# Diamondfan/CTC_pytorch

Measured on AMD Instinct MI355X. Metric: acoustic frames/sec/GPU (train) + utterances/sec beam-decode (`decode` object), TIMIT 4x320 BiLSTM, higher is better.
Workload: dtype f32 via bf16x3 split-operand MFMA (f32 accumulate); 1 GPU; cfg2: 4x320 BiLSTM + BN + Linear(62) + CTC, B=32/GPU, T=800, F=40, dropout 0.1, Adam; global_batch=32, seq_len=800, parallelism=dp1, full_length_utterances=True, sync_bn=False

## Files before the change

ctc_pytorch_amd/_lib.py:

```python
import ctypes
import glob
import os
import subprocess

import torch

_HERE = os.path.dirname(os.path.abspath(__file__))
_CSRC = os.path.join(_HERE, "csrc")
SO_PATH = os.environ.get("CTCN_LIBCTCN") or os.path.join(_HERE, "libctcn.so")
_lib = None

c_void_p, c_int, c_float, c_double, c_size_t, c_u64 = (ctypes.c_void_p, ctypes.c_int, ctypes.c_float,
                                                      ctypes.c_double, ctypes.c_size_t, ctypes.c_uint64)

P, I, F, D, Z, U = c_void_p, c_int, c_float, c_double, c_size_t, c_u64
_SIGS = {
    "ctcn_version": (I, []),
    "ctcn_last_error": (ctypes.c_char_p, []),
    "ctcn_device_cus": (I, []),
    "ctcn_device_xcds": (I, []),
    "ctcn_set_option": (I, [ctypes.c_char_p, I]),
    "ctcn_get_option": (I, [ctypes.c_char_p]),
    "ctcn_option_name": (ctypes.c_char_p, [I]),
    "ctcn_set_status_buffer": (I, [P]),
    "ctcn_gemm": (I, [I, I, I, I, I, P, I, P, I, P, I, F, I, P, Z, P]),
    "ctcn_gemm_dx": (I, [I, I, I, P, I, P, I, P, I, F, I, P, Z, P]),
    "ctcn_transpose01": (I, [P, P, I, I, I, P]),
    "ctcn_copy_strided4": (I, [P, P, I, I, I, I, Z, Z, Z, Z, P]),
    "ctcn_relu_fwd": (I, [P, P, Z, P]),
    "ctcn_relu_bwd": (I, [P, P, P, Z, P]),
    "ctcn_maxpool2d_fwd": (I, [P, P, P, Z, I, I, I, I, P]),
    "ctcn_maxpool2d_bwd": (I, [P, P, P, Z, I, I, I, I, P]),
    "ctcn_rnn_scratch_bytes": (Z, [I, I, I, I]),
    "ctcn_rnn_fwd": (I, [I, I, I, I, I, I, P, P, P, P, P, P, P, P, I, P, Z, P]),
    "ctcn_rnn_fwd_dropout": (I, [I, I, I, I, I, I, P, P, P, P, P, P, P, P, P, F, U, U, I, P, Z, P]),
    "ctcn_rnn_bwd": (I, [I, I, I, I, I, I, P, P, P, P, P, P, P, P, P, P, P, P, P, P, F, I, P, P, Z, P]),
    "ctcn_rnn_bwd_dropout": (I, [I, I, I, I, I, I, P, P, P, P, P, P, P, P, P, P, P, P, P, P, F, I, P, P, Z, P, F, U, U, P]),
    "ctcn_rnn_bwd_weights": (I, [I, I, I, I, I, I, P, P, P, P, P, P, P, P, F, I, ctypes.c_uint, P, Z, P]),
    "ctcn_bn_ws_bytes": (Z, [I, I, I]),
    "ctcn_bn_fwd_train": (I, [P, P, P, P, P, P, P, P, I, I, I, F, F, I, P, Z, P, P]),
    "ctcn_bn_fwd_eval": (I, [P, P, P, P, P, P, I, I, I, F, I, P]),
    "ctcn_bn_fwd_sums": (I, [P, P, I, I, I, P, Z, P]),
    "ctcn_bn_fwd_finish": (I, [P, P, P, P, P, P, P, P, P, D, I, I, I, F, F, I, P, P]),
    "ctcn_bn_bwd_sums": (I, [P, P, P, P, P, P, I, I, I, I, P, Z, P]),
    "ctcn_bn_bwd_finish": (I, [P, P, P, P, P, P, P, P, P, P, P, D, I, I, I, I, F, P, Z, P]),
    "ctcn_bn_bwd": (I, [P, P, P, P, P, P, P, P, P, I, I, I, I, F, P, Z, P]),
    "ctcn_bn_fwd_train_dropout": (I, [P, P, P, P, P, P, P, P, I, I, I, F, F, I, P, Z, P, P, F, U, U]),
    "ctcn_bn_bwd_dropout": (I, [P, P, P, P, P, P, P, P, P, I, I, I, I, F, P, Z, P, F, U, U]),
    "ctcn_dropout": (I, [P, P, Z, F, U, U, P]),
    "ctcn_bn_masked_ws_bytes": (Z, [I, I, I]),
    "ctcn_mask_frames": (I, [P, P, P, I, I, I, I, I, P]),
    "ctcn_bn_fwd_train_masked": (I, [P, P, P, P, P, P, P, P, P, I, I, I, I, I, F, F, I, P, Z, P, P]),
    "ctcn_bn_fwd_eval_masked": (I, [P, P, P, P, P, P, P, I, I, I, I, I, F, I, P]),
    "ctcn_bn_bwd_masked": (I, [P, P, P, P, P, P, P, P, P, P, I, I, I, I, I, I, F, P, Z, P]),
    "ctcn_conv2d_ws_bytes": (Z, [I] * 11),
    "ctcn_conv2d_fwd": (I, [P, P, P, P] + [I] * 11 + [P]),
    "ctcn_conv2d_bwd": (I, [P, P, P, P, P, P] + [I] * 11 + [F, P, Z, P]),
    "ctcn_bctf_to_tbcf": (I, [P, P, I, I, I, I, P]),
    "ctcn_tbcf_to_bctf": (I, [P, P, I, I, I, I, P]),
    "ctcn_log_softmax_fwd": (I, [P, P, P, I, I, P]),
    "ctcn_log_softmax_bwd": (I, [P, P, P, I, I, P]),
    "ctcn_argmax": (I, [P, P, I, I, P]),
    "ctcn_rnn_fwd_ex": (I, [I, I, I, I, I, I, P, P, P, P, P, P, P, P, I, P, Z, P, P]),
    "ctcn_rnn_bwd_ex": (I, [I, I, I, I, I, I, P, P, P, P, P, P, P, P, P, P, P, P, P, P, F, I, P, P, Z, P, P]),
    "ctcn_ctc_fwd": (I, [P, P, P, P, P, P, I, I, I, I, P]),
    "ctcn_ctc_bwd": (I, [P, P, P, P, P, P, P, P, I, I, I, I, P]),
    "ctcn_ctc_fwd_both": (I, [P, P, P, P, P, P, P, I, I, I, I, P]),
    "ctcn_ctc_grad": (I, [P, P, P, P, P, P, P, P, P, I, I, I, I, P]),
    "ctcn_sum_f32": (I, [P, P, I, P]),
    "ctcn_ctc_fwd_ex": (I, [P, P, P, P, P, P, P, I, I, I, I, I, P]),
    "ctcn_ctc_grad_ex": (I, [P, P, P, P, P, P, P, P, I, I, I, I, P, I, I, I, I, P]),
    "ctcn_ctc_reduce": (I, [P, P, P, I, I, I, P]),
    "ctcn_ctc_pack_targets": (I, [P, ctypes.c_int64, P, P, I, I, P]),
    "ctcn_ctc_align_ws_bytes": (Z, [I, I, I]),
    "ctcn_ctc_align": (I, [P, P, P, P, P, P, P, P, P, P, I, I, I, I, I, P, Z, P]),
    "ctcn_adam_step": (I, [P, P, P, P, Z, F, F, F, F, F, I, P]),
    "ctcn_grad_norm_ws_bytes": (Z, [Z, I]),
    "ctcn_grad_norm": (I, [P, Z, I, P, I, P, P, P, I, P, Z, P]),
    "ctcn_clip_control": (I, [P, F, F, F, F, I, P]),
    "ctcn_adam_step_ex": (I, [P, P, P, P, Z, F, F, F, F, P, P]),
    "ctcn_scale_by_device_scalar": (I, [P, Z, P, P]),
    "ctcn_greedy_collapse": (I, [P, Z, Z, P, P, P, I, I, I, P]),
    "ctcn_path_tokens": (I, [P, Z, Z, P, P, P, P, P, P, P, P, P, P, I, I, I, I, P]),
    "ctcn_edit_distance": (I, [P, P, P, P, P, I, I, I, I, P]),
    "ctcn_edit_ops_ws_bytes": (Z, [I, I, I]),
    "ctcn_edit_ops": (I, [P, P, P, P, P, I, P, P, P, P, I, I, I, I, P, Z, P]),
    "ctcn_step_stats": (I, [P, P, P, I, P, P, P]),
    "ctcn_fbank_frames": (I, [ctypes.c_longlong, I, I, I]),
    "ctcn_fbank_plan_bytes": (Z, [P]),
    "ctcn_fbank_plan": (I, [P, P, Z]),
    "ctcn_fbank": (I, [P, I, P, P, P, P, P, P, P, I, I, I, F, U, U, P]),
    "ctcn_mfcc_plan_bytes": (Z, [P]),
    "ctcn_mfcc_plan": (I, [P, P, Z]),
    "ctcn_mfcc": (I, [P, I, P, P, P, P, P, P, P, I, I, I, F, U, U, P]),
    "ctcn_spectrogram_plan_bytes": (Z, [P]),
    "ctcn_spectrogram_plan": (I, [P, P, Z]),
    "ctcn_spectrogram": (I, [P, I, P, P, P, P, P, P, P, I, I, I, F, U, U, P]),
    "ctcn_logspec_frames": (I, [ctypes.c_longlong, I]),
    "ctcn_logspec_plan_bytes": (Z, [P]),
    "ctcn_logspec_plan": (I, [P, P, Z]),
    "ctcn_logspec_ws_bytes": (Z, [P, I, I]),
    "ctcn_logspec": (I, [P, I, P, P, P, P, P, P, I, I, I, P, Z, P]),
    "ctcn_fbank_power_host": (I, [P, I, P]),
    "ctcn_resample_samples": (I, [ctypes.c_longlong, I, I]),
    "ctcn_resample_plan_bytes": (Z, [P]),
    "ctcn_resample_plan": (I, [P, P, Z]),
    "ctcn_resample": (I, [P, I, P, P, P, P, I, I, I, P]),
    "ctcn_resample_host": (I, [P, I, I, P, P, P, I]),
    "ctcn_context_frames": (I, [I, I, I]),
    "ctcn_delta_scales": (I, [I, I, P]),
    "ctcn_frame_context_tile": (I, [P, I]),
    "ctcn_frame_context": (I, [P, P, P, P, P, P, I, I, I, I, P]),
    "ctcn_frame_context_host": (I, [P, I, I, P, P, I, P]),
    "ctcn_spec_augment": (I, [P, P, P, U, U, P, I, I, I, P]),
    "ctcn_spec_augment_plan": (I, [P, U, U, I, I, P, P, P]),
    "ctcn_spec_augment_host": (I, [P, I, I, P, U, U, P]),
    "ctcn_reverb_limits": (I, [P]),
    "ctcn_reverb_bank_bytes": (Z, [I, I, I, I, I]),
    "ctcn_reverb_bank": (I, [P, P, I, I, P, P, I, I, P, I, D, P, Z]),
    "ctcn_reverb_plan": (I, [P, P, U, U, P]),
    "ctcn_reverb_ws_bytes": (Z, [P, I, I]),
    "ctcn_reverb": (I, [P, I, P, P, P, P, U, U, P, I, I, P, Z, P]),
    "ctcn_reverb_host": (I, [P, I, I, P, P, U, U, P]),
    "ctcn_cmvn_accumulate_ws_bytes": (Z, [I, I, I]),
    "ctcn_cmvn_accumulate": (I, [P, P, P, I, I, I, P, Z, P]),
    "ctcn_cmvn_accumulate_groups": (I, [P, P, P, P, I, I, I, I, P, Z, P]),
    "ctcn_cmvn_apply": (I, [P, P, P, P, P, I, I, I, I, I, P]),
    "ctcn_cmvn_sliding": (I, [P, P, P, I, I, I, P, P]),
    "ctcn_cmvn_sliding_run": (I, [P]),
    "ctcn_cmvn_sliding_window": (I, [I, I, P, P, P]),
    "ctcn_cmvn_sliding_host": (I, [P, I, I, P, P]),
    "ctcn_cmvn_norm_host": (I, [P, I, I, P, P]),
    "ctcn_comm_unique_id": (I, [P]),
    "ctcn_comm_init": (I, [P, I, I, ctypes.POINTER(ctypes.c_void_p)]),
    "ctcn_comm_allreduce_sum_f32": (I, [P, P, Z, P]),
    "ctcn_comm_destroy": (I, [P]),
    "ctcn_diag_squat": (I, [I, I, I, ctypes.c_uint, P]),
    "ctcn_diag_pipeline_chunks": (I, [I, I, I, I, I, I, I, I, ctypes.c_uint]),
    "ctcn_diag_gemm_plan": (I, [I] * 13 + [Z, ctypes.c_uint, I, I, I, I, P]),
    "ctcn_diag_dx_plan": (I, [I, I, I, I, I, I, I, Z, I, P]),
    "ctcn_diag_beam_plan": (I, [I, I, I, I, I, I, P]),
    "ctcn_diag_ctc_lattice_plan": (I, [I, P]),
    "ctcn_diag_gemm_on_xcds": (I, [I, I, I, I, I, P, I, P, I, P, I, F, I, P, Z, P, ctypes.c_uint]),
    "ctcn_rnn_last_kernel": (ctypes.c_char_p, [I]),
    "ctcn_levenshtein": (ctypes.c_longlong, [P, ctypes.c_longlong, P, ctypes.c_longlong]),
    "ctcn_levenshtein_ops": (ctypes.c_longlong, [P, ctypes.c_longlong, P, ctypes.c_longlong, P, P]),
    "ctcn_join_tokens": (ctypes.c_longlong, [P, ctypes.c_longlong, P, I, P, P, P, I, I, P, ctypes.c_longlong, P]),
    "ctcn_beam_ws_bytes": (Z, [I, I, I, I]),
    "ctcn_beam_decode": (I, [P, I, P, P, D, I, I, P, P, P, P, I, I, I, P, Z, P]),
    "ctcn_beam_decode_nbest": (I, [P, I, P, P, D, I, I, I, P, P, P, P, P, I, I, I, P, Z, P]),
}


class RnnCall(ctypes.Structure):
    _fields_ = [("drop_p", ctypes.c_float), ("drop_seed", ctypes.c_uint64), ("drop_offset", ctypes.c_uint64), ("y_drop", ctypes.c_void_p),
                ("dy_tmp", ctypes.c_void_p), ("side_stream", ctypes.c_void_p), ("side_event", ctypes.c_void_p), ("side_ws", ctypes.c_void_p),
                ("side_ws_bytes", ctypes.c_size_t), ("xcd_allow", ctypes.c_uint), ("prelaunch_event", ctypes.c_void_p), ("status", ctypes.c_void_p),
                ("launched", ctypes.POINTER(ctypes.c_char_p))]


class FbankOpts(ctypes.Structure):
    _fields_ = [(k, ctypes.c_float) for k in ("samp_freq", "frame_shift_ms", "frame_length_ms", "preemph_coeff", "blackman_coeff", "low_freq",
                                              "high_freq", "energy_floor")] + \
               [(k, ctypes.c_int32) for k in ("window_type", "num_mel_bins", "remove_dc_offset", "round_to_power_of_two", "snip_edges",
                                              "use_energy", "raw_energy", "htk_compat", "use_log_fbank", "use_power")]


class MfccOpts(ctypes.Structure):
    _fields_ = [(k, ctypes.c_float) for k in ("samp_freq", "frame_shift_ms", "frame_length_ms", "preemph_coeff", "blackman_coeff", "low_freq",
                                              "high_freq", "energy_floor", "cepstral_lifter")] + \
               [(k, ctypes.c_int32) for k in ("window_type", "num_mel_bins", "num_ceps", "remove_dc_offset", "round_to_power_of_two", "snip_edges",
                                              "use_energy", "raw_energy", "htk_compat")]


class SpectrogramOpts(ctypes.Structure):
    _fields_ = [(k, ctypes.c_float) for k in ("samp_freq", "frame_shift_ms", "frame_length_ms", "preemph_coeff", "blackman_coeff", "energy_floor")] + \
               [(k, ctypes.c_int32) for k in ("window_type", "remove_dc_offset", "round_to_power_of_two", "snip_edges", "raw_energy", "return_raw_fft")]


class LogSpecOpts(ctypes.Structure):
    _fields_ = [(k, ctypes.c_double) for k in ("sample_rate", "window_size", "window_stride")] + [("input_scale", ctypes.c_float)] + \
               [(k, ctypes.c_int32) for k in ("window", "normalize")]


class ResampleOpts(ctypes.Structure):
    _fields_ = [("cutoff", ctypes.c_double)] + [(k, ctypes.c_int32) for k in ("orig_freq", "new_freq", "num_zeros")]


class ContextOpts(ctypes.Structure):
    _fields_ = [(k, ctypes.c_int32) for k in ("left", "right", "skip", "n_downsample", "delta_order", "delta_window")]


class SpecAugOpts(ctypes.Structure):
    _fields_ = [(k, ctypes.c_int32) for k in ("warp_window", "num_freq_masks", "freq_width", "num_time_masks", "time_width")] + \
               [(k, ctypes.c_float) for k in ("time_ratio", "fill")]


class ReverbOpts(ctypes.Structure):
    _fields_ = [("rir_prob", ctypes.c_float), ("noise_prob", ctypes.c_float), ("normalize", ctypes.c_int32)]


class SlidingCmnOpts(ctypes.Structure):
    _fields_ = [(k, ctypes.c_int32) for k in ("cmn_window", "min_cmn_window", "normalize_variance", "center")]


def sources():
    return sorted(glob.glob(os.path.join(_CSRC, "*.hip")))


def build(force=False, verbose=False):
    from concurrent.futures import ThreadPoolExecutor
    srcs = sources()
    hdrs = glob.glob(os.path.join(_CSRC, "*.h")) + [os.path.join(os.path.dirname(_HERE), "include", "ctcn.h")]
    hipcc = os.environ.get("HIPCC", "/opt/rocm/bin/hipcc")
    objdir = os.path.join(_CSRC, "_obj")
    os.makedirs(objdir, exist_ok=True)
    hdr_time = max(os.path.getmtime(h) for h in hdrs)
    flags = ["--offload-arch=gfx950", "-O3", "-std=c++17", "-fPIC"]
    jobs, objs = [], []
    for src in srcs:
        obj = os.path.join(objdir, os.path.basename(src)[:-4] + ".o")
        objs.append(obj)
        if force or not os.path.exists(obj) or os.path.getmtime(obj) < max(os.path.getmtime(src), hdr_time):
            jobs.append([hipcc] + flags + ["-c", src, "-o", obj])

    def run(cmd):
        if verbose:
            print(" ".join(cmd), flush=True)
        subprocess.check_call(cmd)

    if jobs:
        with ThreadPoolExecutor(max_workers=min(len(jobs), os.cpu_count() or 4)) as pool:
            list(pool.map(run, jobs))
    if jobs or not os.path.exists(SO_PATH) or any(os.path.getmtime(SO_PATH) < os.path.getmtime(o) for o in objs):
        run([hipcc, "--offload-arch=gfx950", "-fPIC", "-shared", "-o", SO_PATH] + objs)
    return SO_PATH


def lib():
    global _lib
    if _lib is None:
        if not os.path.exists(SO_PATH):
            raise RuntimeError(
                "ctc_pytorch_amd: %s is missing -- run `python -c 'import __graft_entry__ as g; g.build()'` "
                "(hipcc --offload-arch=gfx950). There is no CPU fallback." % SO_PATH)
        l = ctypes.CDLL(SO_PATH)
        for name, (res, args) in _SIGS.items():
            fn = getattr(l, name)
            fn.restype = res
            fn.argtypes = args
        _lib = l
        for var, opt in (("CTCN_RNN_PERSISTENT", b"rnn_persistent"), ("CTCN_HANDOFF", b"handoff"), ("CTCN_GEMM_BIG_TILES", b"gemm_big_tiles"), ("CTCN_BWD_SCATTER", b"bwd_scatter"), ("CTCN_HANDOFF_TAGS", b"handoff_tags"), ("CTCN_SIDE_SPLIT_WGS", b"side_split_wgs")):
            env = os.environ.get(var)
            if env is not None:
                l.ctcn_set_option(opt, int(env))
        for var, val in os.environ.items():
            if var.startswith("CTCN_OPT_"):
                check(l.ctcn_set_option(var[len("CTCN_OPT_"):].lower().encode(), int(val)), "set_option(%s)" % var)
    return _lib


def exported_symbols():
    return sorted(_SIGS)


def check(rc, what=""):
    if rc != 0:
        msg = lib().ctcn_last_error()
        raise RuntimeError("libctcn %s failed (rc=%d): %s" % (what, rc, msg.decode() if msg else "?"))


def stream_ptr():
    return torch.cuda.current_stream().cuda_stream


_STATUS = {}


def status_word(device):
    key = (device.type, device.index)
    t = _STATUS.get(key)
    if t is None:
        t = torch.zeros(1, dtype=torch.int32, device=device)
        _STATUS[key] = t
        check(lib().ctcn_set_status_buffer(ctypes.c_void_p(t.data_ptr())), "set_status_buffer")
    return t


def check_status(device):
    t = _STATUS.get((device.type, device.index))
    if t is not None:
        v = int(t.item())
        if v != 0:
            t.zero_()
            raise RuntimeError("libctcn: persistent recurrent kernel reported status %d (in-launch hand-off timed out)" % v)


_WS = {}
_WS_LOCK = __import__("threading").Lock()
WORKSPACE_BYTES = int(os.environ.get("CTCN_WORKSPACE_MB", "1024")) << 20


def workspace(device, nbytes=None, tag="main"):
    nbytes = WORKSPACE_BYTES if nbytes is None else nbytes
    key = (device.type, device.index, tag)
    buf = _WS.get(key)
    if buf is None or buf.numel() < nbytes:
        with _WS_LOCK:
            buf = _WS.get(key)
            if buf is None or buf.numel() < nbytes:
                buf = torch.empty(nbytes, dtype=torch.uint8, device=device)
# ... 3 lines not shown
```

ctc_pytorch_amd/csrc/common.h:

```cpp
#pragma once
#include <hip/hip_runtime.h>
#include <stdarg.h>
#include <stdint.h>
#include <stdio.h>
#include <string.h>

#include "../../include/ctcn.h"

void ctcn_set_error(const char *fmt, ...);
int *ctcn_status_word(void);
int ctcn_opt_rnn_persistent(void);
int ctcn_transpose01_pair(const float *in0, const float *in1, float *out0, float *out1, int A, int B, int C, void *stream);
struct GemmPlanes {
  const float *A = nullptr; int lda = 0, M = 0, Ka = 0, transA = 0; void *ws_a = nullptr, *st_a = nullptr; bool a_valid = false;
  const float *B = nullptr; int ldb = 0, N = 0, Kb = 0, transB = 0, shift = 0; void *ws_b = nullptr, *st_b = nullptr; const void *bh = nullptr; bool b_valid = false;
  bool same_a = false, same_b = false;
};
int ctcn_gemm_on_xcds(int transA, int transB, int M, int N, int K, const float *A, int lda, const float *B, int ldb, float *C,
                      int ldc, float beta, int precision, void *ws, size_t ws_bytes, void *stream, unsigned xcd_allow, GemmPlanes *planes = nullptr);
int ctcn_gemm_shift_b(int M, int N, int K, const float *A, int lda, const float *B, int ldb, float *C, int ldc, float beta, int precision,
                      void *ws, size_t ws_bytes, void *stream, unsigned xcd_allow, int shift, GemmPlanes *planes = nullptr);
int ctcn_opt_handoff(void);
int ctcn_opt_poll_depth(void);
int ctcn_opt_bwd_scatter(void);
int ctcn_opt_handoff_tags(void);
int ctcn_opt_side_split_wgs(void);
int ctcn_opt_gemm_big_tiles(void);
int ctcn_opt_recurrence_only(void);

#define CTCN_REQUIRE(cond, ...)          \
  do {                                   \
    if (!(cond)) {                       \
      ctcn_set_error(__VA_ARGS__);       \
      return CTCN_EINVAL;                \
    }                                    \
  } while (0)

#define CTCN_HIP(expr)                                                                   \
  do {                                                                                   \
    hipError_t e__ = (expr);                                                             \
    if (e__ != hipSuccess) {                                                             \
      ctcn_set_error("%s:%d: %s -> %s", __FILE__, __LINE__, #expr, hipGetErrorString(e__)); \
      return CTCN_EHIP;                                                                  \
    }                                                                                    \
  } while (0)

#define CTCN_LAUNCH_CHECK() CTCN_HIP(hipGetLastError())

typedef float f32x4 __attribute__((ext_vector_type(4)));
typedef float f32x16 __attribute__((ext_vector_type(16)));
typedef short bf16x8 __attribute__((ext_vector_type(8)));
typedef unsigned int u32x4 __attribute__((ext_vector_type(4)));

static inline int ceil_div(int a, int b) { return (a + b - 1) / b; }
static inline size_t ceil_div_z(size_t a, size_t b) { return (a + b - 1) / b; }
static inline size_t align_up(size_t a, size_t b) { return (a + b - 1) / b * b; }

__device__ __forceinline__ float wave_max(float v) {
#pragma unroll
  for (int o = 32; o > 0; o >>= 1) v = fmaxf(v, __shfl_xor(v, o, 64));
  return v;
}
__device__ __forceinline__ float wave_sum(float v) {
#pragma unroll
  for (int o = 32; o > 0; o >>= 1) v += __shfl_xor(v, o, 64);
  return v;
}
__device__ __forceinline__ double wave_sum_d(double v) {
#pragma unroll
  for (int o = 32; o > 0; o >>= 1) v += __shfl_xor(v, o, 64);
  return v;
}
__device__ __forceinline__ void lds_barrier() { asm volatile("s_waitcnt lgkmcnt(0)\n\ts_barrier" ::: "memory"); }

__device__ __forceinline__ float sigmoidf_(float x) { return 1.0f / (1.0f + expf(-x)); }

__host__ __device__ __forceinline__ void philox_round(uint32_t (&c)[4], uint32_t (&k)[2]) {
  const uint32_t M0 = 0xD2511F53u, M1 = 0xCD9E8D57u;
#if defined(__HIP_DEVICE_COMPILE__)
  const uint32_t hi0 = __umulhi(M0, c[0]), lo0 = M0 * c[0];
  const uint32_t hi1 = __umulhi(M1, c[2]), lo1 = M1 * c[2];
#else
  const uint32_t hi0 = (uint32_t)(((uint64_t)M0 * c[0]) >> 32), lo0 = M0 * c[0];
  const uint32_t hi1 = (uint32_t)(((uint64_t)M1 * c[2]) >> 32), lo1 = M1 * c[2];
#endif
  const uint32_t n0 = hi1 ^ c[1] ^ k[0], n1 = lo1, n2 = hi0 ^ c[3] ^ k[1], n3 = lo0;
  c[0] = n0; c[1] = n1; c[2] = n2; c[3] = n3;
  k[0] += 0x9E3779B9u; k[1] += 0xBB67AE85u;
}
__host__ __device__ __forceinline__ void philox4(uint64_t seed, uint64_t ctr, uint32_t (&out)[4]) {
  uint32_t c[4] = {(uint32_t)ctr, (uint32_t)(ctr >> 32), 0u, 0u};
  uint32_t k[2] = {(uint32_t)seed, (uint32_t)(seed >> 32)};
#pragma unroll
  for (int i = 0; i < 10; ++i) philox_round(c, k);
#pragma unroll
  for (int i = 0; i < 4; ++i) out[i] = c[i];
}

__device__ __forceinline__ unsigned short f2bf(float f) {
  return __builtin_bit_cast(unsigned short, (__bf16)f);
}
```

ctc_pytorch_amd/csrc/core.hip:

```cpp
#include "common.h"

static thread_local char g_err[512] = "";

void ctcn_set_error(const char *fmt, ...) {
  va_list ap;
  va_start(ap, fmt);
  vsnprintf(g_err, sizeof(g_err), fmt, ap);
  va_end(ap);
}

extern "C" int ctcn_version(void) { return 100; }
extern "C" const char *ctcn_last_error(void) { return g_err; }
extern "C" int ctcn_device_cus(void) {
  int dev = 0, n = 0;
  if (hipGetDevice(&dev) != hipSuccess) return -1;
  if (hipDeviceGetAttribute(&n, hipDeviceAttributeMultiprocessorCount, dev) != hipSuccess) return -1;
  return n;
}

static int g_opt_rnn_persistent = 1;
static int g_opt_handoff = 1;
static int g_opt_poll_depth = 2;
static int g_opt_recurrence_only = 0;
static int g_opt_bwd_scatter = 1;
static int g_opt_handoff_tags = 1;
static int g_opt_side_split_wgs = 8;
static int g_opt_gemm_big_tiles = 0;
static int g_opt_gemm_tile256 = 1;
static int g_opt_gemm_dbg = 0;
static int g_opt_gemm_a_inline = 1;
static int g_opt_conv_mfma = 1;
static int g_opt_rnn_fwd_tagged = 1;
static int g_opt_rnn_fused_dropout = 1;
static int g_opt_gemm_tn = 1;
static int g_opt_tag_poll_delay = 8;
static int g_opt_edit_wave = 1;
static int g_opt_bwd_item_gather = 1;
static int g_opt_bwd_poll_delay = -1;
static int g_opt_fwd_rsv_lds = 2;
static int g_opt_fwd_pipe_any_chunking = 0;
static int g_opt_fwd_pipe_min_input = 0;
static int g_opt_conv_dbg = 0;
static int g_opt_gemm_bf16_single = 0;
static int g_opt_gemm_dx_wide = 1;
static int g_opt_xcd_interleave = 1;
static int g_opt_bn_rows4 = 1;
static int g_opt_tn_splits_force = 0;
static int g_opt_tn_splits_xcd = 1;
static int g_opt_beam_generic_threads = 0;
static int g_opt_beam_bitonic = 1;
static int g_opt_beam_cand_global = 0;
static int g_opt_beam_occ2 = 0;
static int g_opt_beam_fast = 1;
static int g_opt_rnn_slow_items = 0;
static int g_opt_rnn_slow_exchange = 0;
static int g_opt_ctc_lattice_skew = 1;
static int g_opt_ctc_slow_wave = 0;
static int g_opt_xcd_interleave_force = 0;
static int *g_status_dev = nullptr;

struct OptionRow { const char *name; int *var; int (*norm)(int); };
static const OptionRow k_options[] = {
  {"rnn_persistent", &g_opt_rnn_persistent, [](int value) -> int { return value; }},
  {"handoff", &g_opt_handoff, [](int value) -> int { return value; }},
  {"poll_depth", &g_opt_poll_depth, [](int value) -> int { return value; }},
  {"rnn_recurrence_only", &g_opt_recurrence_only, [](int value) -> int { return value ? 1 : 0; }},
  {"bwd_scatter", &g_opt_bwd_scatter, [](int value) -> int { return value ? 1 : 0; }},
  {"handoff_tags", &g_opt_handoff_tags, [](int value) -> int { return value ? 1 : 0; }},
  {"side_split_wgs", &g_opt_side_split_wgs, [](int value) -> int { return value < 1 ? 1 : (value > 16 ? 16 : value); }},
  {"gemm_big_tiles", &g_opt_gemm_big_tiles, [](int value) -> int { return value ? 1 : 0; }},
  {"beam_fast", &g_opt_beam_fast, [](int value) -> int { return value ? 1 : 0; }},
  {"conv_dbg", &g_opt_conv_dbg, [](int value) -> int { return value & 7; }},
  {"tn_splits_xcd", &g_opt_tn_splits_xcd, [](int value) -> int { return value ? 1 : 0; }},
  {"xcd_interleave", &g_opt_xcd_interleave, [](int value) -> int { return value < 0 ? 0 : (value > 5 ? 5 : value); }},
  {"bn_rows4", &g_opt_bn_rows4, [](int value) -> int { return value ? 1 : 0; }},
  {"tn_splits_force", &g_opt_tn_splits_force, [](int value) -> int { return value < 0 ? 0 : value; }},
  {"gemm_bf16_single", &g_opt_gemm_bf16_single, [](int value) -> int { return value ? 1 : 0; }},
  {"gemm_dx_wide", &g_opt_gemm_dx_wide, [](int value) -> int { return value < 0 ? 0 : (value > 2 ? 2 : value); }},
  {"beam_generic_threads", &g_opt_beam_generic_threads, [](int value) -> int { return (value == 256 || value == 512 || value == 1024) ? value : 0; }},
  {"beam_cand_global", &g_opt_beam_cand_global, [](int value) -> int { return value ? 1 : 0; }},
  {"beam_bitonic", &g_opt_beam_bitonic, [](int value) -> int { return value ? 1 : 0; }},
  {"beam_occ2", &g_opt_beam_occ2, [](int value) -> int { return value < 0 ? 0 : (value > 2 ? 2 : value); }},
  {"fwd_pipe_min_input", &g_opt_fwd_pipe_min_input, [](int value) -> int { return value < 0 ? 0 : value; }},
  {"fwd_pipe_any_chunking", &g_opt_fwd_pipe_any_chunking, [](int value) -> int { return value ? 1 : 0; }},
  {"fwd_rsv_lds", &g_opt_fwd_rsv_lds, [](int value) -> int { return value < 0 ? 0 : (value > 2 ? 2 : value); }},
  {"bwd_item_gather", &g_opt_bwd_item_gather, [](int value) -> int { return value < 0 ? 0 : (value > 2 ? 2 : value); }},
  {"bwd_poll_delay", &g_opt_bwd_poll_delay, [](int value) -> int { return value < 0 ? -1 : (value > 256 ? 256 : value); }},
  {"conv_mfma", &g_opt_conv_mfma, [](int value) -> int { return value ? 1 : 0; }},
  {"edit_wave", &g_opt_edit_wave, [](int value) -> int { return value ? 1 : 0; }},
  {"gemm_tn", &g_opt_gemm_tn, [](int value) -> int { return value != 0; }},
  {"rnn_fused_dropout", &g_opt_rnn_fused_dropout, [](int value) -> int { return value != 0; }},
  {"tag_poll_delay", &g_opt_tag_poll_delay, [](int value) -> int { return value < 0 ? 0 : (value > 64 ? 64 : value); }},
  {"rnn_fwd_tagged", &g_opt_rnn_fwd_tagged, [](int value) -> int { return value ? 1 : 0; }},
  {"gemm_a_inline", &g_opt_gemm_a_inline, [](int value) -> int { return value ? 1 : 0; }},
  {"gemm_dbg", &g_opt_gemm_dbg, [](int value) -> int { return value; }},
  {"gemm_tile256", &g_opt_gemm_tile256, [](int value) -> int { return value ? 1 : 0; }},
  {"xcd_interleave_force", &g_opt_xcd_interleave_force, [](int value) -> int { return value ? 1 : 0; }},
  {"rnn_slow_exchange", &g_opt_rnn_slow_exchange, [](int value) -> int { return value < 0 ? 0 : (value > 4096 ? 4096 : value); }},
  {"ctc_lattice_skew", &g_opt_ctc_lattice_skew, [](int value) -> int { return value ? 1 : 0; }},
  {"ctc_slow_wave", &g_opt_ctc_slow_wave, [](int value) -> int { return value < 0 ? 0 : (value > 15 ? 15 : value); }},
  {"rnn_slow_items", &g_opt_rnn_slow_items, [](int value) -> int { return value < 0 ? 0 : (value > 4096 ? 4096 : value); }},
};
static const int k_noptions = (int)(sizeof(k_options) / sizeof(k_options[0]));
static const OptionRow *find_option(const char *name) {
  if (name)
    for (int i = 0; i < k_noptions; ++i)
      if (!strcmp(name, k_options[i].name)) return &k_options[i];
  return nullptr;
}
extern "C" int ctcn_set_option(const char *name, int value) {
  if (const OptionRow *o = find_option(name)) { *o->var = o->norm(value); return CTCN_OK; }
  ctcn_set_error("ctcn_set_option: unknown option %s", name ? name : "(null)");
  return CTCN_EINVAL;
}
extern "C" int ctcn_get_option(const char *name) {
  const OptionRow *o = find_option(name);
  return o ? *o->var : -1;
}
extern "C" const char *ctcn_option_name(int index) { return index >= 0 && index < k_noptions ? k_options[index].name : nullptr; }
extern "C" int ctcn_set_status_buffer(int *dev_word) { g_status_dev = dev_word; return CTCN_OK; }
int *ctcn_status_word(void) { return g_status_dev; }
int ctcn_opt_rnn_persistent(void) { return g_opt_rnn_persistent; }
int ctcn_opt_handoff(void) { return g_opt_handoff; }
int ctcn_opt_poll_depth(void) { return g_opt_poll_depth; }
int ctcn_opt_recurrence_only(void) { return g_opt_recurrence_only; }
int ctcn_opt_bwd_scatter(void) { return g_opt_bwd_scatter; }
int ctcn_opt_handoff_tags(void) { return g_opt_handoff_tags; }
int ctcn_opt_side_split_wgs(void) { return g_opt_side_split_wgs; }
int ctcn_opt_gemm_big_tiles(void) { return g_opt_gemm_big_tiles; }
```

ctc_pytorch_amd/csrc/gemm.hip:

```cpp
#include <algorithm>
#include <type_traits>

#include "common.h"

namespace {

constexpr int BM = 128, BN = 128, BK = 16, PAD = 4;

__device__ __forceinline__ int xcd_band_tile(int bid, int nt) {
  const int xcd = bid & 7, q = nt >> 3, r = nt & 7;
  return (xcd < r ? xcd * (q + 1) : r * (q + 1) + (xcd - r) * q) + (bid >> 3);
}
__device__ __forceinline__ void g2r_kc(const float *__restrict__ src, int ld, int r0, int R, int k0, int Kend,
                                       bool vec, int tid, float (&reg)[8]) {
#pragma unroll
  for (int j = 0; j < 2; ++j) {
    const int idx = tid + 256 * j;
    const int r = idx >> 2, kq = (idx & 3) * 4;
    const int gr = r0 + r, gk = k0 + kq;
    const float *p = src + (size_t)gr * ld + gk;
    if (vec && gr < R && gk + 3 < Kend) {
      const float4 v = *reinterpret_cast<const float4 *>(p);
      reg[4 * j + 0] = v.x; reg[4 * j + 1] = v.y; reg[4 * j + 2] = v.z; reg[4 * j + 3] = v.w;
    } else {
#pragma unroll
      for (int c = 0; c < 4; ++c) reg[4 * j + c] = (gr < R && gk + c < Kend) ? p[c] : 0.0f;
    }
  }
}
__device__ __forceinline__ void r2s_kc(float (*s)[BM + PAD], int tid, const float (&reg)[8]) {
#pragma unroll
  for (int j = 0; j < 2; ++j) {
    const int idx = tid + 256 * j;
    const int r = idx >> 2, kq = (idx & 3) * 4;
#pragma unroll
    for (int c = 0; c < 4; ++c) s[kq + c][r] = reg[4 * j + c];
  }
}
__device__ __forceinline__ void g2r_mc(const float *__restrict__ src, int ld, int r0, int R, int k0, int Kend,
                                       bool vec, int tid, float (&reg)[8]) {
#pragma unroll
  for (int j = 0; j < 2; ++j) {
    const int idx = tid + 256 * j;
    const int k = idx >> 5, rq = (idx & 31) * 4;
    const int gk = k0 + k, gr = r0 + rq;
    const float *p = src + (size_t)gk * ld + gr;
    if (vec && gk < Kend && gr + 3 < R) {
      const float4 v = *reinterpret_cast<const float4 *>(p);
      reg[4 * j + 0] = v.x; reg[4 * j + 1] = v.y; reg[4 * j + 2] = v.z; reg[4 * j + 3] = v.w;
    } else {
#pragma unroll
      for (int c = 0; c < 4; ++c) reg[4 * j + c] = (gk < Kend && gr + c < R) ? p[c] : 0.0f;
    }
  }
}
__device__ __forceinline__ void r2s_mc(float (*s)[BM + PAD], int tid, const float (&reg)[8]) {
#pragma unroll
  for (int j = 0; j < 2; ++j) {
    const int idx = tid + 256 * j;
    const int k = idx >> 5, rq = (idx & 31) * 4;
    *reinterpret_cast<float4 *>(&s[k][rq]) = make_float4(reg[4 * j], reg[4 * j + 1], reg[4 * j + 2], reg[4 * j + 3]);
  }
}

template <bool TA, bool TB>
__device__ __forceinline__ void f32_tile(float (*sA)[BM + PAD], float (*sB)[BN + PAD], int bid, int split, int M, int N, int K,
                                         const float *__restrict__ A, int lda, const float *__restrict__ B, int ldb, float *__restrict__ C,
                                         int ldc, float beta, int kchunk, float *__restrict__ ws, int tiles_n, bool vecA, bool vecB) {
  const int tid = threadIdx.x, lane = tid & 63, wave = tid >> 6;
  const int wm = wave >> 1, wn = wave & 1;
  const int tm = bid / tiles_n, tn = bid - tm * tiles_n;
  const int m0 = tm * BM, n0 = tn * BN;
  const int kbeg = split * kchunk;
  const int kend = min(K, kbeg + kchunk);

  f32x16 acc[2][2];
#pragma unroll
  for (int i = 0; i < 2; ++i)
#pragma unroll
    for (int j = 0; j < 2; ++j)
#pragma unroll
      for (int e = 0; e < 16; ++e) acc[i][j][e] = 0.0f;

  float ra[8], rb[8];
  auto loadA = [&](int k0) {
    if (TA) g2r_mc(A, lda, m0, M, k0, kend, vecA, tid, ra);
    else g2r_kc(A, lda, m0, M, k0, kend, vecA, tid, ra);
  };
  auto loadB = [&](int k0) {
    if (TB) g2r_kc(B, ldb, n0, N, k0, kend, vecB, tid, rb);
    else g2r_mc(B, ldb, n0, N, k0, kend, vecB, tid, rb);
  };
  if (kbeg < kend) {
    loadA(kbeg);
    loadB(kbeg);
  }
  for (int k0 = kbeg; k0 < kend; k0 += BK) {
    __syncthreads();
    if (TA) r2s_mc(sA, tid, ra); else r2s_kc(sA, tid, ra);
    if (TB) r2s_kc(sB, tid, rb); else r2s_mc(sB, tid, rb);
    __syncthreads();
    if (k0 + BK < kend) {
      loadA(k0 + BK);
      loadB(k0 + BK);
    }
    const int kl = lane >> 5, ml = lane & 31;
#pragma unroll
    for (int k = 0; k < BK; k += 2) {
      const float a0 = sA[k + kl][wm * 64 + ml], a1 = sA[k + kl][wm * 64 + 32 + ml];
      const float b0 = sB[k + kl][wn * 64 + ml], b1 = sB[k + kl][wn * 64 + 32 + ml];
      acc[0][0] = __builtin_amdgcn_mfma_f32_32x32x2f32(a0, b0, acc[0][0], 0, 0, 0);
      acc[0][1] = __builtin_amdgcn_mfma_f32_32x32x2f32(a0, b1, acc[0][1], 0, 0, 0);
      acc[1][0] = __builtin_amdgcn_mfma_f32_32x32x2f32(a1, b0, acc[1][0], 0, 0, 0);
      acc[1][1] = __builtin_amdgcn_mfma_f32_32x32x2f32(a1, b1, acc[1][1], 0, 0, 0);
    }
  }
  float *out = ws ? ws + (size_t)split * M * N : C;
  const int ldo = ws ? N : ldc;
#pragma unroll
  for (int i = 0; i < 2; ++i)
#pragma unroll
    for (int j = 0; j < 2; ++j) {
      const int col = n0 + wn * 64 + j * 32 + (lane & 31);
#pragma unroll
      for (int e = 0; e < 16; ++e) {
        const int row = m0 + wm * 64 + i * 32 + (e & 3) + 8 * (e >> 2) + 4 * (lane >> 5);
        if (row < M && col < N) {
          float v = acc[i][j][e];
          float *p = out + (size_t)row * ldo + col;
          if (!ws && beta != 0.0f) v += beta * *p;
          *p = v;
        }
      }
    }
}

template <bool TA, bool TB>
__global__ __launch_bounds__(256) void gemm_f32_kernel(int M, int N, int K, const float *__restrict__ A, int lda,
                                                       const float *__restrict__ B, int ldb, float *__restrict__ C,
                                                       int ldc, float beta, int kchunk, float *__restrict__ ws,
                                                       int tiles_m, int tiles_n, bool vecA, bool vecB) {
  __shared__ __attribute__((aligned(16))) float sA[BK][BM + PAD];
  __shared__ __attribute__((aligned(16))) float sB[BK][BN + PAD];
  const int bid = xcd_band_tile(blockIdx.x, tiles_m * tiles_n);
  f32_tile<TA, TB>(sA, sB, bid, blockIdx.y, M, N, K, A, lda, B, ldb, C, ldc, beta, kchunk, ws, tiles_n, vecA, vecB);
}

template <bool TA, bool TB>
__global__ __launch_bounds__(256) void gemm_f32_queue_kernel(int M, int N, int K, const float *__restrict__ A, int lda,
                                                             const float *__restrict__ B, int ldb, float *__restrict__ C, int ldc,
                                                             float beta, int kchunk, float *__restrict__ ws, int tiles_m, int tiles_n,
                                                             bool vecA, bool vecB, int splits, unsigned xcd_allow,
                                                             unsigned *__restrict__ queue) {
// ... 961 lines not shown
    for (int t = 0; t < 3; ++t)
#pragma unroll
      for (int i = 0; i < WI; ++i)
#pragma unroll
        for (int j = 0; j < WJ; ++j) {
          if (t == 0) acc[i][j] = __builtin_amdgcn_mfma_f32_32x32x16_bf16(al[i], bh[j], acc[i][j], 0, 0, 0);
          else if (t == 1) acc[i][j] = __builtin_amdgcn_mfma_f32_32x32x16_bf16(ah[i], bl[j], acc[i][j], 0, 0, 0);
          else acc[i][j] = __builtin_amdgcn_mfma_f32_32x32x16_bf16(ah[i], bh[j], acc[i][j], 0, 0, 0);
          const int n = t * NMM + i * WJ + j;
          if (n < NBP || n == CV0 || n == CV0 + 1) {
            __builtin_amdgcn_sched_barrier(0);
            if constexpr (WHICH == 1) {
              if (HAS1 && n < NBP) issue_b_piece(n, (s + 1) * 32, (s + 1) & 1);
              if (HAS1 && n == CV0) {
                static_assert(NBP == 5, "vmcnt literals");
                if constexpr (HAS2) WAIT_A(7, 1); else WAIT_A(5, 1);
              }
              if (HAS1 && n >= CV0) convert_half(1, n - CV0, (s + 1) * 32);
            } else {
              if (HAS2 && n == CV0) WAIT_A(2, 0);
              if (HAS2 && n >= CV0) convert_half(0, n - CV0, (s + 2) * 32);
            }
            __builtin_amdgcn_sched_barrier(0);
          }
        }
  };
  constexpr std::integral_constant<int, 1> first{};
  constexpr std::integral_constant<int, 2> second{};
  constexpr std::integral_constant<bool, true> yes{};
  constexpr std::integral_constant<bool, false> no{};
#pragma unroll
  for (int q = 0; q < 4; ++q) aw[q] = (u32x4){0u, 0u, 0u, 0u};
#pragma unroll
  for (int q = 0; q < 4; ++q) load_a_piece(q, 0);
#pragma unroll
  for (int n = 0; n < NBP; ++n) issue_b_piece(n, 0, 0);
  WAIT_A(0, 0); WAIT_A(0, 1);
#pragma unroll
  for (int r = 0; r < 2; ++r) {
    convert_half(r, 0, 0); convert_half(r, 1, 0);
    store_a_row(r, 0);
  }
  if (nst > 1) {
    asm volatile("s_waitcnt lgkmcnt(0)" ::: "memory");
#pragma unroll
    for (int q = 0; q < 4; ++q) load_a_piece(q, 32);
    WAIT_A(2, 0);
    convert_half(0, 0, 32); convert_half(0, 1, 32);
  }
  pp_barrier_vm();
  if (wave >= 4) pp_barrier();
#ifdef CTCN_GEMM_STATS
  long long gs_work[4] = {0, 0, 0, 0}, gs_wait[4] = {0, 0, 0, 0};
  const long long gs_t0 = clock64();
  long long gs_prev = gs_t0;
#endif
  auto stage = [&](int s, auto has1, auto has2) {
    constexpr bool HAS1 = decltype(has1)::value, HAS2 = decltype(has2)::value;
    load_frags(s, 0);
    if constexpr (HAS1) store_a_row(0, (s + 1) & 1);
    if constexpr (HAS2) {
      __builtin_amdgcn_sched_barrier(0);
      load_a_piece(0, (s + 2) * 32); load_a_piece(1, (s + 2) * 32);
    }
    PPB(0);
    multiply(first, has1, has2, s);
    PPB(1);
    load_frags(s, 1);
    if constexpr (HAS1) store_a_row(1, (s + 1) & 1);
    if constexpr (HAS2) {
      __builtin_amdgcn_sched_barrier(0);
      load_a_piece(2, (s + 2) * 32); load_a_piece(3, (s + 2) * 32);
    }
#ifdef CTCN_GEMM_STATS
    PPB_VM(2);
#else
    __builtin_amdgcn_sched_barrier(0);
    if constexpr (HAS2) asm volatile("s_waitcnt vmcnt(2) lgkmcnt(0)\n\ts_barrier" ::: "memory");
    else asm volatile("s_waitcnt vmcnt(0) lgkmcnt(0)\n\ts_barrier" ::: "memory");
    __builtin_amdgcn_sched_barrier(0);
#endif
    multiply(second, has1, has2, s);
    PPB(3);
  };
  int s = 0;
  for (; s + 2 < nst; ++s) stage(s, yes, yes);
#ifdef CTCN_GEMM_STATS
  if (lane == 0 && (wave & 3) == 0 && (blockIdx.x == 0 || blockIdx.x == 1000) && g_gemm_stats) {
    long long *o = g_gemm_stats + ((blockIdx.x ? 2 : 0) + (wave >> 2)) * 16;
    for (int i = 0; i < 4; ++i) { o[i] = gs_work[i]; o[4 + i] = gs_wait[i]; }
    o[8] = clock64() - gs_t0; o[9] = nst - 2; o[10] = 0;
  }
#endif
  if (s + 1 < nst) { stage(s, yes, no); ++s; }
  stage(s, no, no);
  if (wave < 4) pp_barrier();
  int zero = 0;
  asm volatile("" : "+v"(zero));
  const int elane = (int)__builtin_amdgcn_mbcnt_hi(~0u, __builtin_amdgcn_mbcnt_lo(~0u, (unsigned)zero));
#pragma unroll
  for (int i = 0; i < WI; ++i)
#pragma unroll
    for (int j = 0; j < WJ; ++j) {
      const int col = n0 + wn * 160 + j * 32 + (elane & 31);
#pragma unroll
      for (int e = 0; e < 16; ++e) {
        const int row = m0 + wm * 64 + i * 32 + (e & 3) + 8 * (e >> 2) + 4 * (elane >> 5);
        if (row < M) {
          float v = acc[i][j][e];
          float *p = C + (size_t)row * ldc + col;
          if (beta != 0.0f) v += beta * *p;
          *p = v;
        }
      }
    }
}


typedef short s16x4_t __attribute__((ext_vector_type(4)));
typedef short s16x8_t __attribute__((ext_vector_type(8)));

template <int WNT, int NP = 3>
__global__ __launch_bounds__(512) void gemm_tn_f32_pp_kernel(int M, int N, int K, const float *__restrict__ A, int lda, const float *__restrict__ B,
                                                             int ldb, float *__restrict__ C, int ldc, float beta, int kchunk, int splits,
                                                             float *__restrict__ part, int tiles_m, int tiles_n, unsigned xcd_mask,
                                                             unsigned *__restrict__ queue) {
  constexpr int TBM = 256, TBN = 128 * WNT;
  constexpr int A_BYTES = TBM * 64, B_BYTES = TBN * 64;
  constexpr int STAGE = 2 * A_BYTES + 2 * B_BYTES;
  constexpr int NB = 2 * WNT;
  constexpr int NMM = 4 * WNT;
  extern __shared__ __attribute__((aligned(16))) unsigned char qsm[];
  __shared__ int s_item;
  {
    unsigned xcc;
    asm volatile("s_getreg_b32 %0, hwreg(HW_REG_XCC_ID)" : "=s"(xcc));
    if (!((xcd_mask >> (xcc & 15u)) & 1u)) return;
  }
  const int tid = threadIdx.x, lane = tid & 63, wave = __builtin_amdgcn_readfirstlane(tid >> 6);
  const int wm = wave >> 2, wn = wave & 3;
  const int nt = tiles_m * tiles_n;
  const int krow = lane >> 3, c4 = 4 * (lane & 7);
  const int bsub = WNT == 2 ? wave : (wave & 3), bk0 = WNT == 2 ? 0 : 16 * (wave >> 2);
  const int st_a = wave * 2048 + krow * 64 + (lane & 7) * 8;
  const int st_b = 2 * A_BYTES + bsub * 2048 + (bk0 + krow) * 64 + (lane & 7) * 8;
  const int troff = (8 * (lane >> 5) + ((lane & 15) >> 2)) * 64 + ((lane >> 4) & 1) * 32 + (lane & 3) * 8;
  typedef __attribute__((address_space(3))) s16x4_t *lds4_t;

  for (;;) {
    if (tid == 0) s_item = (int)atomicAdd(queue, 1u);
    __syncthreads();
    const int item = __builtin_amdgcn_readfirstlane(s_item);
    if (item >= nt * splits) return;
    const int z = item / nt, tile = item - z * nt;
    const int tm = tile / tiles_n, tn = tile - tm * tiles_n;
    const int m0 = tm * TBM, n0 = tn * TBN;
    const int kbeg = z * kchunk, kend = min(K, kbeg + kchunk);
    const int nst = (kend - kbeg + 31) / 32;

    f32x16 acc[4][WNT];
#pragma unroll
    for (int i = 0; i < 4; ++i)
#pragma unroll
      for (int j = 0; j < WNT; ++j)
#pragma unroll
        for (int e = 0; e < 16; ++e) acc[i][j][e] = 0.0f;

    const int acol = m0 + 32 * wave + c4, bcol = n0 + 32 * bsub + c4;
    const bool a_ok = acol < M, b_ok = bcol < N;
    u32x4 pw[4 + NB];
    const unsigned voff_a = a_ok ? (unsigned)((krow * lda + acol) * 4) : 0xfffffff0u;
    const unsigned voff_b = b_ok ? (unsigned)((krow * ldb + bcol) * 4) : 0xfffffff0u;
    auto load_piece = [&](int q, int k0) {
      const int kr = q < 4 ? k0 + 8 * q : k0 + bk0 + 8 * (q - 4);
      const int ld = q < 4 ? lda : ldb;
      const float *base = (q < 4 ? A : B) + (size_t)min(kr, K - 1) * ld;
      int rows = min(8, kend - kr);
      asm volatile("" : "+s"(rows));
      const int nrec = max(0, rows) * ld * 4;
      const __amdgpu_buffer_rsrc_t rs = __builtin_amdgcn_make_buffer_rsrc(const_cast<float *>(base), 0, nrec, 0x00020000);
      pw[q] = __builtin_amdgcn_raw_buffer_load_b128(rs, q < 4 ? voff_a : voff_b, 0, 0);
    };
    auto split_pair = [](float a, float b, unsigned &hw, unsigned &lw) {
      typedef __bf16 bf16x2_t __attribute__((ext_vector_type(2)));
      typedef float f32x2_t __attribute__((ext_vector_type(2)));
      hw = __builtin_bit_cast(unsigned, __builtin_convertvector((f32x2_t){a, b}, bf16x2_t));
      const f32x2_t r = {a - __uint_as_float(hw << 16), b - __uint_as_float(hw & 0xffff0000u)};
      lw = __builtin_bit_cast(unsigned, __builtin_convertvector(r, bf16x2_t));
    };
    auto convert_piece = [&](int q) {
      unsigned h01, l01, h23, l23;
      if constexpr (NP == 3) {
        split_pair(__uint_as_float(pw[q][0]), __uint_as_float(pw[q][1]), h01, l01);
        split_pair(__uint_as_float(pw[q][2]), __uint_as_float(pw[q][3]), h23, l23);
      } else {
        typedef __bf16 bf16x2_t __attribute__((ext_vector_type(2)));
        typedef float f32x2_t __attribute__((ext_vector_type(2)));
        h01 = __builtin_bit_cast(unsigned, __builtin_convertvector((f32x2_t){__uint_as_float(pw[q][0]), __uint_as_float(pw[q][1])}, bf16x2_t));
        h23 = __builtin_bit_cast(unsigned, __builtin_convertvector((f32x2_t){__uint_as_float(pw[q][2]), __uint_as_float(pw[q][3])}, bf16x2_t));
        l01 = l23 = 0u;
      }
      pw[q] = (u32x4){h01, h23, l01, l23};
    };
    auto store_ab = [&](int buf) {
      unsigned char *sb = qsm + buf * STAGE;
#pragma unroll
      for (int q = 0; q < 4 + NB; ++q) {
        unsigned char *p = sb + (q < 4 ? st_a + q * 512 : st_b + (q - 4) * 512);
        *reinterpret_cast<uint2 *>(p) = make_uint2(pw[q][0], pw[q][1]);
        if constexpr (NP == 3) *reinterpret_cast<uint2 *>(p + (q < 4 ? A_BYTES : B_BYTES)) = make_uint2(pw[q][2], pw[q][3]);
      }
    };
    bf16x8_t ah[4], al[4], bh[WNT], bl[WNT];
    auto tr_frag = [&](const unsigned char *p) {
      const s16x4_t x0 = __builtin_amdgcn_ds_read_tr16_b64_v4i16((lds4_t)(p));
      const s16x4_t x1 = __builtin_amdgcn_ds_read_tr16_b64_v4i16((lds4_t)(p + 256));
      return __builtin_bit_cast(bf16x8_t, __builtin_shufflevector(x0, x1, 0, 1, 2, 3, 4, 5, 6, 7));
    };
    auto load_frags = [&](int stage, int ks) {
      const unsigned char *sb = qsm + (stage & 1) * STAGE + ks * 1024 + troff;
#pragma unroll
      for (int j = 0; j < WNT; ++j) {
        const unsigned char *p = sb + 2 * A_BYTES + (wn * WNT + j) * 2048;
        bh[j] = tr_frag(p);
        if constexpr (NP == 3) bl[j] = tr_frag(p + B_BYTES);
      }
#pragma unroll
      for (int i = 0; i < 4; ++i) {
        const unsigned char *p = sb + (wm * 4 + i) * 2048;
        ah[i] = tr_frag(p);
        if constexpr (NP == 3) al[i] = tr_frag(p + A_BYTES);
      }
    };
    auto multiply = [&](auto mode, int k0) {
      constexpr int MODE = decltype(mode)::value;
      constexpr int NITEM = MODE == 1 ? 4 : 4 + NB;
#pragma unroll
      for (int t = 0; t < NP; ++t)
#pragma unroll
        for (int i = 0; i < 4; ++i)
#pragma unroll
          for (int j = 0; j < WNT; ++j) {
            if (NP == 3 && t == 0) acc[i][j] = __builtin_amdgcn_mfma_f32_32x32x16_bf16(al[i], bh[j], acc[i][j], 0, 0, 0);
            else if (NP == 3 && t == 1) acc[i][j] = __builtin_amdgcn_mfma_f32_32x32x16_bf16(ah[i], bl[j], acc[i][j], 0, 0, 0);
            else acc[i][j] = __builtin_amdgcn_mfma_f32_32x32x16_bf16(ah[i], bh[j], acc[i][j], 0, 0, 0);
            const int n = t * NMM + i * WNT + j;
            if constexpr (NP == 3) {
              if (MODE != 0 && (n & 1) && (n >> 1) < NITEM) {
                __builtin_amdgcn_sched_barrier(0);
                if constexpr (MODE == 1) load_piece(n >> 1, k0);
                if constexpr (MODE == 2) convert_piece(n >> 1);
                __builtin_amdgcn_sched_barrier(0);
              }
            } else if (MODE != 0 && 2 * n < NITEM) {
              __builtin_amdgcn_sched_barrier(0);
#pragma unroll
              for (int u = 2 * n; u < 2 * n + 2 && u < NITEM; ++u) {
                if constexpr (MODE == 1) load_piece(u, k0);
                if constexpr (MODE == 2) convert_piece(u);
              }
              __builtin_amdgcn_sched_barrier(0);
            }
          }
    };
    constexpr std::integral_constant<int, 0> bare{};
    constexpr std::integral_constant<int, 1> with_loads{};
    constexpr std::integral_constant<int, 2> with_split{};
#pragma unroll
    for (int q = 0; q < 4 + NB; ++q) load_piece(q, kbeg);
#pragma unroll
    for (int q = 0; q < 4 + NB; ++q) convert_piece(q);
    store_ab(0);
    if (nst > 1) {
#pragma unroll
      for (int q = 0; q < 4; ++q) load_piece(q, kbeg + 32);
    }
    pp_barrier();
    if (wm == 1) pp_barrier();
#ifdef CTCN_GEMM_STATS
    long long gs_work[4] = {0, 0, 0, 0}, gs_wait[4] = {0, 0, 0, 0};
    const long long gs_t0 = clock64();
    long long gs_prev = gs_t0;
#endif
    auto stage = [&](int s, auto do_store, auto c1) {
      load_frags(s, 0);
      if constexpr (decltype(do_store)::value == 1) {
        __builtin_amdgcn_sched_barrier(0);
#pragma unroll
        for (int q = 4; q < 4 + NB; ++q) load_piece(q, kbeg + (s + 1) * 32);
      }
      PPB(0);
      if constexpr (decltype(do_store)::value == 1) multiply(with_split, 0);
      else multiply(bare, 0);
      PPB(1);
      load_frags(s, 1);
      if constexpr (decltype(do_store)::value == 1) store_ab((s + 1) & 1);
      PPB(2);
      multiply(c1, kbeg + (s + 2) * 32);
      PPB(3);
    };
    int s = 0;
    for (; s + 2 < nst; ++s) stage(s, with_loads, with_loads);
#ifdef CTCN_GEMM_STATS
    if (lane == 0 && (wave & 3) == 0 && item == 0 && g_gemm_stats) {
      long long *o = g_gemm_stats + (wave >> 2) * 16;
      for (int i = 0; i < 4; ++i) { o[i] = gs_work[i]; o[4 + i] = gs_wait[i]; }
      o[8] = clock64() - gs_t0; o[9] = nst - 2; o[10] = 0;
    }
#endif
    if (s + 1 < nst) { stage(s, with_loads, bare); ++s; }
    stage(s, bare, bare);
    if (wm == 0) pp_barrier();

    float *o = splits > 1 ? part + (size_t)z * M * N : C;
    const int ldo = splits > 1 ? N : ldc;
    const float bt = splits > 1 ? 0.0f : beta;
#pragma unroll
    for (int i = 0; i < 4; ++i)
#pragma unroll
      for (int j = 0; j < WNT; ++j) {
        const int col = n0 + wn * 32 * WNT + j * 32 + (lane & 31);
#pragma unroll
        for (int e = 0; e < 16; ++e) {
          const int row = m0 + wm * 128 + i * 32 + (e & 3) + 8 * (e >> 2) + 4 * (lane >> 5);
          if (row < M && col < N) {
            float v = acc[i][j][e];
            float *p = o + (size_t)row * ldo + col;
            if (bt != 0.0f) v += bt * *p;
            *p = v;
          }
        }
      }
    __syncthreads();
  }
}

__global__ void splitk_reduce_kernel(const float *__restrict__ ws, float *__restrict__ C, int M, int N, int ldc,
                                     int splits, float beta) {
  const size_t total = (size_t)M * N;
  if ((N & 3) == 0 && (ldc & 3) == 0 && (((uintptr_t)C | (uintptr_t)ws) & 15) == 0 && total < ((size_t)1 << 33)) {
    const unsigned n4 = (unsigned)(N >> 2), total4 = (unsigned)(total >> 2);
    const float4 *w4 = reinterpret_cast<const float4 *>(ws);
    for (unsigned i = blockIdx.x * blockDim.x + threadIdx.x; i < total4; i += gridDim.x * blockDim.x) {
      float4 s = {0.0f, 0.0f, 0.0f, 0.0f};
      int z = 0;
      for (; z + 8 <= splits; z += 8) {
        float4 v[8];
#pragma unroll
        for (int u = 0; u < 8; ++u) v[u] = w4[(size_t)(z + u) * total4 + i];
#pragma unroll
        for (int u = 0; u < 8; ++u) { s.x += v[u].x; s.y += v[u].y; s.z += v[u].z; s.w += v[u].w; }
      }
      for (; z < splits; ++z) { const float4 v = w4[(size_t)z * total4 + i]; s.x += v.x; s.y += v.y; s.z += v.z; s.w += v.w; }
      const unsigned m = i / n4, n = (i - m * n4) << 2;
      float4 *p = reinterpret_cast<float4 *>(C + (size_t)m * ldc + n);
      if (beta != 0.0f) { const float4 o = *p; s.x += beta * o.x; s.y += beta * o.y; s.z += beta * o.z; s.w += beta * o.w; }
      *p = s;
    }
    return;
  }
  for (size_t i = blockIdx.x * (size_t)blockDim.x + threadIdx.x; i < total; i += (size_t)gridDim.x * blockDim.x) {
    float s = 0.0f;
    int z = 0;
    for (; z + 8 <= splits; z += 8) {
      float v[8];
#pragma unroll
      for (int u = 0; u < 8; ++u) v[u] = ws[(size_t)(z + u) * total + i];
#pragma unroll
      for (int u = 0; u < 8; ++u) s += v[u];
    }
    for (; z < splits; ++z) s += ws[(size_t)z * total + i];
    const size_t m = i / N, n = i - m * N;
    float *p = C + m * ldc + n;
    if (beta != 0.0f) s += beta * *p;
    *p = s;
  }
}

__global__ void transpose01_kernel(const float *__restrict__ in, float *__restrict__ out, int A, int B, int C) {
  const size_t total = (size_t)A * B * C;
  for (size_t i = blockIdx.x * (size_t)blockDim.x + threadIdx.x; i < total; i += (size_t)gridDim.x * blockDim.x) {
    const int c = i % C;
    const size_t ab = i / C;
    const int a = ab % A;
    const int b = ab / A;
    out[i] = in[((size_t)a * B + b) * C + c];
  }
}

}

enum GemmPath { GP_F32 = 0, GP_F32_QUEUE, GP_BF16X3, GP_PLANES128, GP_PLANES128_QUEUE, GP_PLANES256, GP_PLANES256_AF32, GP_PLANES256_QUEUE, GP_TN };
enum SplitPass { SP_NONE = 0, SP_ROWS, SP_TRANSPOSE, SP_TRANSPOSE_QUEUE };
struct GemmShape { int transA, transB, M, N, K, lda, ldb, ldc, precision, b_shift; };
struct GemmOptions { int tile256, a_inline, tn, big_tiles, tn_splits_xcd, tn_splits_force; };
struct GemmEnv {
  int a_mod16, b_mod16;
  bool has_ws;
  size_t ws_bytes;
  unsigned xcd_allow;
  bool same_a, same_b;
  int cus, xcds;
  GemmOptions opt;
};
struct GemmPlan {
  GemmPath path;
  int ti, tj;
  int wnt;
  int splits, kchunk;
  SplitPass split_a, split_b;
  int Kp;
  size_t off_al, off_bh, off_bl, off_part, off_queue;
  int tiles_m, tiles_n;
  unsigned grid_x, grid_y;
  bool vecA, vecB;
  unsigned xcd_mask;
};
static bool uses_planes(GemmPath p) { return p >= GP_PLANES128 && p <= GP_PLANES256_QUEUE; }
static GemmOptions gemm_options() {
  return {ctcn_get_option("gemm_tile256"), ctcn_get_option("gemm_a_inline"), ctcn_get_option("gemm_tn"), ctcn_opt_gemm_big_tiles(),
          ctcn_get_option("tn_splits_xcd"), ctcn_get_option("tn_splits_force")};
}
static int check_gemm_shape(const GemmShape &g) {
  CTCN_REQUIRE(g.precision == 0 || g.precision == 1, "ctcn_gemm: precision %d (0 = f32 MFMA, 1 = bf16x3 split MFMA)", g.precision);
  CTCN_REQUIRE(g.M > 0 && g.N > 0 && g.K >= 0, "ctcn_gemm: bad dims M=%d N=%d K=%d", g.M, g.N, g.K);
  CTCN_REQUIRE(g.lda >= (g.transA ? g.M : g.K) && g.ldb >= (g.transB ? g.K : g.N) && g.ldc >= g.N, "ctcn_gemm: leading dim too small");
  return CTCN_OK;
}
struct PlaneLayout { int Kp; size_t a_el, b_el, bytes; };
static PlaneLayout plane_layout(int M, int N, int K) {
  const int Kp = ceil_div(K, PBK) * PBK;
  const size_t a_el = (size_t)M * Kp, b_el = (size_t)N * Kp;
  return {Kp, a_el, b_el, align_up(2 * (a_el + b_el) * sizeof(unsigned short), 256)};
}
static bool tn_eligible(const GemmShape &g, const GemmEnv &e) {
  return g.precision == 1 && g.transA && !g.transB && e.has_ws && e.ws_bytes >= 1024 && e.opt.tn != 0 && g.M >= 128 && g.N >= 32 && g.K >= 1024 &&
         g.M % 4 == 0 && g.N % 4 == 0 && g.lda % 4 == 0 && g.ldb % 4 == 0 && e.a_mod16 == 0 && e.b_mod16 == 0 &&
         g.lda < (1 << 24) && g.ldb < (1 << 24);
}

static GemmPlan plan_gemm(const GemmShape &g, const GemmEnv &e) {
  const int M = g.M, N = g.N, K = g.K;
  const size_t mn_bytes = (size_t)M * N * sizeof(float);
  GemmPlan p = {};
  p.splits = 1;
  p.off_queue = e.ws_bytes >= 256 ? (e.ws_bytes - 256) & ~(size_t)255 : 0;
  if (tn_eligible(g, e) && g.b_shift == 0) {
    p.path = GP_TN;
    p.wnt = ceil_div(N, 256) * 256 == ceil_div(N, 128) * 128 ? 2 : 1;
    p.ti = 4; p.tj = 2 * p.wnt;
    p.tiles_m = ceil_div(M, 256); p.tiles_n = ceil_div(N, 128 * p.wnt);
    int cus = 256;
    if (e.xcd_allow && e.opt.tn_splits_xcd != 0) {
      const int nx = std::max(1, std::min(e.xcds, 16));
      cus = std::max(e.cus / nx * __builtin_popcount(e.xcd_allow & ((1u << nx) - 1u)), 32);
    }
    const int tiles = p.tiles_m * p.tiles_n;
    int s = std::min(std::max(cus / tiles, 1), std::max(K / 512, 1));
    s = std::min(s, 32);
    if (const int f = e.opt.tn_splits_force) s = std::min(f, std::max(K / 64, 1));
    s = std::min(s, (int)((e.ws_bytes - 512) / mn_bytes));
    if (s < 2) s = 1;
    p.kchunk = ceil_div(ceil_div(K, s), 32) * 32;
    p.splits = ceil_div(K, p.kchunk);
    const int nx = std::min(e.xcds, 16);
    p.xcd_mask = e.xcd_allow ? e.xcd_allow : (nx > 1 ? (1u << nx) - 1u : 0xffffu);
    p.grid_x = e.cus; p.grid_y = 1;
    return p;
  }
  const PlaneLayout lay = plane_layout(M, N, K);
  if (g.precision == 1 && K >= 64 && e.has_ws && e.ws_bytes >= lay.bytes + 1024) {
    const int Kp = p.Kp = lay.Kp;
    p.off_al = lay.a_el * sizeof(unsigned short); p.off_bh = 2 * p.off_al; p.off_bl = p.off_bh + lay.b_el * sizeof(unsigned short);
    p.off_part = lay.bytes;
    const size_t part_bytes = e.ws_bytes - lay.bytes - 512;
    p.kchunk = Kp;
    const SplitPass pass_a = g.transA == 0 ? SP_ROWS : (e.xcd_allow ? SP_TRANSPOSE_QUEUE : SP_TRANSPOSE);
    const SplitPass pass_b = g.transB != 0 ? SP_ROWS : (e.xcd_allow ? SP_TRANSPOSE_QUEUE : SP_TRANSPOSE);
    p.split_b = e.same_b ? SP_NONE : pass_b;
    const int wnt256 = (N % 256 == 0 || (N > 512 && ceil_div(N, 256) * 256 - N <= N / 8)) ? 2 : 1;
    const int t256_m = ceil_div(M, 256), t256_n = ceil_div(N, 128 * wnt256);
    const bool use256 = !e.xcd_allow && e.opt.tile256 != 0 && M >= 1024 && N >= 96 && (long)t256_m * t256_n * 4 >= (long)e.cus * 3;
    const bool a_inline = use256 && !e.same_a && !g.transA && e.opt.a_inline != 0 && K >= 32 && K % 4 == 0 && g.lda % 4 == 0 && e.a_mod16 == 0 &&
                          t256_n <= 5;
    p.split_a = (a_inline || e.same_a) ? SP_NONE : pass_a;
    bool queue256 = false;
    if (e.xcd_allow && e.opt.tile256 != 0 && M >= 1024 && N >= 96) {
      const int cus = e.cus / std::max(1, std::min(e.xcds, 16)) * __builtin_popcount(e.xcd_allow);
      const int t256 = t256_m * t256_n, rounds = ceil_div(t256, std::max(cus, 1));
      queue256 = cus > 0 && t256 * 4 >= rounds * cus * 3;
    }
    if (use256 || queue256) {
      p.path = a_inline ? GP_PLANES256_AF32 : (use256 ? GP_PLANES256 : GP_PLANES256_QUEUE);
      p.wnt = wnt256; p.ti = 4; p.tj = 2 * wnt256;
      p.tiles_m = t256_m; p.tiles_n = t256_n;
      p.grid_x = queue256 ? e.cus : t256_m * t256_n; p.grid_y = 1;
      return p;
    }
    p.ti = p.tj = 2; p.tiles_m = ceil_div(M, BM); p.tiles_n = ceil_div(N, BN);
    {
      const long t22 = (long)p.tiles_m * p.tiles_n * 128 * 128;
      const int m42 = ceil_div(M, 256), n42 = ceil_div(N, 128), m24 = ceil_div(M, 128), n24 = ceil_div(N, 256);
      const long t42 = (long)m42 * n42 * 256 * 128, t24 = (long)m24 * n24 * 128 * 256;
      const bool ok42 = m42 * n42 >= e.cus && t42 <= t22 + t22 / 32, ok24 = m24 * n24 >= e.cus && t24 <= t22 + t22 / 32;
      if (e.opt.big_tiles && (ok42 || ok24)) {
        if (ok24 && (!ok42 || t24 <= t42)) { p.tj = 4; p.tiles_m = m24; p.tiles_n = n24; }
        else { p.ti = 4; p.tiles_m = m42; p.tiles_n = n42; }
      }
    }
    const int pnt = p.tiles_m * p.tiles_n;
    if (pnt < 256 && Kp >= 1024 && part_bytes >= 2 * mn_bytes) {
      p.splits = std::min(std::min(ceil_div(512, pnt), Kp / 512), (int)(part_bytes / mn_bytes));
      if (p.splits < 2) p.splits = 1;
    }
    if (p.splits > 1) {
      p.kchunk = ceil_div(ceil_div(Kp, p.splits), PBK) * PBK;
      p.splits = ceil_div(Kp, p.kchunk);
    }
    p.path = e.xcd_allow ? GP_PLANES128_QUEUE : GP_PLANES128;
    p.grid_x = e.xcd_allow ? 2 * e.cus : pnt; p.grid_y = e.xcd_allow ? 1 : p.splits;
    return p;
  }
  p.ti = p.tj = 2; p.tiles_m = ceil_div(M, BM); p.tiles_n = ceil_div(N, BN);
  const int nt = p.tiles_m * p.tiles_n;
  if (nt < 256 && K >= 512 && e.has_ws && e.ws_bytes >= 2 * mn_bytes) {
    p.splits = std::min(std::min(ceil_div(512, nt), K / 256), (int)(e.ws_bytes / mn_bytes));
    if (p.splits < 2) p.splits = 1;
  }
  p.kchunk = K;
// ... 52 lines not shown
  GemmPlanes scratch_planes;
  GemmPlanes &pl = planes ? *planes : scratch_planes;
  const bool want_same_a = pl.same_a, want_same_b = pl.same_b;
  pl.same_a = pl.same_b = false;
  const GemmShape g = {transA, transB, M, N, K, lda, ldb, ldc, precision, b_shift};
  if (const int rc = check_gemm_shape(g)) return rc;
  CTCN_REQUIRE(A && B && C, "ctcn_gemm: null pointer");
  CTCN_REQUIRE(!ws || (uintptr_t)ws % 16 == 0, "ctcn_gemm: the workspace must be 16-byte aligned");
  hipStream_t st = (hipStream_t)stream;
  char *const wsb = (char *)ws;
  const void *bh_here = wsb + 2 * plane_layout(M, N, K).a_el * sizeof(unsigned short);
  GemmEnv e = {(int)((uintptr_t)A & 15), (int)((uintptr_t)B & 15), ws != nullptr, ws_bytes, xcd_allow, false, false, ctcn_device_cus(), 0, gemm_options()};
  e.same_a = want_same_a && pl.a_valid && pl.A == A && pl.lda == lda && pl.M == M && pl.Ka == K && pl.transA == transA && pl.ws_a == ws && pl.st_a == (void *)st;
  e.same_b = want_same_b && pl.b_valid && pl.B == B && pl.ldb == ldb && pl.N == N && pl.Kb == K && pl.transB == transB && pl.shift == b_shift &&
             pl.ws_b == ws && pl.st_b == (void *)st && pl.bh == bh_here;
  if (xcd_allow || tn_eligible(g, e)) e.xcds = ctcn_device_xcds();
  const GemmPlan p = plan_gemm(g, e);

  unsigned short *ah = (unsigned short *)wsb, *al = (unsigned short *)(wsb + p.off_al), *bh = (unsigned short *)(wsb + p.off_bh),
                 *bl = (unsigned short *)(wsb + p.off_bl);
  float *part = p.splits > 1 ? (float *)(wsb + p.off_part) : nullptr;
  unsigned *queue = (unsigned *)(wsb + p.off_queue);
  pl.a_valid = pl.b_valid = false;
  if (uses_planes(p.path)) {
    pl.B = B; pl.ldb = ldb; pl.N = N; pl.Kb = K; pl.transB = transB; pl.shift = b_shift; pl.ws_b = ws;
    pl.st_b = (void *)st; pl.bh = (const void *)bh; pl.b_valid = true;
    if (p.path != GP_PLANES256_AF32) {
      pl.A = A; pl.lda = lda; pl.M = M; pl.Ka = K; pl.transA = transA; pl.ws_a = ws; pl.st_a = (void *)st;
      pl.a_valid = true;
    }
    if (xcd_allow) CTCN_HIP(hipMemsetAsync(queue, 0, 16, st));
    int nq = 0;
    launch_split(p.split_a, st, A, lda, M, K, p.Kp, ah, al, 0, xcd_allow, queue + (p.split_a == SP_TRANSPOSE_QUEUE ? ++nq : 0));
    launch_split(p.split_b, st, B, ldb, N, K, p.Kp, bh, bl, b_shift, xcd_allow, queue + (p.split_b == SP_TRANSPOSE_QUEUE ? ++nq : 0));
    CTCN_LAUNCH_CHECK();
  }
  const int tiles_m = p.tiles_m, tiles_n = p.tiles_n, Kp = p.Kp, kchunk = p.kchunk, splits = p.splits;
  const dim3 grid(p.grid_x, p.grid_y);
  int rc = CTCN_OK;
  switch (p.path) {
    case GP_TN:
      CTCN_HIP(hipMemsetAsync(queue, 0, 128, st));
      rc = with_wnt(p.wnt, [&](auto W) {
        constexpr int WNT = decltype(W)::value;
        return launch_tile256(bf16_single() ? gemm_tn_f32_pp_kernel<WNT, 1> : gemm_tn_f32_pp_kernel<WNT, 3>, p.grid_x, WNT, st, M, N, K, A, lda, B, ldb, C, ldc,
                              beta, kchunk, splits, part, tiles_m, tiles_n, p.xcd_mask, queue);
      });
      break;
    case GP_PLANES256_AF32:
      rc = with_wnt(p.wnt, [&](auto W) {
        constexpr int WNT = decltype(W)::value;
        return launch_tile256(bf16_single() ? gemm_planes_nt256pp_af32_kernel<WNT, 1> : gemm_planes_nt256pp_af32_kernel<WNT, 3>, p.grid_x, WNT, st, M, N, K, Kp,
                              A, lda, (const unsigned short *)bh, (const unsigned short *)bl, C, ldc, beta, tiles_m, tiles_n);
      });
      break;
    case GP_PLANES256:
      rc = with_wnt(p.wnt, [&](auto W) {
        constexpr int WNT = decltype(W)::value;
        return launch_tile256(bf16_single() ? gemm_planes_nt256pp_kernel<WNT, 1> : gemm_planes_nt256pp_kernel<WNT, 3>, p.grid_x, WNT, st, M, N, Kp,
                              (const unsigned short *)ah, (const unsigned short *)al, (const unsigned short *)bh, (const unsigned short *)bl, C, ldc, beta,
                              tiles_m, tiles_n, ctcn_get_option("gemm_dbg"));
      });
      break;
    case GP_PLANES256_QUEUE:
      rc = with_wnt(p.wnt, [&](auto W) {
        constexpr int WNT = decltype(W)::value;
        return launch_tile256(bf16_single() ? gemm_planes_nt256pp_queue_kernel<WNT, 1> : gemm_planes_nt256pp_queue_kernel<WNT, 3>, p.grid_x, WNT, st, M, N, Kp,
                              (const unsigned short *)ah, (const unsigned short *)al, (const unsigned short *)bh, (const unsigned short *)bl, C, ldc, beta,
                              tiles_m, tiles_n, xcd_allow, queue);
      });
      break;
    case GP_PLANES128:
    case GP_PLANES128_QUEUE: {
      auto launch = [&](auto TI_, auto TJ_) {
        constexpr int TI = decltype(TI_)::value, TJ = decltype(TJ_)::value;
        const size_t lds = (size_t)2 * (64 * TI + 64 * TJ) * 128;
        if (p.path == GP_PLANES128_QUEUE) {
          auto kern = gemm_planes_nt_queue_kernel<TI, TJ>;
          if (lds > 64 * 1024) CTCN_HIP(hipFuncSetAttribute(reinterpret_cast<const void *>(kern), hipFuncAttributeMaxDynamicSharedMemorySize, (int)lds));
          hipLaunchKernelGGL(kern, grid, dim3(256), lds, st, M, N, Kp, ah, al, bh, bl, C, ldc, beta, kchunk, part, tiles_m, tiles_n, splits, xcd_allow, queue);
        } else {
          auto kern = gemm_planes_nt_kernel<TI, TJ>;
          if (lds > 64 * 1024) CTCN_HIP(hipFuncSetAttribute(reinterpret_cast<const void *>(kern), hipFuncAttributeMaxDynamicSharedMemorySize, (int)lds));
          hipLaunchKernelGGL(kern, grid, dim3(256), lds, st, M, N, Kp, ah, al, bh, bl, C, ldc, beta, kchunk, part, tiles_m, tiles_n);
        }
        return (int)CTCN_OK;
      };
      constexpr std::integral_constant<int, 2> two{};
      constexpr std::integral_constant<int, 4> four{};
      rc = p.ti == 4 ? launch(four, two) : (p.tj == 4 ? launch(two, four) : launch(two, two));
      break;
    }
    case GP_F32_QUEUE:
      CTCN_HIP(hipMemsetAsync(queue, 0, 4, st));
      with_trans(transA, transB, [&](auto TA, auto TB) {
        hipLaunchKernelGGL((gemm_f32_queue_kernel<decltype(TA)::value, decltype(TB)::value>), grid, dim3(256), 0, st, M, N, K, A, lda, B, ldb, C, ldc, beta, kchunk,
                           part, tiles_m, tiles_n, p.vecA, p.vecB, splits, xcd_allow, queue);
      });
      break;
    case GP_F32:
      with_trans(transA, transB, [&](auto TA, auto TB) {
        hipLaunchKernelGGL((gemm_f32_kernel<decltype(TA)::value, decltype(TB)::value>), grid, dim3(256), 0, st, M, N, K, A, lda, B, ldb, C, ldc, beta, kchunk, part,
                           tiles_m, tiles_n, p.vecA, p.vecB);
      });
      break;
    case GP_BF16X3:
      with_trans(transA, transB, [&](auto TA, auto TB) {
        hipLaunchKernelGGL((gemm_bf16x3_kernel<decltype(TA)::value, decltype(TB)::value>), grid, dim3(256), 0, st, M, N, K, A, lda, B, ldb, C, ldc, beta, kchunk,
                           part, tiles_m, tiles_n, p.vecA, p.vecB);
      });
      break;
  }
  if (rc) return rc;
  CTCN_LAUNCH_CHECK();
  if (splits > 1) {
    const size_t total = (size_t)M * N;
    hipLaunchKernelGGL(splitk_reduce_kernel, dim3((int)std::min((size_t)2048, ceil_div_z(total, 256))), dim3(256), 0, st, (const float *)part, C, M, N, ldc,
                       splits, beta);
    CTCN_LAUNCH_CHECK();
  }
  return CTCN_OK;
}

int ctcn_gemm_on_xcds(int transA, int transB, int M, int N, int K, const float *A, int lda, const float *B, int ldb, float *C,
                      int ldc, float beta, int precision, void *ws, size_t ws_bytes, void *stream, unsigned xcd_allow, GemmPlanes *planes) {
  return gemm_core(transA, transB, M, N, K, A, lda, B, ldb, C, ldc, beta, precision, ws, ws_bytes, stream, xcd_allow, planes, 0);
}
extern "C" int ctcn_diag_gemm_on_xcds(int transA, int transB, int M, int N, int K, const float *A, int lda, const float *B, int ldb, float *C, int ldc,
                                      float beta, int precision, void *ws, size_t ws_bytes, void *stream, unsigned xcd_allow) {
  return gemm_core(transA, transB, M, N, K, A, lda, B, ldb, C, ldc, beta, precision, ws, ws_bytes, stream, xcd_allow, nullptr, 0);
}

int ctcn_gemm_shift_b(int M, int N, int K, const float *A, int lda, const float *B, int ldb, float *C, int ldc, float beta, int precision,
                      void *ws, size_t ws_bytes, void *stream, unsigned xcd_allow, int shift, GemmPlanes *planes) {
  const int as = shift < 0 ? -shift : shift;
  CTCN_REQUIRE(as < K, "ctcn_gemm_shift_b: |shift| %d >= K %d", as, K);
  const GemmEnv e = {(int)((uintptr_t)A & 15), (int)((uintptr_t)B & 15), ws != nullptr, ws_bytes, xcd_allow, false, false, ctcn_device_cus(), 0, gemm_options()};
  const bool plane = uses_planes(plan_gemm({1, 0, M, N, K, lda, ldb, ldc, precision, shift}, e).path) &&
                     plan_gemm({1, 0, M, N, K - as, lda, ldb, ldc, precision, 0}, e).path != GP_TN;
  if (!plane) {
    if (planes) planes->same_a = false;
    const float *A2 = shift > 0 ? A + (size_t)as * lda : A, *B2 = shift < 0 ? B + (size_t)as * ldb : B;
    return gemm_core(1, 0, M, N, K - as, A2, lda, B2, ldb, C, ldc, beta, precision, ws, ws_bytes, stream, xcd_allow, planes, 0);
  }
  return gemm_core(1, 0, M, N, K, A, lda, B, ldb, C, ldc, beta, precision, ws, ws_bytes, stream, xcd_allow, planes, shift);
}

extern "C" int ctcn_gemm(int transA, int transB, int M, int N, int K, const float *A, int lda, const float *B,
                         int ldb, float *C, int ldc, float beta, int precision, void *ws, size_t ws_bytes,
                         void *stream) {
  return gemm_core(transA, transB, M, N, K, A, lda, B, ldb, C, ldc, beta, precision, ws, ws_bytes, stream, 0u, nullptr, 0);
}

constexpr double DX_WIDE_COST = 1.87;
struct DxPlan { bool eligible, wide; int tiles_wide, tiles_128; };
static DxPlan plan_dx(int M, int N, int K, int lda, int precision, int a_mod16, bool has_ws, size_t ws_bytes, int cus, int opt_wide, bool single) {
  DxPlan p = {};
  p.tiles_128 = ceil_div(M, 256) * ceil_div(N, 128);
  p.eligible = precision == 1 && !single && N % 320 == 0 && K >= 64 && K % 4 == 0 && lda % 4 == 0 && a_mod16 == 0 && has_ws &&
               ws_bytes >= plane_layout(0, N, K).bytes;
  if (!p.eligible) return p;
  p.tiles_wide = ceil_div(M, 256) * (N / 320);
  const int c = std::max(cus, 1);
  p.wide = opt_wide == 2 || (opt_wide == 1 && ceil_div(p.tiles_wide, c) * DX_WIDE_COST < (double)ceil_div(p.tiles_128, c));
  return p;
}
extern "C" int ctcn_diag_dx_plan(int M, int N, int K, int lda, int precision, int a_mod16, int has_ws, size_t ws_bytes, int cus, int *out) {
  CTCN_REQUIRE(out && M > 0 && N > 0 && K >= 0 && cus > 0 && a_mod16 >= 0 && a_mod16 < 16, "ctcn_diag_dx_plan: bad args");
  const DxPlan p = plan_dx(M, N, K, lda, precision, a_mod16, has_ws != 0, ws_bytes, cus, ctcn_get_option("gemm_dx_wide"), bf16_single());
  const int v[CTCN_DX_PLAN_INTS] = {p.eligible, p.wide, p.tiles_wide, p.tiles_128};
  memcpy(out, v, sizeof(v));
  return CTCN_OK;
}
extern "C" int ctcn_gemm_dx(int M, int N, int K, const float *A, int lda, const float *B, int ldb, float *C, int ldc, float beta, int precision, void *ws,
                            size_t ws_bytes, void *stream) {
  const GemmShape g = {0, 0, M, N, K, lda, ldb, ldc, precision, 0};
  if (const int rc = check_gemm_shape(g)) return rc;
  CTCN_REQUIRE(A && B && C, "ctcn_gemm_dx: null pointer");
  CTCN_REQUIRE(!ws || (uintptr_t)ws % 16 == 0, "ctcn_gemm_dx: the workspace must be 16-byte aligned");
  const DxPlan p = plan_dx(M, N, K, lda, precision, (int)((uintptr_t)A & 15), ws != nullptr, ws_bytes, ctcn_device_cus(), ctcn_get_option("gemm_dx_wide"),
                           bf16_single());
  if (!p.wide) return gemm_core(0, 0, M, N, K, A, lda, B, ldb, C, ldc, beta, precision, ws, ws_bytes, stream, 0u, nullptr, 0);
  hipStream_t st = (hipStream_t)stream;
  const PlaneLayout lay = plane_layout(0, N, K);
  unsigned short *bh = (unsigned short *)ws, *bl = bh + lay.b_el;
  launch_split(SP_TRANSPOSE, st, B, ldb, N, K, lay.Kp, bh, bl, 0, 0u, nullptr);
  CTCN_LAUNCH_CHECK();
  const size_t lds = (size_t)2 * (2 * 256 * 64 + 2 * 320 * 64);
  CTCN_HIP(hipFuncSetAttribute(reinterpret_cast<const void *>(gemm_af32_n320pp_kernel), hipFuncAttributeMaxDynamicSharedMemorySize, (int)lds));
  hipLaunchKernelGGL(gemm_af32_n320pp_kernel, dim3(p.tiles_wide), dim3(512), lds, st, M, N, K, lay.Kp, A, lda, (const unsigned short *)bh,
                     (const unsigned short *)bl, C, ldc, beta, ceil_div(M, 256), N / 320);
  CTCN_LAUNCH_CHECK();
  return CTCN_OK;
}

__global__ void transpose01_pair_kernel(const float *__restrict__ in0, const float *__restrict__ in1, float *__restrict__ out0, float *__restrict__ out1,
                                        int A, int B, int C) {
  const float *in = blockIdx.y ? in1 : in0;
  float *out = blockIdx.y ? out1 : out0;
  const size_t total = (size_t)A * B * C;
  for (size_t i = blockIdx.x * (size_t)blockDim.x + threadIdx.x; i < total; i += (size_t)gridDim.x * blockDim.x) {
    const int c = i % C;
    const size_t ab = i / C;
    const int a = ab % A;
    const int b = ab / A;
    out[i] = in[((size_t)a * B + b) * C + c];
  }
}
__global__ __launch_bounds__(256) void transpose2d_pair_kernel(const float *__restrict__ in0, const float *__restrict__ in1, float *__restrict__ out0,
                                                               float *__restrict__ out1, int A, int B) {
  __shared__ float tile[32][33];
  const float *in = blockIdx.z ? in1 : in0;
  float *out = blockIdx.z ? out1 : out0;
  const int tx = threadIdx.x & 31, ty = threadIdx.x >> 5;
  const int b0 = blockIdx.x * 32, a0 = blockIdx.y * 32;
#pragma unroll
  for (int k = 0; k < 4; ++k) {
    const int a = a0 + ty + 8 * k, b = b0 + tx;
    if (a < A && b < B) tile[ty + 8 * k][tx] = in[(size_t)a * B + b];
  }
  __syncthreads();
#pragma unroll
  for (int k = 0; k < 4; ++k) {
    const int b = b0 + ty + 8 * k, a = a0 + tx;
    if (a < A && b < B) out[(size_t)b * A + a] = tile[tx][ty + 8 * k];
  }
}
int ctcn_transpose01_pair(const float *in0, const float *in1, float *out0, float *out1, int A, int B, int C, void *stream) {
  CTCN_REQUIRE(in0 && in1 && out0 && out1 && A > 0 && B > 0 && C > 0, "ctcn_transpose01_pair: bad args");
  if (C == 1) {
    hipLaunchKernelGGL(transpose2d_pair_kernel, dim3(ceil_div(B, 32), ceil_div(A, 32), 2), dim3(256), 0, (hipStream_t)stream, in0, in1, out0, out1, A, B);
    CTCN_LAUNCH_CHECK();
    return CTCN_OK;
  }
  const size_t total = (size_t)A * B * C;
  const int blocks = (int)min((size_t)4096, ceil_div_z(total, 256));
  hipLaunchKernelGGL(transpose01_pair_kernel, dim3(blocks, 2), dim3(256), 0, (hipStream_t)stream, in0, in1, out0, out1, A, B, C);
  CTCN_LAUNCH_CHECK();
  return CTCN_OK;
}

extern "C" int ctcn_transpose01(const float *in, float *out, int A, int B, int C, void *stream) {
  CTCN_REQUIRE(in && out && A > 0 && B > 0 && C > 0, "ctcn_transpose01: bad args");
  const size_t total = (size_t)A * B * C;
  const int blocks = (int)min((size_t)4096, ceil_div_z(total, 256));
  hipLaunchKernelGGL(transpose01_kernel, dim3(blocks), dim3(256), 0, (hipStream_t)stream, in, out, A, B, C);
  CTCN_LAUNCH_CHECK();
  return CTCN_OK;
}
```

ctc_pytorch_amd/csrc/rnn.hip:

```cpp
#include <algorithm>
#include <stdlib.h>

#include <atomic>

#include "common.h"
#include <type_traits>

namespace {

__device__ __forceinline__ float act_sigmoid(float x) { return __builtin_amdgcn_rcpf(1.0f + __builtin_amdgcn_exp2f(-1.4426950408889634f * x)); }
__device__ __forceinline__ float act_tanh(float x) {
  const float e = __builtin_amdgcn_exp2f(-2.8853900817779268f * fabsf(x));
  return copysignf((1.0f - e) * __builtin_amdgcn_rcpf(1.0f + e), x);
}

typedef __bf16 bf16x8_t __attribute__((ext_vector_type(8)));
union Bf16Pack { u32x4 u; bf16x8_t v; };
__device__ __forceinline__ void split_bf16(float x, unsigned &hi, unsigned &lo) {
  hi = f2bf(x);
  lo = f2bf(x - __uint_as_float(hi << 16));
}
__device__ __forceinline__ void split8(const f32x4 &a, const f32x4 &b, bf16x8_t &hi, bf16x8_t &lo) {
  unsigned h[8], l[8];
#pragma unroll
// ... 2044 lines not shown
  for (int pr = 1; pr < p.nchunk / 2; ++pr) {
    if (pr > 1) pl_side.same_b = true;
    int rc = project_chunk(c, p, pr, ov.side_ws, ov.side_ws_bytes, ov.side_stream, ov.xcd_allow, pl_side);
    pl_side.same_b = true;
    if (!rc) rc = project_chunk(c, p, p.nchunk - 1 - pr, ov.side_ws, ov.side_ws_bytes, ov.side_stream, ov.xcd_allow, pl_side);
    if (rc) {
      hipLaunchKernelGGL(set_counter_kernel, dim3(1), dim3(1), 0, sd, chunk_ready, (unsigned)p.nchunk);
      return rc;
    }
    hipLaunchKernelGGL(set_counter_kernel, dim3(1), dim3(1), 0, sd, chunk_ready, (unsigned)pr);
  }
  CTCN_LAUNCH_CHECK();
  return CTCN_OK;
}

static int fwd_try_tagged(const FwdCall &c, const PipePlan &p, GemmPlanes &pl_main, bool &drop_pending, bool &launched) {
  const int H = c.H, nsl = H / 16, wpx = ceil_div(c.groups, c.nxd) * nsl;
  hipStream_t st = c.st();
  Handoff h;
  if (carve_handoff(c.ws, c.ws_bytes, align_up((size_t)2 * c.dirs * c.nbt * (H / 32) * 2048, 256), 512, h)) {
    PersistArgs pa = persist_args(c.a, h, c.status, {1, c.nxd, c.groups, nsl, c.nbt, 16, wpx});
    const bool rsv = (c.rsv_lds == 1 || (c.rsv_lds == 2 && nsl > 24)) &&
                     ((uintptr_t)c.a.gates | (uintptr_t)c.a.aux | (uintptr_t)c.a.y | (uintptr_t)(drop_pending ? c.call.y_drop : nullptr)) % 16 == 0;
    pa.poll_depth = 1; pa.rsv_lds = rsv; pa.tagmode = 1; pa.poll_delay = c.tag_poll_delay;
    pa.chunk_T = p.on ? p.chunk_T : 0; pa.nchunk = p.nchunk; pa.chunk_ready = pa.flags;
    const bool fuse_drop = drop_pending && c.fused_dropout;
    if (fuse_drop) {
      pa.ydrop = c.call.y_drop; pa.drop_p = c.call.drop_p; pa.drop_scale = 1.0f / (1.0f - c.call.drop_p);
      pa.drop_seed = c.call.drop_seed; pa.drop_off = c.call.drop_offset;
    }
    pa.slow = c.slow_items; pa.slow_x = c.slow_exchange;
    CTCN_HIP(clear_handoff(h, true, st));
    if (p.on) CTCN_HIP(hipEventRecord((hipEvent_t)c.call.side_event, st));
    launched = launch_fwd_tagged(ceil_div(H / 32, 12), xcd_local_grid(c.nxd, wpx), st, pa, wpx);
    if (launched) {
      CTCN_LAUNCH_CHECK();
      note_kernel(0, "rnn_fwd_tagged", c.call);
      if (fuse_drop) drop_pending = false;
      return p.on ? project_side_pairs(c, p, pa.chunk_ready) : CTCN_OK;
    }
  }
  if (p.on)
    for (int ch = 1; ch < p.nchunk - 1; ++ch)
      if (int rc = project_chunk(c, p, ch, c.ws, c.ws_bytes, c.stream, 0, pl_main)) return rc;
  return CTCN_OK;
}

static int fwd_try_persist(const FwdCall &c, bool &launched, const char *&why) {
  const int H = c.H;
  int kq = ceil_div(H, 64);
  if (kq == 7) kq = 8;
  struct Cand { int mode, hsu; };
  Cand cands[8];
  int nc = 0;
  if (c.cell == CTCN_CELL_TANH) {
    if (c.nxd > 1) cands[nc++] = {1, 16};
    cands[nc++] = {0, 16};
  } else {
    if (c.nxd > 1) {
      if (H % 8 == 0) cands[nc++] = {1, 8};
      cands[nc++] = {1, 12}; cands[nc++] = {1, 16}; cands[nc++] = {1, 4};
    }
    cands[nc++] = {0, H % 8 == 0 ? 8 : 4};
  }
  why = kq > 8 ? "hidden size above 512" : "no candidate geometry is co-resident on this device";
  for (int ci = 0; ci < nc && kq <= 8; ++ci) {
    const int mode = cands[ci].mode, HSU = cands[ci].hsu;
    const int nx = mode ? c.nxd : 1;
    const int NT = c.cell == CTCN_CELL_TANH ? 1 : ceil_div(HSU, 4);
    const int nsl = ceil_div(H, HSU);
    const int wpx = ceil_div(c.groups, nx) * nsl;
    const int prec = c.precision == 1 && HSU % 4 == 0 && H % 8 == 0 ? 1 : 0;
    const size_t hx_bytes = align_up((size_t)2 * c.groups * (prec ? ceil_div(H, 32) * 512 : ceil_div(H, 16) * 256) * sizeof(float), 256);
    const size_t fl_bytes = align_up((size_t)2 * c.groups * nsl * sizeof(unsigned), 256) + 256;
    Handoff h;
    if (!carve_handoff(c.ws, c.ws_bytes, hx_bytes, fl_bytes, h)) { why = "workspace too small for the hand-off tiles"; break; }
    PersistArgs pa = persist_args(c.a, h, c.status, {mode, nx, c.groups, nsl, c.nbt, HSU, wpx});
    CTCN_HIP(clear_handoff(h, prec != 0, c.st()));
    launched = launch_fwd_persist(prec, NT, kq, mode ? xcd_local_grid(nx, wpx) : dim3(nsl, c.dirs, c.nbt), 0, c.st(), pa, wpx);
    if (launched) {
      CTCN_LAUNCH_CHECK();
      note_kernel(0, "rnn_fwd_persist", c.call);
      break;
    }
  }
  return CTCN_OK;
}

static int fwd_per_timestep(FwdCall &c) {
  const int HS = c.cell == CTCN_CELL_TANH ? 16 : 4;
  const int MT = c.B <= 16 ? 1 : (c.B <= 32 ? 2 : 4);
  const dim3 grid(ceil_div(c.H, HS), c.dirs, ceil_div(c.B, 16 * MT));
  const int kq4 = pick_kq4(c.H, 4, MT, 20);
  note_kernel(0, "rnn_fwd_step", c.call);
  for (int s = 0; s < c.T; ++s) {
    c.a.step = s;
    launch_fwd(MT, kq4, grid, c.st(), c.a);
  }
  CTCN_LAUNCH_CHECK();
  return CTCN_OK;
}

static int rnn_fwd_impl(int cell, int T, int B, int I, int H, int dirs, const float *x, const float *w_ih0,
                        const float *w_hh0, const float *w_ih1, const float *w_hh1, float *y, float *gates,
                        float *aux, int precision, void *ws, size_t ws_bytes, void *stream, const ctcn_rnn_call &call, bool &drop_pending) {
  if (int rc = fwd_validate(cell, T, B, I, H, dirs, x, w_ih0, w_hh0, w_ih1, w_hh1, y, gates, aux, ws)) return rc;
  FwdCall c = {cell, T, B, I, H, dirs, precision, x, {w_ih0, w_ih1}, gates, ws, ws_bytes, stream, call};
  fwd_begin(c, w_hh0, w_hh1, y, aux);
  const PipePlan plan = decide_pipeline(c);
  if (getenv("CTCN_LOG_PIPE")) fprintf(stderr, "libctcn: rnn_fwd T=%d B=%d I=%d H=%d: projection pipeline %s (chunks %d x %d steps, fits=%d)\n", T, B, I, H, plan.on ? "ON" : "off", plan.nchunk, plan.chunk_T, (int)plan.fits);
  GemmPlanes pl_main;
  if (!c.recurrence_only)
    if (int rc = plan.on ? project_first_pair(c, plan, pl_main) : project_all(c)) return rc;
  if (c.persistent && T > 1 && !c.fits32) {
    log_fallback("ctcn_rnn_fwd", T, B, H, dirs, "a reserve tensor of 4 GB or more");
  } else if (c.persistent && T > 1) {
    bool launched = false;
    const char *why = nullptr;
    if (tagged_gather_applies(c))
      if (int rc = fwd_try_tagged(c, plan, pl_main, drop_pending, launched)) return rc;
    if (!launched)
      if (int rc = fwd_try_persist(c, launched, why)) return rc;
    if (launched) return CTCN_OK;
    log_fallback("ctcn_rnn_fwd", T, B, H, dirs, why);
  }
  return fwd_per_timestep(c);
}

extern "C" int ctcn_dropout(const float *x, float *y, size_t n, float p, uint64_t seed, uint64_t offset, void *stream);
extern "C" int ctcn_rnn_fwd_ex(int cell, int T, int B, int I, int H, int dirs, const float *x, const float *w_ih0, const float *w_hh0,
                               const float *w_ih1, const float *w_hh1, float *y, float *gates, float *aux, int precision, void *ws, size_t ws_bytes,
                               void *stream, const ctcn_rnn_call *call) {
  const ctcn_rnn_call &c = call ? *call : k_plain_call;
  CTCN_REQUIRE(!c.y_drop || (c.drop_p >= 0.0f && c.drop_p < 1.0f), "ctcn_rnn_fwd_ex: dropout p=%f outside [0,1)", (double)c.drop_p);
  bool drop_pending = c.y_drop != nullptr;
  const int rc = rnn_fwd_impl(cell, T, B, I, H, dirs, x, w_ih0, w_hh0, w_ih1, w_hh1, y, gates, aux, precision, ws, ws_bytes, stream, c, drop_pending);
  if (rc) return rc;
  return drop_pending ? ctcn_dropout(y, c.y_drop, (size_t)T * B * dirs * H, c.drop_p, c.drop_seed, c.drop_offset, stream) : CTCN_OK;
}
extern "C" int ctcn_rnn_fwd(int cell, int T, int B, int I, int H, int dirs, const float *x, const float *w_ih0,
                            const float *w_hh0, const float *w_ih1, const float *w_hh1, float *y, float *gates,
                            float *aux, int precision, void *ws, size_t ws_bytes, void *stream) {
  return ctcn_rnn_fwd_ex(cell, T, B, I, H, dirs, x, w_ih0, w_hh0, w_ih1, w_hh1, y, gates, aux, precision, ws, ws_bytes, stream, nullptr);
}
extern "C" int ctcn_rnn_fwd_dropout(int cell, int T, int B, int I, int H, int dirs, const float *x, const float *w_ih0, const float *w_hh0,
                                    const float *w_ih1, const float *w_hh1, float *y, float *gates, float *aux, float *y_drop, float p, uint64_t seed,
                                    uint64_t offset, int precision, void *ws, size_t ws_bytes, void *stream) {
  CTCN_REQUIRE(y_drop && p >= 0.0f && p < 1.0f, "ctcn_rnn_fwd_dropout: y_drop NULL or p=%f outside [0,1)", (double)p);
  ctcn_rnn_call c = {};
  c.y_drop = y_drop; c.drop_p = p; c.drop_seed = seed; c.drop_offset = offset;
  return ctcn_rnn_fwd_ex(cell, T, B, I, H, dirs, x, w_ih0, w_hh0, w_ih1, w_hh1, y, gates, aux, precision, ws, ws_bytes, stream, &c);
}

static int rnn_bwd_gemms(int cell, int T, int B, int I, int H, int dirs, const float *x, const float *w_ih0, const float *w_ih1,
                         const float *y, const float *gates, const float *aux, float *dx, float *dw_ih0, float *dw_hh0, float *dw_ih1,
                         float *dw_hh1, float beta_w, int precision, bool weights, unsigned xcd_allow, void *ws, size_t ws_bytes,
                         void *stream) {
  const int G = gates_of(cell), GH = G * H, TB = T * B;
  const float *w_ih[2] = {w_ih0, w_ih1};
  float *dw_ih[2] = {dw_ih0, dw_ih1};
  float *dw_hh[2] = {dw_hh0, dw_hh1};
  GemmPlanes pl;
  bool dx_done = false;
  if (dx && dirs == 2) {
    StackedWih s;
    if (int rc = stack_w_ih(w_ih0, w_ih1, GH, I, ws, ws_bytes, (hipStream_t)stream, s)) return rc;
    if (s.w) {
      if (int rc = xcd_allow ? ctcn_gemm_on_xcds(0, 0, TB, I, 2 * GH, gates, 2 * GH, s.w, I, dx, I, 0.0f, precision, s.ws, s.ws_bytes, stream, xcd_allow)
                             : ctcn_gemm_dx(TB, I, 2 * GH, gates, 2 * GH, s.w, I, dx, I, 0.0f, precision, s.ws, s.ws_bytes, stream)) return rc;
      dx_done = true;
    }
  }
  for (int d = 0; d < dirs; ++d) {
    const float *da = gates + (size_t)d * GH;
    const int ldg = dirs * GH;
    int rc;
    if (dx && !dx_done) {
      rc = ctcn_gemm_on_xcds(0, 0, TB, I, GH, da, ldg, w_ih[d], I, dx, I, d == 0 ? 0.0f : 1.0f, precision, ws, ws_bytes, stream, xcd_allow);
      if (rc) return rc;
    }
    if (!weights || !dw_ih[d]) continue;
    rc = ctcn_gemm_on_xcds(1, 0, GH, I, TB, da, ldg, x, I, dw_ih[d], I, beta_w, precision, ws, ws_bytes, stream, xcd_allow, &pl);
    if (rc) return rc;
    const int Kh = (T - 1) * B;
    if (Kh <= 0) {
      if (beta_w == 0.0f) CTCN_HIP(hipMemsetAsync(dw_hh[d], 0, (size_t)GH * H * sizeof(float), (hipStream_t)stream));
      continue;
    }
    const size_t offA = d == 0 ? (size_t)B : 0, offY = d == 0 ? 0 : (size_t)B;
    const float *yh = y + (size_t)d * H + offY * dirs * H;
    if (cell == CTCN_CELL_GRU) {
      rc = ctcn_gemm_on_xcds(1, 0, 2 * H, H, Kh, da + offA * ldg, ldg, yh, dirs * H, dw_hh[d], H, beta_w, precision, ws, ws_bytes, stream, xcd_allow);
      if (rc) return rc;
      const float *dn = aux + (size_t)d * H + offA * dirs * H;
      rc = ctcn_gemm_on_xcds(1, 0, H, H, Kh, dn, dirs * H, yh, dirs * H, dw_hh[d] + (size_t)2 * H * H, H, beta_w, precision, ws, ws_bytes, stream, xcd_allow);
      if (rc) return rc;
    } else {
      pl.same_a = true;
      rc = ctcn_gemm_shift_b(GH, H, TB, da, ldg, y + (size_t)d * H, dirs * H, dw_hh[d], H, beta_w, precision, ws, ws_bytes, stream, xcd_allow,
                             d == 0 ? B : -B, &pl);
      if (rc) return rc;
    }
  }
  return CTCN_OK;
}

struct BwdCall {
  int cell, T, B, I, H, dirs, precision;
  const float *dy;
  void *ws; size_t ws_bytes;
  void *stream;
  const ctcn_rnn_call &call;
  int G, GH;
  RnnArgs a;
  dim3 grid;
  int *status;
  bool fits32;
  bool dy_dropped;
  void *prelaunch_event;
  int nxd;
  bool persistent, bwd_scatter, fused_dropout;
  int handoff_tags, item_gather, poll_delay, slow_items, slow_exchange;
  hipStream_t st() const { return (hipStream_t)stream; }
};

static void record_prelaunch(BwdCall &c) {
  if (!c.prelaunch_event) return;
  (void)hipEventRecord((hipEvent_t)c.prelaunch_event, c.st());
  c.prelaunch_event = nullptr;
}

static int materialise_dropped_dy(BwdCall &c) {
  if (c.dy_dropped) return CTCN_OK;
  const ctcn_rnn_call &k = c.call;
  if (int rc = ctcn_dropout(c.dy, k.dy_tmp, (size_t)c.T * c.B * c.dirs * c.H, k.drop_p, k.drop_seed, k.drop_offset, c.stream)) return rc;
  c.a.dy = k.dy_tmp; c.dy_dropped = true;
  return CTCN_OK;
}

struct BwdPlan { int kq, nbt, nsl, groups, prec, ntw; bool gather2, scatter, feasible; size_t hx_bytes, fl_bytes; };
static BwdPlan bwd_choose_formulation(const BwdCall &c) {
  BwdPlan p;
  p.kq = ceil_div(c.GH, 256);
  if (p.kq == 7) p.kq = 8;
  p.nbt = c.grid.z; p.nsl = c.grid.x; p.groups = c.dirs * p.nbt;
  const int nsl = p.nsl;
  p.prec = c.precision == 1 && c.H % 8 == 0 ? 1 : 0;
  p.gather2 = (c.item_gather == 2 || (c.item_gather >= 1 && (nsl > 20 || !c.fits32))) && nsl <= 40 && c.handoff_tags && c.H % 4 == 0 &&
              (uintptr_t)c.dy % 16 == 0 && (uintptr_t)c.a.y % 16 == 0 && (!c.call.dy_tmp || (uintptr_t)c.call.dy_tmp % 16 == 0);
  p.scatter = c.bwd_scatter && p.prec && nsl <= (p.gather2 ? 40 : 24);
  p.ntw = nsl <= 12 ? 1 : 2;
  p.hx_bytes = p.scatter ? align_up((size_t)2 * p.groups * nsl * nsl * 1024, 256)
                         : align_up((size_t)2 * p.groups * (p.prec ? ceil_div(c.GH, 32) * 512 : ceil_div(c.GH, 16) * 256) * sizeof(float), 256);
  p.fl_bytes = align_up((size_t)2 * p.groups * nsl * (p.scatter ? nsl : 1) * sizeof(unsigned), 256) + 256;
  p.feasible = (p.kq <= 8 || p.scatter) && (c.fits32 || (p.scatter && p.gather2));
  return p;
}

static int bwd_try_persistent(BwdCall &c, const BwdPlan &p, const Handoff &h, int mode, bool &done) {
  const int nx = mode ? c.nxd : 1, nsl = p.nsl, wpx = ceil_div(p.groups, nx) * nsl;
  hipStream_t st = c.st();
  PersistArgs pa = persist_args(c.a, h, c.status, {mode, nx, p.groups, nsl, p.nbt, 16, wpx});
  const dim3 pgrid = mode ? xcd_local_grid(nx, wpx) : c.grid;
  if (!p.scatter) {
    if (int rc = materialise_dropped_dy(c)) return rc;
    pa.a.dy = c.a.dy;
    CTCN_HIP(clear_handoff(h, p.prec != 0, st));
    record_prelaunch(c);
    done = launch_bwd_persist(p.prec, p.kq, pgrid, 0, st, pa, wpx);
    if (done) note_kernel(1, "rnn_bwd_persist", c.call);
    return CTCN_OK;
  }
  pa.tagmode = c.handoff_tags;
  pa.slow = c.slow_items; pa.slow_x = c.slow_exchange;
  CTCN_HIP(clear_handoff(h, pa.tagmode != 0, st));
  if (!c.dy_dropped && c.fused_dropout) {
    pa.drop_bwd = 1; pa.drop_p = c.call.drop_p; pa.drop_scale = 1.0f / (1.0f - c.call.drop_p); pa.drop_seed = c.call.drop_seed; pa.drop_off = c.call.drop_offset;
  } else {
    if (int rc = materialise_dropped_dy(c)) return rc;
    pa.a.dy = c.a.dy;
  }
  record_prelaunch(c);
  if (p.gather2) {
    pa.poll_delay = c.poll_delay < 0 ? (nsl <= 24 ? 16 : 24) : c.poll_delay;
    done = launch_bwd_scatter2(nsl, pgrid, st, pa, wpx);
    if (done) note_kernel(1, "rnn_bwd_scatter2", c.call);
  } else {
    done = launch_bwd_scatter(p.prec, p.ntw, pgrid, st, pa, wpx);
    if (done) note_kernel(1, "rnn_bwd_scatter", c.call);
  }
  return CTCN_OK;
}

static int bwd_per_timestep(BwdCall &c) {
  if (int rc = materialise_dropped_dy(c)) return rc;
  CTCN_HIP(hipMemsetAsync(c.a.state, 0, (size_t)c.B * c.dirs * c.H * sizeof(float), c.st()));
  const int kq4 = pick_kq4(c.GH, 16, 1, 5);
  note_kernel(1, "rnn_bwd_step", c.call);
  for (int s = 0; s < c.T; ++s) {
    c.a.step = s;
    launch_bwd(kq4, c.grid, c.st(), c.a);
  }
  return CTCN_OK;
}

extern "C" int ctcn_rnn_bwd_ex(int cell, int T, int B, int I, int H, int dirs, const float *x, const float *w_ih0,
                               const float *w_hh0, const float *w_ih1, const float *w_hh1, const float *y,
                               float *gates, float *aux, const float *dy, float *dx, float *dw_ih0, float *dw_hh0,
                               float *dw_ih1, float *dw_hh1, float beta_w, int precision, void *scratch, void *ws,
                               size_t ws_bytes, void *stream, const ctcn_rnn_call *call_p) {
  const ctcn_rnn_call &call = call_p ? *call_p : k_plain_call;
  CTCN_REQUIRE(!call.dy_tmp || (call.drop_p >= 0.0f && call.drop_p < 1.0f), "ctcn_rnn_bwd_ex: dropout p=%f outside [0,1)", (double)call.drop_p);
  CTCN_REQUIRE(cell >= 0 && cell <= 2, "ctcn_rnn_bwd: unknown cell %d", cell);
  CTCN_REQUIRE(T > 0 && B > 0 && I > 0 && H > 0 && (dirs == 1 || dirs == 2), "ctcn_rnn_bwd: bad dims");
  if (H % 4 != 0) { ctcn_set_error("ctcn_rnn_bwd: hidden size %d must be a multiple of 4", H); return CTCN_EUNSUPPORTED; }
  CTCN_REQUIRE(x && w_ih0 && w_hh0 && y && gates && dy && scratch, "ctcn_rnn_bwd: null pointer");
  CTCN_REQUIRE((dw_ih0 != nullptr) == (dw_hh0 != nullptr), "ctcn_rnn_bwd: dw_ih0 / dw_hh0 must both be given or both be NULL (weights deferred to ctcn_rnn_bwd_weights)");
  CTCN_REQUIRE(dirs == 1 || (w_ih1 && w_hh1 && (!dw_ih0 || (dw_ih1 && dw_hh1))), "ctcn_rnn_bwd: null pointer (reverse direction)");
  CTCN_REQUIRE(cell == CTCN_CELL_TANH || aux, "ctcn_rnn_bwd: aux reserve required for LSTM/GRU");
  CTCN_REQUIRE((uintptr_t)gates % 16 == 0 && (uintptr_t)scratch % 16 == 0 && (cell == CTCN_CELL_TANH || (uintptr_t)aux % 16 == 0),
               "ctcn_rnn_bwd: gates / aux / scratch must be 16-byte aligned");
  CTCN_REQUIRE((uintptr_t)ws % 16 == 0, "ctcn_rnn_bwd: the workspace must be 16-byte aligned (hand-off tiles)");
  BwdCall c = {cell, T, B, I, H, dirs, precision, dy, ws, ws_bytes, stream, call};
  c.G = gates_of(cell); c.GH = c.G * H;
  const int GH = c.GH;
  c.grid = dim3(ceil_div(H, 16), dirs, ceil_div(B, 16));
  c.status = call.status ? call.status : ctcn_status_word();
  c.fits32 = (size_t)T * B * dirs * GH * sizeof(float) < ((size_t)1 << 32);
  c.dy_dropped = call.dy_tmp == nullptr;
  c.prelaunch_event = call.prelaunch_event;
  c.nxd = ctcn_opt_handoff() ? ctcn_device_xcds() : 1;
  c.persistent = ctcn_opt_rnn_persistent() != 0; c.bwd_scatter = ctcn_opt_bwd_scatter() != 0; c.fused_dropout = ctcn_get_option("rnn_fused_dropout") != 0;
  c.handoff_tags = ctcn_opt_handoff_tags(); c.item_gather = ctcn_get_option("bwd_item_gather");
  c.poll_delay = ctcn_get_option("bwd_poll_delay"); c.slow_items = ctcn_get_option("rnn_slow_items"); c.slow_exchange = ctcn_get_option("rnn_slow_exchange");
// ... 66 lines not shown
```

ctc_pytorch_amd/ops.py:

```python
import collections
import ctypes
import os
import numpy as np

import torch

from . import _lib

CELL = {"lstm": 0, "gru": 1, "tanh": 2}
GATES = {0: 4, 1: 3, 2: 1}

def _precision_from_env():
    v = os.environ.get("CTCN_PRECISION", "1").strip()
    if v not in ("0", "1"):
        raise ValueError("CTCN_PRECISION must be 0 (exact f32 MFMA) or 1 (bf16x3 split-operand MFMA), got %r" % v)
    return int(v)


DEFAULT_PRECISION = _precision_from_env()
_precision = [DEFAULT_PRECISION]


def set_precision(p):
    if int(p) not in (0, 1):
# ... 81 lines not shown
    for n, v in snap["options"].items():
        if get_option(n) != v:
            set_option(n, v)
    set_precision(snap["precision"])
    _chunks_on[0], _fuse_bn_dropout[0] = snap["chunks_on"], snap["fuse_bn_dropout"]
    for k, v in snap["side"].items():
        _side[k] = v
    if not snap["grad_ready_hook"]:
        parallel.enable_overlap(False)
    if not snap["sync_bn"]:
        _sync_bn["reduce"] = None
    parallel._batch["global"], parallel._batch["local"] = snap["batch_split"]
    parallel._overlap["works"], parallel._overlap["done"], parallel._overlap["events"] = [], [], []


_kernel_counts = {}
_debug_note = [None]


def kernel_counts(reset=False):
    out = dict(_kernel_counts)
    if reset:
        _kernel_counts.clear()
    return out


def _count_kernel(name):
    k = (name or b"?").decode() if isinstance(name, (bytes, bytearray)) or name is None else str(name)
    _kernel_counts[k] = _kernel_counts.get(k, 0) + 1


def rnn_last_kernels():
    L = _lib.lib()
    return (L.ctcn_rnn_last_kernel(0) or b"").decode(), (L.ctcn_rnn_last_kernel(1) or b"").decode()


def diag_squat(wgs_per_xcd, usec, threads=256, lds_bytes=0, stream=None):
    st = stream.cuda_stream if stream is not None else _lib.stream_ptr()
    _lib.check(_lib.lib().ctcn_diag_squat(int(wgs_per_xcd), int(threads), int(lds_bytes), int(usec), ctypes.c_void_p(st)), "diag_squat")


def check_health(device=None):
    _lib.check_status(torch.device("cuda", torch.cuda.current_device()) if device is None else device)


def _ws(t, tag="main"):
    _lib.status_word(t.device)
    w = _lib.workspace(t.device, tag=tag)
    return w, ctypes.c_void_p(w.data_ptr()), w.numel()


_grad_ready = {"hook": None}


_XCD_ORDERS = ((0, 1, 2, 3, 4, 5, 6, 7), (0, 2, 4, 6, 1, 3, 5, 7), (0, 1, 4, 5, 2, 3, 6, 7), (0, 3, 4, 7, 1, 2, 5, 6), (0, 2, 5, 7, 1, 3, 4, 6), (0, 4, 1, 5, 2, 6, 3, 7))


def _idle_xcd_mask(nx, groups):
    if nx == 8:
        order = _XCD_ORDERS[min(max(get_option("xcd_interleave"), 0), 5)]
        return sum(1 << order[g] for g in range(min(groups, nx), nx))
    return ((1 << nx) - 1) & ~((1 << groups) - 1)


def set_grad_ready_hook(fn):
    _grad_ready["hook"] = fn


def _env_on(name):
    return os.environ.get(name, "1") != "0"


SIDE_MIN_ITEMS_FWD, SIDE_MIN_ITEMS_BWD = 1 << 21, 1 << 18
SMALL_SPLIT_MAX_ITEMS = 1 << 23
_side = {"fwd_overlap": _env_on("CTCN_FWD_OVERLAP"), "enabled": _env_on("CTCN_SIDE_STREAM"),
         "min_items": int(os.environ.get("CTCN_SIDE_MIN_ITEMS", SIDE_MIN_ITEMS_FWD)),
         "min_items_bwd": int(os.environ.get("CTCN_SIDE_MIN_ITEMS_BWD", os.environ.get("CTCN_SIDE_MIN_ITEMS", SIDE_MIN_ITEMS_BWD))),
         "small_split": _env_on("CTCN_SMALL_SPLIT"),
         "capacity_slack": float(os.environ.get("CTCN_SIDE_CAPACITY_SLACK", "1.0"))}


def set_side_stream(flag, min_items=None, min_items_bwd=None):
    _side["enabled"] = bool(flag)
    if min_items is not None:
        _side["min_items"] = int(min_items)
        _side["min_items_bwd"] = int(min_items)
    if min_items_bwd is not None:
        _side["min_items_bwd"] = int(min_items_bwd)


def set_fwd_overlap(flag):
    _side["fwd_overlap"] = bool(flag)


def _tiles16(n):
    return (n + 15) // 16


def _recurrence_xcds(B, dirs, nx):
    groups = dirs * _tiles16(B)
    return groups, (_idle_xcd_mask(nx, groups) if nx > 1 else 0)


def side_stream_plan(cell, T, B, I, H, dirs, nx, cus, slack=1.0):
    if nx <= 1:
        return 0
    groups, idle = _recurrence_xcds(B, dirs, nx)
    per = cus // nx
    wpx = ((groups + nx - 1) // nx) * _tiles16(H)
    used = wpx + max(2, wpx // 8)
    if groups < nx:
        if used + 2 > per:
            return 0
        share, allow = (nx - groups) / float(nx), idle
    else:
        if per - used < 8:
            return 0
        share, allow = (per - used) / float(per), (1 << nx) - 1
    side_us = 2.0 * T * B * (dirs * GATES[cell] * H) * (I + H) / (300e6 * share)
    return allow if side_us <= 0.9 * T * (1.2 + H / 400.0) * slack else 0


def side_stream_fits(cell, T, B, I, H, dirs, nx, cus, slack=1.0):
    return side_stream_plan(cell, T, B, I, H, dirs, nx, cus, slack) != 0


def plan_fwd_pipeline(T, B, H, dirs, nx, settings=None):
    s = _side if settings is None else settings
    idle = _recurrence_xcds(B, dirs, nx)[1]
    return idle if s["enabled"] and s["fwd_overlap"] and dirs == 2 and T * B * H >= s["min_items"] else 0


WG_INLINE = "inline"
WG_DEFERRED = "deferred side"
WG_SPLIT_END = "split, joined at end of backward"
WG_SPLIT_NOW = "split, joined at once"


def plan_weight_grads(cell, T, B, I, H, dirs, nx, cus, into_flat, chunk, bottom, above_parked, settings=None):
    s = _side if settings is None else settings
    items = T * B * H
    if chunk or not (into_flat and s["enabled"] and T > 1):
        return WG_INLINE, 0
    allow = side_stream_plan(cell, T, B, I, H, dirs, nx, cus, s["capacity_slack"]) if nx > 1 and items >= s["min_items_bwd"] else 0
    if allow and not bottom:
        return WG_DEFERRED, allow
    if allow and dirs == 2:
        return WG_SPLIT_END, 0
    if s["small_split"] and dirs == 2 and not above_parked and items < SMALL_SPLIT_MAX_ITEMS:
        return WG_SPLIT_NOW, 0
    return WG_INLINE, 0


class _DeviceSide(object):

    def __init__(self, dev):
        self.dev, self.stream, self.event, self.pending, self.deferred, self.live = dev, None, None, False, None, 0

    def side_stream(self):
        if self.stream is None:
            self.stream = torch.cuda.Stream(device=self.dev)
        return self.stream

    def prelaunch_event(self):
        if self.event is None:
            self.event = torch.cuda.Event()
            self.event.record(torch.cuda.current_stream(self.dev))
        return self.event

    def join(self):
        fn, self.deferred = self.deferred, None
        if fn is not None:
            fn()
        if self.pending:
            self.pending = False
            torch.cuda.current_stream(self.dev).wait_stream(self.stream)

    def join_at_end(self):
        self.join()
        self.live = 0


_devices = {}


def _device_side(dev):
    key = (dev.type, dev.index)
    d = _devices.get(key)
    if d is None:
        d = _devices[key] = _DeviceSide(dev)
    return d


def join_side_stream(device=None):
    for d in (list(_devices.values()) if device is None else [_device_side(device)]):
        d.join()


def _copy_strided(src):
    _need_gpu(src)
    if src.dim() > 4:
        raise NotImplementedError("ctc_pytorch_amd.contiguous: rank %d > 4" % src.dim())
    dims = [1] * (4 - src.dim()) + list(src.shape)
    strides = [0] * (4 - src.dim()) + list(src.stride())
    out = torch.empty(src.shape, dtype=torch.float32, device=src.device)
    if out.numel():
        _lib.check(_lib.lib().ctcn_copy_strided4(_ptr(src), _ptr(out), dims[0], dims[1], dims[2], dims[3], strides[0],
                                                 strides[1], strides[2], strides[3], _lib.stream_ptr()), "copy_strided4")
    return out


class _Contiguous(torch.autograd.Function):
    @staticmethod
    def forward(ctx, x):
        return _copy_strided(x)

    @staticmethod
    def backward(ctx, g):
        return g


def contiguous(x):
    if x.is_contiguous():
        return x
    if x.dtype != torch.float32:
        raise TypeError("ctc_pytorch_amd.contiguous: float32 only")
    return _Contiguous.apply(x)


class _BctfToTbcf(torch.autograd.Function):

    @staticmethod
    def forward(ctx, x):
        _need_gpu(x)
        x = _f32c(x)
        B, C, T, Fq = x.shape
        ctx.shape = (B, C, T, Fq)
        out = torch.empty((T, B, C * Fq), dtype=torch.float32, device=x.device)
        _lib.check(_lib.lib().ctcn_bctf_to_tbcf(_ptr(x), _ptr(out), B, C, T, Fq, _lib.stream_ptr()), "bctf_to_tbcf")
        return out

    @staticmethod
    def backward(ctx, g):
        B, C, T, Fq = ctx.shape
        g = _f32c(g)
        out = torch.empty((B, C, T, Fq), dtype=torch.float32, device=g.device)
        _lib.check(_lib.lib().ctcn_tbcf_to_bctf(_ptr(g), _ptr(out), B, C, T, Fq, _lib.stream_ptr()), "tbcf_to_bctf")
        return out


def bctf_to_tbcf(x):
    return _BctfToTbcf.apply(x)


def gemm(transA, transB, M, N, K, A, lda, Bm, ldb, C, ldc, beta=0.0, xcd_allow=0):
    _need_gpu(A, Bm, C)
    w, wp, wn = _ws(C)
    args = (int(transA), int(transB), M, N, K, _ptr(A), lda, _ptr(Bm), ldb, _ptr(C), ldc, float(beta), get_precision(), wp, wn, _lib.stream_ptr())
    _lib.check(_lib.lib().ctcn_diag_gemm_on_xcds(*args, int(xcd_allow)) if xcd_allow else _lib.lib().ctcn_gemm(*args), "gemm")
    return C


def gemm_dx(M, N, K, A, lda, Bm, ldb, C, ldc, beta=0.0):
    _need_gpu(A, Bm, C)
    w, wp, wn = _ws(C)
    _lib.check(_lib.lib().ctcn_gemm_dx(M, N, K, _ptr(A), lda, _ptr(Bm), ldb, _ptr(C), ldc, float(beta), get_precision(), wp, wn, _lib.stream_ptr()),
               "gemm_dx")
    return C


class _Linear(torch.autograd.Function):

    @staticmethod
    def forward(ctx, x, w):
        _need_gpu(x, w)
        ctx.gw_view = _gview(w)
        x, w = _f32c(x), _f32c(w)
        M, K = x.shape
        N = w.shape[0]
        y = torch.empty((M, N), dtype=torch.float32, device=x.device)
        gemm(0, 1, M, N, K, x, K, w, K, y, N)
        ctx.save_for_backward(x, w)
        return y

    @staticmethod
    def backward(ctx, gy):
        x, w = ctx.saved_tensors
        gy = _f32c(gy)
        M, K = x.shape
        N = w.shape[0]
        gx = gw = None
        if ctx.needs_input_grad[0]:
            gx = torch.empty((M, K), dtype=torch.float32, device=x.device)
            gemm(0, 0, M, K, N, gy, N, w, K, gx, K)
        if ctx.needs_input_grad[1]:
            if ctx.gw_view is not None:
                gemm(1, 0, N, K, M, gy, N, x, K, ctx.gw_view, K, beta=1.0)
            else:
                gw = torch.empty((N, K), dtype=torch.float32, device=x.device)
                gemm(1, 0, N, K, M, gy, N, x, K, gw, K)
        return gx, gw


def linear(x2d, w):
    return _Linear.apply(x2d, w)


_Saved = collections.namedtuple("_Saved", "x y gates aux w_ih0 w_hh0 w_ih1 w_hh1")


def _new_rnn_call(dev):
    call, launched = _lib.RnnCall(), ctypes.c_char_p(None)
    call.status = _lib.status_word(dev).data_ptr()
    call.launched = ctypes.pointer(launched)
    return call, launched


def _note_launch(launched, step_kernel, cell, T, B, H, dirs):
    _count_kernel(launched)
    if T > 1 and B > 16 and (launched or b"") == step_kernel and get_option("rnn_persistent"):
        _fallback_shapes.add((cell, H, dirs, B))


def _note_rnn_fwd(I, s, y_drop, w):
    adr = lambda t: t.data_ptr() if t is not None else 0
    _debug_note[0]("rnn_fwd", dict(I=int(I), x=adr(s.x), gates=adr(s.gates), aux=adr(s.aux), y=adr(s.y), y_drop=adr(y_drop), ws=adr(w), w_ih=adr(s.w_ih0), w_hh=adr(s.w_hh0)),
                   dict(x=s.x, y=s.y, gates=s.gates, aux=s.aux, y_drop=y_drop, w_ih=(s.w_ih0, s.w_ih1)))


def _weight_grads(cell, dims, s, dws, prec, xcd_allow=0, side=None):
    w, wp, wn = _ws(s.x, tag="main" if side is None else "side")
    _lib.check(_lib.lib().ctcn_rnn_bwd_weights(cell, *dims, _ptr(s.x), _ptr(s.y), _ptr(s.gates), _ptr(s.aux), *[_ptr(d) for d in dws],
                                               1.0, prec, xcd_allow, wp, wn, _lib.stream_ptr()), "rnn_bwd_weights")
    if side is not None:
        for t in (s.x, s.y, s.gates, s.aux):
            if t is not None:
                t.record_stream(side)


class _RNNLayer(torch.autograd.Function):
    @staticmethod
    def forward(ctx, x, w_ih0, w_hh0, w_ih1, w_hh1, cell, training, drop_p=0.0):
        _need_gpu(x, w_ih0, w_hh0, w_ih1, w_hh1)
        ctx.gviews = [_gview(w) for w in (w_ih0, w_hh0, w_ih1, w_hh1)]
        x = _f32c(x)
        ws = [_f32c(w) if w is not None else None for w in (w_ih0, w_hh0, w_ih1, w_hh1)]
        for k in (1, 3):
            if ws[k] is not None and ws[k].data_ptr() % 16:
                ws[k] = ws[k].clone()
        T, B, I = x.shape
        G = GATES[cell]
        H = ws[1].shape[1]
        dirs = 2 if ws[2] is not None else 1
        dev = x.device
        y = torch.empty((T, B, dirs * H), dtype=torch.float32, device=dev)
        gates = torch.empty((T, B, dirs, G * H), dtype=torch.float32, device=dev)
        aux = torch.empty((T, B, dirs, H), dtype=torch.float32, device=dev) if cell != 2 else None
        s = _Saved(x, y, gates, aux, *ws)
        w, wp, wn = _ws(x)
        L = _lib.lib()
        side = _device_side(dev)
        call, launched = _new_rnn_call(dev)
        piped = plan_fwd_pipeline(T, B, H, dirs, L.ctcn_device_xcds())
        if piped:
            st = side.side_stream()
            w2, wp2, wn2 = _ws(x, tag="side")
            call.side_stream, call.side_event, call.side_ws, call.side_ws_bytes, call.xcd_allow = st.cuda_stream, side.prelaunch_event().cuda_event, w2.data_ptr(), wn2, piped
        ctx.drop = None
        y_drop = None
        if training and drop_p > 0.0:
            y_drop = torch.empty_like(y)
            seed, off = _next_dropout_stream(y.numel())
            ctx.drop = (float(drop_p), seed, off)
            call.y_drop, call.drop_p, call.drop_seed, call.drop_offset = y_drop.data_ptr(), float(drop_p), seed, off
        _lib.check(L.ctcn_rnn_fwd_ex(cell, T, B, I, H, dirs, _ptr(x), _ptr(ws[0]), _ptr(ws[1]), _ptr(ws[2]), _ptr(ws[3]),
                                     _ptr(y), _ptr(gates), _ptr(aux), get_precision(), wp, wn, _lib.stream_ptr(), ctypes.byref(call)), "rnn_fwd_ex")
        _note_launch(launched.value, b"rnn_fwd_step", cell, T, B, H, dirs)
        if _debug_note[0] is not None:
            _note_rnn_fwd(I, s, y_drop, w)
        if piped:
            torch.cuda.current_stream(dev).wait_stream(st)
            for t in (x, gates, ws[0], ws[2]):
                if t is not None:
                    t.record_stream(st)
        ctx.cell, ctx.dims = cell, (T, B, I, H, dirs)
        ctx.early_ok = not _chunking[0]
        ctx.consumed = False
        ctx.counted = any(ctx.needs_input_grad)
        if ctx.counted:
            side.live += 1
        ctx.save_for_backward(*s)
        return y if y_drop is None else y_drop

    @staticmethod
    def backward(ctx, gy):
        if ctx.consumed:
            raise RuntimeError("ctc_pytorch_amd RNN layer: backward ran twice (the gate reserve is overwritten in place)")
        ctx.consumed = True
        dims = T, B, I, H, dirs = ctx.dims
        cell = ctx.cell
        s = _Saved(*ctx.saved_tensors)
        wts = (s.w_ih0, s.w_hh0, s.w_ih1, s.w_hh1)
        gy = _f32c(gy)
        dev = s.x.device
        dx = torch.empty_like(s.x) if ctx.needs_input_grad[0] else None
        into_flat = all(g is not None for g, w in zip(ctx.gviews, wts) if w is not None)
        dws = [None if w is None else (g if into_flat else torch.empty_like(w)) for g, w in zip(ctx.gviews, wts)]
        L = _lib.lib()
        scratch = torch.empty(L.ctcn_rnn_scratch_bytes(cell, B, H, dirs), dtype=torch.uint8, device=dev)
        w, wp, wn = _ws(s.x)
        side = _device_side(dev)
        if ctx.counted:
            side.live = max(0, side.live - 1)
        mode, allow = plan_weight_grads(cell, T, B, I, H, dirs, L.ctcn_device_xcds(), L.ctcn_device_cus(), into_flat=into_flat, chunk=not ctx.early_ok,
                                        bottom=dx is None or side.live == 0, above_parked=side.deferred is not None)
        above, side.deferred, ev = side.deferred, None, None
        call, launched = _new_rnn_call(dev)
        if above is not None:
            ev = side.prelaunch_event()
            call.prelaunch_event = ev.cuda_event
        gd = None
        if ctx.drop is not None:
            p_, seed_, off_ = ctx.drop
            gd = torch.empty_like(gy)
            call.dy_tmp, call.drop_p, call.drop_seed, call.drop_offset = gd.data_ptr(), p_, seed_, off_
        prec = get_precision()
        try:
            _lib.check(L.ctcn_rnn_bwd_ex(cell, T, B, I, H, dirs, _ptr(s.x), *[_ptr(t) for t in wts], _ptr(s.y), _ptr(s.gates), _ptr(s.aux), _ptr(gy), _ptr(dx),
                                         *[_ptr(d) if mode == WG_INLINE else None for d in dws],
                                         1.0 if into_flat else 0.0, prec, _ptr(scratch), wp, wn, _lib.stream_ptr(), ctypes.byref(call)), "rnn_bwd_ex")
        except Exception:
            side.deferred = above
            raise
        _note_launch(launched.value, b"rnn_bwd_step", cell, T, B, H, dirs)
        if above is not None:
            above(ev)
        if mode in (WG_SPLIT_END, WG_SPLIT_NOW):
            st, main = side.side_stream(), torch.cuda.current_stream(dev)
            st.wait_stream(main)
            with torch.cuda.stream(st):
                _weight_grads(cell, dims, s, [None, None] + dws[2:], prec, side=st)
            _weight_grads(cell, dims, s, dws[:2] + [None, None], prec)
            if mode == WG_SPLIT_NOW:
                main.wait_stream(st)
            else:
                side.pending = True
                torch.autograd.Variable._execution_engine.queue_callback(side.join_at_end)
        elif mode == WG_DEFERRED:
            st = side.side_stream()

            def weights_on_side_stream(after=None):
                if after is None:
                    st.wait_stream(torch.cuda.current_stream(dev))
                else:
                    st.wait_event(after)
                with torch.cuda.stream(st):
                    _weight_grads(cell, dims, s, dws, prec, allow, side=st)
                    if _grad_ready["hook"] is not None:
                        _grad_ready["hook"]([t for t in dws if t is not None])
                side.pending = True

            side.deferred = weights_on_side_stream
            torch.autograd.Variable._execution_engine.queue_callback(side.join_at_end)
        return (dx,) + ((None,) * 7 if into_flat else tuple(dws) + (None,) * 3)


def persistent_batch_limit(H, dirs, nx, cus):
    nsl = _tiles16(H)
    per_xcd = (cus // max(nx, 1)) // nsl if nsl else 0
    return 16 * ((per_xcd * max(nx, 1)) // dirs) if nx > 1 else 0


def rnn_layer(x, w_ih0, w_hh0, w_ih1, w_hh1, cell, training=True, drop_p=0.0):
    cellc = CELL[cell] if isinstance(cell, str) else cell
    T, B = int(x.shape[0]), int(x.shape[1])
    H, dirs = int(w_hh0.shape[1]), 2 if w_ih1 is not None else 1
    if x.is_cuda and T > 1 and _chunks_on[0] and (cellc, H, dirs, B) in _fallback_shapes and get_option("rnn_persistent"):
        L = _lib.lib()
        bmax = persistent_batch_limit(H, dirs, L.ctcn_device_xcds(), L.ctcn_device_cus())
        if 0 < bmax < B:
            _chunking[0] = True
            try:
                ys = [_RNNLayer.apply(xc, w_ih0, w_hh0, w_ih1, w_hh1, cellc, training, 0.0) for xc in x.split(bmax, dim=1)]
            finally:
                _chunking[0] = False
            return dropout(torch.cat(ys, dim=1), float(drop_p), training)
    return _RNNLayer.apply(x, w_ih0, w_hh0, w_ih1, w_hh1, cellc, training, float(drop_p))


_chunks_on = [os.environ.get("CTCN_BATCH_CHUNKS", "1") != "0"]
_chunking = [False]
_fallback_shapes = set()


def set_batch_chunks(flag):
    _chunks_on[0] = bool(flag)


def mark_batch_chunks(cell, H, dirs, B):
    _fallback_shapes.add((CELL[cell] if isinstance(cell, str) else int(cell), int(H), int(dirs), int(B)))


_sync_bn = {"reduce": None}


def set_sync_bn(reducer):
    _sync_bn["reduce"] = reducer


class _BatchNorm(torch.autograd.Function):
    @staticmethod
    def forward(ctx, x, gamma, beta, rm, rv, outer, C, inner, training, momentum, eps, relu, nbt=None, drop_p=0.0):
        _need_gpu(x, gamma, beta)
        ctx.gviews = (_gview(gamma), _gview(beta))
        x = _f32c(x)
        dev = x.device
        y = torch.empty_like(x)
        L = _lib.lib()
        ctx.sync = None
        ctx.drop = None
        if training and drop_p > 0.0:
            mean = torch.empty(C, dtype=torch.float32, device=dev)
            rstd = torch.empty(C, dtype=torch.float32, device=dev)
            seed, off = _next_dropout_stream(x.numel())
            w, wp, wn = _ws(x)
            _lib.check(L.ctcn_bn_fwd_train_dropout(_ptr(x), _ptr(y), _ptr(gamma), _ptr(beta), _ptr(rm), _ptr(rv), _ptr(mean), _ptr(rstd),
                                                   outer, C, inner, float(eps), float(momentum), int(relu), wp, wn, _lib.stream_ptr(), _ptr(nbt),
                                                   float(drop_p), seed, off), "bn_fwd_train_dropout")
            ctx.save_for_backward(x, None, gamma, mean, rstd, beta)
            ctx.train_mode = True
            ctx.drop = (float(drop_p), seed, off)
            ctx.geom = (outer, C, inner, relu, eps)
            return y
        if training and _sync_bn["reduce"] is not None:
            mean = torch.empty(C, dtype=torch.float32, device=dev)
            rstd = torch.empty(C, dtype=torch.float32, device=dev)
            sums = torch.empty((C, 2), dtype=torch.float64, device=dev)
            w, wp, wn = _ws(x)
            _lib.check(L.ctcn_bn_fwd_sums(_ptr(x), _ptr(sums), outer, C, inner, wp, wn, _lib.stream_ptr()), "bn_fwd_sums")
            total = float(_sync_bn["reduce"](sums, outer * inner))
            _lib.check(L.ctcn_bn_fwd_finish(_ptr(x), _ptr(y), _ptr(gamma), _ptr(beta), _ptr(rm), _ptr(rv), _ptr(mean), _ptr(rstd),
                                            _ptr(sums), total, outer, C, inner, float(eps), float(momentum), int(relu),
                                            _lib.stream_ptr(), _ptr(nbt)), "bn_fwd_finish")
            ctx.save_for_backward(x, y if relu else None, gamma, mean, rstd)
            ctx.train_mode = True
            ctx.sync = (_sync_bn["reduce"], total)
        elif training:
            mean = torch.empty(C, dtype=torch.float32, device=dev)
            rstd = torch.empty(C, dtype=torch.float32, device=dev)
            w, wp, wn = _ws(x)
            _lib.check(L.ctcn_bn_fwd_train(_ptr(x), _ptr(y), _ptr(gamma), _ptr(beta), _ptr(rm), _ptr(rv), _ptr(mean), _ptr(rstd),
                                           outer, C, inner, float(eps), float(momentum), int(relu), wp, wn, _lib.stream_ptr(), _ptr(nbt)),
                       "bn_fwd_train")
            ctx.save_for_backward(x, y if relu else None, gamma, mean, rstd)
            ctx.train_mode = True
        else:
            _lib.check(L.ctcn_bn_fwd_eval(_ptr(x), _ptr(y), _ptr(gamma), _ptr(beta), _ptr(rm), _ptr(rv), outer, C, inner, float(eps),
                                          int(relu), _lib.stream_ptr()), "bn_fwd_eval")
            ctx.save_for_backward(x, y if relu else None, gamma, rm, rv)
            ctx.train_mode = False
        ctx.geom = (outer, C, inner, relu, eps)
        return y

    @staticmethod
    def backward(ctx, gy):
        outer, C, inner, relu, eps = ctx.geom
        if ctx.drop is not None:
            x, _, gamma, a, b, beta = ctx.saved_tensors
            gy = _f32c(gy)
            dx = torch.empty_like(x)
            into_flat = ctx.gviews[0] is not None and ctx.gviews[1] is not None
            dgamma, dbeta = ctx.gviews if into_flat else (torch.empty(C, dtype=torch.float32, device=x.device), torch.empty(C, dtype=torch.float32, device=x.device))
            w, wp, wn = _ws(x)
            p_, seed_, off_ = ctx.drop
            _lib.check(_lib.lib().ctcn_bn_bwd_dropout(_ptr(x), _ptr(gy), _ptr(gamma), _ptr(beta), _ptr(a), _ptr(b), _ptr(dx), _ptr(dgamma), _ptr(dbeta),
                                                      outer, C, inner, int(relu), 1.0 if into_flat else 0.0, wp, wn, _lib.stream_ptr(), p_, seed_, off_),
                       "bn_bwd_dropout")
            if into_flat:
                dgamma = dbeta = None
            return dx, dgamma, dbeta, None, None, None, None, None, None, None, None, None, None, None
        x, y, gamma, a, b = ctx.saved_tensors
        gy = _f32c(gy)
        dev = x.device
        if not ctx.train_mode:
            raise NotImplementedError("ctc_pytorch_amd: backward through eval-mode BatchNorm is not part of the hot path")
        dx = torch.empty_like(x)
        into_flat = ctx.gviews[0] is not None and ctx.gviews[1] is not None
        if into_flat:
            dgamma, dbeta = ctx.gviews
        else:
# ... 1498 lines not shown
```

include/ctcn.h:

```cpp
#ifndef CTCN_H
#define CTCN_H
#include <stddef.h>
#include <stdint.h>
#ifdef __cplusplus
extern "C" {
#endif

#define CTCN_OK 0
#define CTCN_EINVAL (-1)
#define CTCN_EHIP (-2)
#define CTCN_EUNSUPPORTED (-3)
#define CTCN_EWORKSPACE (-4)

#define CTCN_REDUCTION_NONE 0
#define CTCN_REDUCTION_MEAN 1
#define CTCN_REDUCTION_SUM 2

#define CTCN_CELL_LSTM 0
#define CTCN_CELL_GRU 1
#define CTCN_CELL_TANH 2

int ctcn_version(void);
const char *ctcn_last_error(void);
int ctcn_device_cus(void);
int ctcn_device_xcds(void);
int ctcn_set_option(const char *name, int value);
int ctcn_get_option(const char *name);
const char *ctcn_option_name(int index);
int ctcn_set_status_buffer(int *dev_word);

int ctcn_gemm(int transA, int transB, int M, int N, int K, const float *A, int lda, const float *B, int ldb,
              float *C, int ldc, float beta, int precision, void *ws, size_t ws_bytes, void *stream);

int ctcn_gemm_dx(int M, int N, int K, const float *A, int lda, const float *B, int ldb, float *C, int ldc, float beta, int precision, void *ws,
                 size_t ws_bytes, void *stream);

int ctcn_transpose01(const float *in, float *out, int A, int B, int C, void *stream);
int ctcn_copy_strided4(const float *in, float *out, int d0, int d1, int d2, int d3, size_t s0, size_t s1, size_t s2,
                       size_t s3, void *stream);
int ctcn_relu_fwd(const float *x, float *y, size_t n, void *stream);
int ctcn_relu_bwd(const float *y, const float *dy, float *dx, size_t n, void *stream);
int ctcn_maxpool2d_fwd(const float *x, float *y, unsigned char *arg, size_t planes, int Hi, int Wi, int kh, int kw, void *stream);
int ctcn_maxpool2d_bwd(const float *dy, const unsigned char *arg, float *dx, size_t planes, int Hi, int Wi, int kh, int kw, void *stream);

size_t ctcn_rnn_scratch_bytes(int cell, int B, int H, int dirs);
int ctcn_rnn_fwd(int cell, int T, int B, int I, int H, int dirs, const float *x, const float *w_ih0,
                 const float *w_hh0, const float *w_ih1, const float *w_hh1, float *y, float *gates, float *aux,
                 int precision, void *ws, size_t ws_bytes, void *stream);
int ctcn_rnn_fwd_dropout(int cell, int T, int B, int I, int H, int dirs, const float *x, const float *w_ih0, const float *w_hh0,
                         const float *w_ih1, const float *w_hh1, float *y, float *gates, float *aux, float *y_drop, float p, uint64_t seed,
                         uint64_t offset, int precision, void *ws, size_t ws_bytes, void *stream);
int ctcn_rnn_bwd(int cell, int T, int B, int I, int H, int dirs, const float *x, const float *w_ih0,
                 const float *w_hh0, const float *w_ih1, const float *w_hh1, const float *y, float *gates,
                 float *aux, const float *dy, float *dx, float *dw_ih0, float *dw_hh0, float *dw_ih1,
                 float *dw_hh1, float beta_w, int precision, void *scratch, void *ws, size_t ws_bytes,
                 void *stream);
int ctcn_rnn_bwd_dropout(int cell, int T, int B, int I, int H, int dirs, const float *x, const float *w_ih0, const float *w_hh0,
                         const float *w_ih1, const float *w_hh1, const float *y, float *gates, float *aux, const float *dy, float *dx,
                         float *dw_ih0, float *dw_hh0, float *dw_ih1, float *dw_hh1, float beta_w, int precision, void *scratch, void *ws,
                         size_t ws_bytes, void *stream, float p, uint64_t seed, uint64_t offset, float *dy_tmp);
typedef struct ctcn_rnn_call {
  float drop_p;
  uint64_t drop_seed, drop_offset;
  float *y_drop;
  float *dy_tmp;
  void *side_stream, *side_event, *side_ws;
  size_t side_ws_bytes;
  unsigned xcd_allow;
  void *prelaunch_event;
  int *status;
  const char **launched;
} ctcn_rnn_call;
int ctcn_rnn_fwd_ex(int cell, int T, int B, int I, int H, int dirs, const float *x, const float *w_ih0, const float *w_hh0,
                    const float *w_ih1, const float *w_hh1, float *y, float *gates, float *aux, int precision, void *ws, size_t ws_bytes,
                    void *stream, const ctcn_rnn_call *call);
int ctcn_rnn_bwd_ex(int cell, int T, int B, int I, int H, int dirs, const float *x, const float *w_ih0, const float *w_hh0,
                    const float *w_ih1, const float *w_hh1, const float *y, float *gates, float *aux, const float *dy, float *dx,
                    float *dw_ih0, float *dw_hh0, float *dw_ih1, float *dw_hh1, float beta_w, int precision, void *scratch, void *ws,
                    size_t ws_bytes, void *stream, const ctcn_rnn_call *call);
int ctcn_rnn_bwd_weights(int cell, int T, int B, int I, int H, int dirs, const float *x, const float *y,
                         const float *gates, const float *aux, float *dw_ih0, float *dw_hh0, float *dw_ih1,
                         float *dw_hh1, float beta_w, int precision, unsigned xcd_allow, void *ws, size_t ws_bytes,
                         void *stream);

size_t ctcn_bn_ws_bytes(int outer, int C, int inner);
int ctcn_bn_fwd_train(const float *x, float *y, const float *gamma, const float *beta, float *running_mean,
                      float *running_var, float *save_mean, float *save_rstd, int outer, int C, int inner,
                      float eps, float momentum, int relu, void *ws, size_t ws_bytes, void *stream,
                      long long *num_batches_tracked );
int ctcn_bn_fwd_sums(const float *x, double *sums, int outer, int C, int inner, void *ws, size_t ws_bytes, void *stream);
int ctcn_bn_fwd_finish(const float *x, float *y, const float *gamma, const float *beta, float *running_mean,
                       float *running_var, float *save_mean, float *save_rstd, const double *sums, double count_total,
                       int outer, int C, int inner, float eps, float momentum, int relu, void *stream,
                       long long *num_batches_tracked );
int ctcn_bn_bwd_sums(const float *x, const float *y, const float *dy, const float *save_mean, const float *save_rstd,
                     double *sums, int outer, int C, int inner, int relu, void *ws, size_t ws_bytes, void *stream);
int ctcn_bn_bwd_finish(const float *x, const float *y, const float *dy, const float *gamma, const float *save_mean,
                       const float *save_rstd, float *dx, float *dgamma, float *dbeta, const double *local_sums,
                       const double *global_sums, double count_total, int outer, int C, int inner, int relu,
                       float beta_acc, void *ws, size_t ws_bytes, void *stream);
int ctcn_bn_fwd_eval(const float *x, float *y, const float *gamma, const float *beta, const float *running_mean,
                     const float *running_var, int outer, int C, int inner, float eps, int relu, void *stream);
int ctcn_bn_bwd(const float *x, const float *y, const float *dy, const float *gamma, const float *save_mean,
                const float *save_rstd, float *dx, float *dgamma, float *dbeta, int outer, int C, int inner,
                int relu, float beta_acc, void *ws, size_t ws_bytes, void *stream);
int ctcn_bn_fwd_train_dropout(const float *x, float *y_drop, const float *gamma, const float *beta, float *running_mean, float *running_var,
                              float *save_mean, float *save_rstd, int outer, int C, int inner, float eps, float momentum, int relu, void *ws,
                              size_t ws_bytes, void *stream, long long *num_batches_tracked, float p, uint64_t seed, uint64_t offset);
int ctcn_bn_bwd_dropout(const float *x, const float *dy_drop, const float *gamma, const float *beta, const float *save_mean, const float *save_rstd,
                        float *dx, float *dgamma, float *dbeta, int outer, int C, int inner, int relu, float beta_acc, void *ws, size_t ws_bytes,
                        void *stream, float p, uint64_t seed, uint64_t offset);

size_t ctcn_bn_masked_ws_bytes(int outer, int C, int inner);
int ctcn_mask_frames(const float *x, float *y, const int *lens, int batch, int frame, int outer, int C, int inner, void *stream);
int ctcn_bn_fwd_train_masked(const float *x, float *y, const float *gamma, const float *beta, float *running_mean, float *running_var,
                             float *save_mean, float *save_rstd, const int *lens, int batch, int frame, int outer, int C, int inner,
                             float eps, float momentum, int relu, void *ws, size_t ws_bytes, void *stream, long long *num_batches_tracked);
int ctcn_bn_fwd_eval_masked(const float *x, float *y, const float *gamma, const float *beta, const float *running_mean,
                            const float *running_var, const int *lens, int batch, int frame, int outer, int C, int inner, float eps,
                            int relu, void *stream);
int ctcn_bn_bwd_masked(const float *x, const float *y, const float *dy, const float *gamma, const float *save_mean, const float *save_rstd,
                       float *dx, float *dgamma, float *dbeta, const int *lens, int batch, int frame, int outer, int C, int inner, int relu,
                       float beta_acc, void *ws, size_t ws_bytes, void *stream);

int ctcn_dropout(const float *x, float *y, size_t n, float p, uint64_t seed, uint64_t offset, void *stream);

size_t ctcn_conv2d_ws_bytes(int B, int Ci, int Hi, int Wi, int Co, int kh, int kw, int sh, int sw, int ph, int pw);
int ctcn_conv2d_fwd(const float *x, const float *w, const float *bias, float *y, int B, int Ci, int Hi, int Wi,
                    int Co, int kh, int kw, int sh, int sw, int ph, int pw, void *stream);
int ctcn_conv2d_bwd(const float *x, const float *w, const float *dy, float *dx , float *dw,
                    float *dbias, int B, int Ci, int Hi, int Wi, int Co, int kh, int kw, int sh, int sw, int ph,
                    int pw, float beta_acc, void *ws, size_t ws_bytes, void *stream);
int ctcn_bctf_to_tbcf(const float *in, float *out, int B, int C, int T, int F, void *stream);
int ctcn_tbcf_to_bctf(const float *in, float *out, int B, int C, int T, int F, void *stream);

int ctcn_log_softmax_fwd(const float *logits, float *lp, int32_t *argmax, int rows, int V, void *stream);
int ctcn_log_softmax_bwd(const float *lp, const float *dlp, float *dlogits, int rows, int V, void *stream);
int ctcn_argmax(const float *lp, int32_t *argmax, int rows, int V, void *stream);

int ctcn_ctc_fwd(const float *lp, const int64_t *targets, const int64_t *in_len, const int64_t *tgt_len,
                 float *alpha, float *nll, int T, int B, int V, int Lmax, void *stream);
int ctcn_ctc_bwd(const float *lp, const int64_t *targets, const int64_t *in_len, const int64_t *tgt_len,
                 float *alpha, const float *nll, const float *gscale, float *grad_lp, int T, int B, int V,
                 int Lmax, void *stream);
int ctcn_ctc_fwd_both(const float *lp, const int64_t *targets, const int64_t *in_len, const int64_t *tgt_len,
                      float *alpha, float *beta, float *nll, int T, int B, int V, int Lmax, void *stream);
int ctcn_ctc_grad(const float *lp, const int64_t *targets, const int64_t *in_len, const int64_t *tgt_len,
                  const float *alpha, const float *beta, const float *nll, const float *gscale, float *grad_lp,
                  int T, int B, int V, int Lmax, void *stream);
int ctcn_sum_f32(const float *x, float *out, int n, void *stream);
int ctcn_ctc_fwd_ex(const float *lp, const int64_t *targets, const int64_t *in_len, const int64_t *tgt_len, float *alpha,
                    float *beta, float *nll, int T, int B, int V, int Lmax, int blank, void *stream);
int ctcn_ctc_grad_ex(const float *lp, const int64_t *targets, const int64_t *in_len, const int64_t *tgt_len, const float *alpha,
                     const float *beta, const float *nll, const float *gscale, int gscale_stride, int reduction, int zero_infinity,
                     int blank, float *grad_lp, int T, int B, int V, int Lmax, void *stream);
int ctcn_ctc_reduce(const float *nll, const int64_t *tgt_len, float *out, int B, int reduction, int zero_infinity, void *stream);
int ctcn_ctc_pack_targets(const int64_t *flat, int64_t n_flat, const int64_t *tgt_len, int64_t *padded, int B, int Lmax, void *stream);
size_t ctcn_ctc_align_ws_bytes(int T, int B, int Lmax);
int ctcn_ctc_align(const float *lp, const int64_t *targets, const int64_t *in_len, const int64_t *tgt_len, int32_t *paths,
                   float *frame_scores, float *score, int32_t *ok, int32_t *starts, int32_t *ends, int T, int B, int V, int Lmax,
                   int blank, void *ws, size_t ws_bytes, void *stream);

int ctcn_adam_step(float *p, const float *g, float *m, float *v, size_t n, float lr, float beta1, float beta2,
                   float eps, float weight_decay, int step, void *stream);

#define CTCN_NORM_L2 2
#define CTCN_NORM_INF 0
typedef struct ctcn_clip_ctl {
  float total_norm;
  int32_t nonfinite;
  float clip_coef;
  int32_t apply;
  int32_t step;
  int32_t skipped;
  float step_size;
  float sqrt_bc2;
} ctcn_clip_ctl;
size_t ctcn_grad_norm_ws_bytes(size_t n, int nseg);
int ctcn_grad_norm(const float *g, size_t n, int norm_type, const int64_t *seg_offsets, int nseg, float *seg_norms, float *total_norm,
                   int32_t *nonfinite, int grid_blocks, void *ws, size_t ws_bytes, void *stream);
int ctcn_clip_control(ctcn_clip_ctl *ctl, float max_norm, float lr, float beta1, float beta2, int skip_nonfinite, void *stream);
int ctcn_adam_step_ex(float *p, const float *g, float *m, float *v, size_t n, float beta1, float beta2, float eps, float weight_decay,
                      const ctcn_clip_ctl *ctl, void *stream);
int ctcn_scale_by_device_scalar(float *x, size_t n, const float *scalar, void *stream);

int ctcn_comm_unique_id(void *id128);
int ctcn_comm_init(const void *id128, int rank, int world, void **comm);
int ctcn_comm_allreduce_sum_f32(void *comm, float *buf, size_t n, void *stream);
int ctcn_comm_destroy(void *comm);

int ctcn_greedy_collapse(const int32_t *idx, size_t stride_t, size_t stride_b, const int32_t *lens, int32_t *out_ids,
                         int32_t *out_len, int T, int B, int blank, void *stream);

int ctcn_path_tokens(const int32_t *path, size_t stride_t, size_t stride_b, const float *lp, const int32_t *lens, int32_t *out_ids,
                     int32_t *out_len, int32_t *starts, int32_t *ends, float *tok_mean, float *tok_min, float *tok_margin,
                     float *path_score, int T, int B, int V, int blank, void *stream);

int ctcn_edit_distance(const int32_t *a, const int32_t *a_len, const int64_t *b, const int64_t *b_len, int32_t *out, int B,
                       int lda, int ldb, int max_b_len, void *stream);
size_t ctcn_edit_ops_ws_bytes(int B, int lda, int max_b_len);
int ctcn_edit_ops(const int32_t *a, const int32_t *a_len, const int64_t *b, const int64_t *b_len, const int32_t *map, int V,
                  int32_t *counts, int32_t *ali, int32_t *ali_len, long long *conf, int B, int lda, int ldb, int max_b_len, void *ws,
                  size_t ws_bytes, void *stream);
int ctcn_step_stats(const float *loss, const int32_t *dist, const int64_t *tgt_len, int B, const int32_t *status, double *out4, void *stream);

typedef struct ctcn_fbank_opts {
  float samp_freq, frame_shift_ms, frame_length_ms, preemph_coeff, blackman_coeff, low_freq, high_freq, energy_floor;
  int32_t window_type, num_mel_bins, remove_dc_offset, round_to_power_of_two, snip_edges, use_energy, raw_energy, htk_compat, use_log_fbank,
      use_power;
} ctcn_fbank_opts;
int ctcn_fbank_frames(long long num_samples, int frame_length, int frame_shift, int snip_edges);
size_t ctcn_fbank_plan_bytes(const ctcn_fbank_opts *opts);
int ctcn_fbank_plan(const ctcn_fbank_opts *opts, void *plan, size_t plan_bytes);
int ctcn_fbank(const void *wave, int wave_is_int16, const int32_t *lens, const ctcn_fbank_opts *opts, const void *plan, const float *mean,
               const float *scale, float *feats, int32_t *frames, int B, int Nmax, int Tmax, float dither, uint64_t seed, uint64_t utt_offset,
               void *stream);
size_t ctcn_cmvn_accumulate_ws_bytes(int B, int Tmax, int F);
int ctcn_cmvn_accumulate(const float *feats, const int32_t *frames, double *stats, int B, int Tmax, int F, void *ws, size_t ws_bytes,
                         void *stream);
typedef struct ctcn_mfcc_opts {
  float samp_freq, frame_shift_ms, frame_length_ms, preemph_coeff, blackman_coeff, low_freq, high_freq, energy_floor, cepstral_lifter;
  int32_t window_type, num_mel_bins, num_ceps, remove_dc_offset, round_to_power_of_two, snip_edges, use_energy, raw_energy, htk_compat;
} ctcn_mfcc_opts;
size_t ctcn_mfcc_plan_bytes(const ctcn_mfcc_opts *opts);
int ctcn_mfcc_plan(const ctcn_mfcc_opts *opts, void *plan, size_t plan_bytes);
int ctcn_mfcc(const void *wave, int wave_is_int16, const int32_t *lens, const ctcn_mfcc_opts *opts, const void *plan, const float *mean,
              const float *scale, float *feats, int32_t *frames, int B, int Nmax, int Tmax, float dither, uint64_t seed, uint64_t utt_offset,
              void *stream);
typedef struct ctcn_spectrogram_opts {
  float samp_freq, frame_shift_ms, frame_length_ms, preemph_coeff, blackman_coeff, energy_floor;
  int32_t window_type, remove_dc_offset, round_to_power_of_two, snip_edges, raw_energy, return_raw_fft;
} ctcn_spectrogram_opts;
size_t ctcn_spectrogram_plan_bytes(const ctcn_spectrogram_opts *opts);
int ctcn_spectrogram_plan(const ctcn_spectrogram_opts *opts, void *plan, size_t plan_bytes);
int ctcn_spectrogram(const void *wave, int wave_is_int16, const int32_t *lens, const ctcn_spectrogram_opts *opts, const void *plan,
                     const float *mean, const float *scale, float *feats, int32_t *frames, int B, int Nmax, int Tmax, float dither, uint64_t seed,
                     uint64_t utt_offset, void *stream);
typedef struct ctcn_logspec_opts {
  double sample_rate, window_size, window_stride;
  float input_scale;
  int32_t window, normalize;
} ctcn_logspec_opts;
int ctcn_logspec_frames(long long num_samples, int hop);
size_t ctcn_logspec_plan_bytes(const ctcn_logspec_opts *opts);
int ctcn_logspec_plan(const ctcn_logspec_opts *opts, void *plan, size_t plan_bytes);
size_t ctcn_logspec_ws_bytes(const ctcn_logspec_opts *opts, int B, int Tmax);
int ctcn_logspec(const void *wave, int wave_is_int16, const int32_t *lens, const ctcn_logspec_opts *opts, const void *plan, float *feats,
                 int32_t *frames, float *stats, int B, int Nmax, int Tmax, void *ws, size_t ws_bytes, void *stream);
int ctcn_fbank_power_host(const double *frame, int n, double *power);
typedef struct ctcn_resample_opts {
  double cutoff;
  int32_t orig_freq, new_freq, num_zeros;
} ctcn_resample_opts;
int ctcn_resample_samples(long long num_samples, int orig_freq, int new_freq);
size_t ctcn_resample_plan_bytes(const ctcn_resample_opts *opts);
int ctcn_resample_plan(const ctcn_resample_opts *opts, void *plan, size_t plan_bytes);
int ctcn_resample(const void *wave, int wave_is_int16, const int32_t *lens, const ctcn_resample_opts *opts, const void *plan, float *out, int B,
                  int Nmax, int Mmax, void *stream);
int ctcn_resample_host(const void *wave, int wave_is_int16, int num_samples, const ctcn_resample_opts *opts, const void *plan, float *out,
                       int out_cap);
typedef struct ctcn_context_opts {
  int32_t left, right, skip, n_downsample, delta_order, delta_window;
} ctcn_context_opts;
int ctcn_context_frames(int num_frames, int skip, int n_downsample);
int ctcn_delta_scales(int order, int window, float *scales);
int ctcn_frame_context_tile(const ctcn_context_opts *opts, int F);
int ctcn_frame_context(const float *feats, const int32_t *frames, const ctcn_context_opts *opts, float *out, int32_t *out_frames,
                       float *fractions, int B, int Tin_max, int F, int Tout_max, void *stream);
int ctcn_frame_context_host(const float *feats, int num_frames, int F, const ctcn_context_opts *opts, float *out, int out_rows,
                            float *fraction);
typedef struct ctcn_specaug_opts {
  int32_t warp_window, num_freq_masks, freq_width, num_time_masks, time_width;
  float time_ratio, fill;
} ctcn_specaug_opts;
int ctcn_spec_augment(const float *feats, const int32_t *frames, const ctcn_specaug_opts *opts, uint64_t seed, uint64_t utt_offset, float *out,
                      int B, int Tmax, int F, void *stream);
int ctcn_spec_augment_plan(const ctcn_specaug_opts *opts, uint64_t seed, uint64_t utt_index, int T, int F, int32_t *warp, int32_t *freq,
                           int32_t *time);
int ctcn_spec_augment_host(const float *feats, int T, int F, const ctcn_specaug_opts *opts, uint64_t seed, uint64_t utt_index, float *out);
typedef struct ctcn_reverb_opts {
  float rir_prob, noise_prob;
  int32_t normalize;
} ctcn_reverb_opts;
int ctcn_reverb_limits(int32_t *out);
size_t ctcn_reverb_bank_bytes(int R, int rir_stride, int N, int noise_stride, int num_snrs);
int ctcn_reverb_bank(const float *rirs, const int32_t *rir_len, int R, int rir_stride, const float *noises, const int32_t *noise_len, int N,
                     int noise_stride, const double *snrs, int num_snrs, double sample_frequency, void *bank, size_t bank_bytes);
int ctcn_reverb_plan(const void *bank, const ctcn_reverb_opts *opts, uint64_t seed, uint64_t utt_index, int32_t *draws);
size_t ctcn_reverb_ws_bytes(const void *bank_host, int B, int Nmax);
int ctcn_reverb(const void *wave, int wave_is_int16, const int32_t *lens, const void *bank_host, const void *bank_dev,
                const ctcn_reverb_opts *opts, uint64_t seed, uint64_t utt_offset, float *out, int B, int Nmax, void *ws, size_t ws_bytes,
                void *stream);
int ctcn_reverb_host(const void *wave, int wave_is_int16, int num_samples, const void *bank, const ctcn_reverb_opts *opts, uint64_t seed,
                     uint64_t utt_index, float *out);
typedef struct ctcn_sliding_cmn_opts {
  int32_t cmn_window, min_cmn_window, normalize_variance, center;
} ctcn_sliding_cmn_opts;
int ctcn_cmvn_accumulate_groups(const float *feats, const int32_t *frames, const int32_t *group, double *stats, int B, int Tmax, int F, int G,
                                void *ws, size_t ws_bytes, void *stream);
int ctcn_cmvn_apply(const float *feats, const int32_t *frames, const int32_t *group, const double *stats, float *out, int B, int Tmax, int F,
                    int G, int norm_vars, void *stream);
int ctcn_cmvn_sliding(const float *feats, const int32_t *frames, float *out, int B, int Tmax, int F, const ctcn_sliding_cmn_opts *opts,
                      void *stream);
int ctcn_cmvn_sliding_run(const ctcn_sliding_cmn_opts *opts);
int ctcn_cmvn_sliding_window(int t, int n, const ctcn_sliding_cmn_opts *opts, int32_t *start, int32_t *end);
int ctcn_cmvn_sliding_host(const float *feats, int num_frames, int F, const ctcn_sliding_cmn_opts *opts, float *out);
int ctcn_cmvn_norm_host(const double *stats, int F, int norm_vars, float *mean, float *scale);

size_t ctcn_beam_ws_bytes(int T, int B, int V, int W);
int ctcn_beam_decode(const float *x, int input_is_prob, const int32_t *lens, const double *lm, double alpha,
                     int W, int blank, int32_t *out_ids, int32_t *out_len, double *out_score, int32_t *status,
                     int T, int B, int V, void *ws, size_t ws_bytes, void *stream);
int ctcn_beam_decode_nbest(const float *x, int input_is_prob, const int32_t *lens, const double *lm, double alpha,
                           int W, int blank, int nbest, int32_t *out_ids, int32_t *out_len, double *out_score,
                           int32_t *out_count, int32_t *status, int T, int B, int V, void *ws, size_t ws_bytes, void *stream);

int ctcn_diag_squat(int wgs_per_xcd, int threads, int lds_bytes, unsigned usec, void *stream);
int ctcn_diag_pipeline_chunks(int cell, int T, int B, int I, int H, int dirs, int xcds, int cus, unsigned xcd_allow);
#define CTCN_GEMM_PLAN_INTS 12
int ctcn_diag_gemm_plan(int transA, int transB, int M, int N, int K, int lda, int ldb, int ldc, int precision, int b_shift, int a_mod16,
                        int b_mod16, int has_ws, size_t ws_bytes, unsigned xcd_allow, int same_a, int same_b, int cus, int xcds, int *out);
int ctcn_diag_gemm_on_xcds(int transA, int transB, int M, int N, int K, const float *A, int lda, const float *B, int ldb, float *C, int ldc,
                           float beta, int precision, void *ws, size_t ws_bytes, void *stream, unsigned xcd_allow);
#define CTCN_DX_PLAN_INTS 4
int ctcn_diag_dx_plan(int M, int N, int K, int lda, int precision, int a_mod16, int has_ws, size_t ws_bytes, int cus, int *out);
#define CTCN_BEAM_PLAN_INTS 19
int ctcn_diag_beam_plan(int T, int B, int V, int W, int lds_max, int generic_static_lds, int *out);
#define CTCN_CTC_LATTICE_PLAN_INTS 6
int ctcn_diag_ctc_lattice_plan(int Lmax, int *out);
const char *ctcn_rnn_last_kernel(int which);

long long ctcn_join_tokens(const int32_t *ids, long long row_stride, const int32_t *lens, int B, const char *words, const int32_t *word_off,
                           const int32_t *word_len, int V, int sep, char *out, long long out_cap, long long *out_off);
long long ctcn_levenshtein(const int32_t *a, long long na, const int32_t *b, long long nb);
long long ctcn_levenshtein_ops(const int32_t *hyp, long long nh, const int32_t *ref, long long nr, long long *counts4, int32_t *ali);

#ifdef __cplusplus
}
#endif
#endif
```

Measured before the change: 1.992 million frames/s.

## Group RNN weight-gradient TN GEMMs into one persistent work-queue launch

Adds a grouped TN GEMM kernel that packs several weight-gradient products (dW_ih and dW_hh for both directions) into a single persistent launch with an atomic tile queue and a grouped split-K reduce. The per-item GEMM body is moved into a shared include so the single and grouped kernels use the same code. In the BiLSTM backward pass, when the weight-gradient mode is split and dirs==2, the Python side now computes these products inline on the main stream instead of on a side stream. The goal is fewer launches and fuller use of the CUs across small GEMMs, at the cost of giving up overlap with the side stream and adding a queue in the workspace.

```diff
diff --git a/ctc_pytorch_amd/_lib.py b/ctc_pytorch_amd/_lib.py
--- a/ctc_pytorch_amd/_lib.py
+++ b/ctc_pytorch_amd/_lib.py
@@ -139,6 +139,10 @@
     "ctcn_diag_pipeline_chunks": (I, [I, I, I, I, I, I, I, I, ctypes.c_uint]),
     "ctcn_diag_gemm_plan": (I, [I] * 13 + [Z, ctypes.c_uint, I, I, I, I, P]),
     "ctcn_diag_dx_plan": (I, [I, I, I, I, I, I, I, Z, I, P]),
+    "ctcn_gemm_tn_group": (I, [I, P, I, P, Z, P, ctypes.c_uint]),
+    "ctcn_diag_tn_group_plan": (I, [I, P, I, I, Z, I, I, ctypes.c_uint, P]),
+    "ctcn_diag_tn_group_launches": (I, [P]),
+    "ctcn_diag_rnn_weights_grouped": (I, [I, I, I, I, I, I, I, Z, I, I, ctypes.c_uint]),
     "ctcn_diag_beam_plan": (I, [I, I, I, I, I, I, P]),
     "ctcn_diag_ctc_lattice_plan": (I, [I, P]),
     "ctcn_diag_gemm_on_xcds": (I, [I, I, I, I, I, P, I, P, I, P, I, F, I, P, Z, P, ctypes.c_uint]),
@@ -157,6 +161,11 @@
                 ("dy_tmp", ctypes.c_void_p), ("side_stream", ctypes.c_void_p), ("side_event", ctypes.c_void_p), ("side_ws", ctypes.c_void_p),
                 ("side_ws_bytes", ctypes.c_size_t), ("xcd_allow", ctypes.c_uint), ("prelaunch_event", ctypes.c_void_p), ("status", ctypes.c_void_p),
                 ("launched", ctypes.POINTER(ctypes.c_char_p))]
+
+
+class TnProduct(ctypes.Structure):
+    _fields_ = [("M", ctypes.c_int), ("N", ctypes.c_int), ("K", ctypes.c_int), ("A", ctypes.c_void_p), ("lda", ctypes.c_int), ("B", ctypes.c_void_p),
+                ("ldb", ctypes.c_int), ("C", ctypes.c_void_p), ("ldc", ctypes.c_int), ("beta", ctypes.c_float)]
 
 
 class FbankOpts(ctypes.Structure):
diff --git a/ctc_pytorch_amd/csrc/common.h b/ctc_pytorch_amd/csrc/common.h
--- a/ctc_pytorch_amd/csrc/common.h
+++ b/ctc_pytorch_amd/csrc/common.h
@@ -20,6 +20,8 @@
                       int ldc, float beta, int precision, void *ws, size_t ws_bytes, void *stream, unsigned xcd_allow, GemmPlanes *planes = nullptr);
 int ctcn_gemm_shift_b(int M, int N, int K, const float *A, int lda, const float *B, int ldb, float *C, int ldc, float beta, int precision,
                       void *ws, size_t ws_bytes, void *stream, unsigned xcd_allow, int shift, GemmPlanes *planes = nullptr);
+int ctcn_gemm_tn_group_try(int n, const ctcn_tn_product *p, int precision, void *ws, size_t ws_bytes, void *stream, unsigned xcd_allow, bool *taken);
+bool ctcn_tn_group_applies(int n, const ctcn_tn_product *p, int precision, bool has_ws, size_t ws_bytes, unsigned xcd_allow, int cus, int xcds);
 int ctcn_opt_handoff(void);
 int ctcn_opt_poll_depth(void);
 int ctcn_opt_bwd_scatter(void);
diff --git a/ctc_pytorch_amd/csrc/core.hip b/ctc_pytorch_amd/csrc/core.hip
--- a/ctc_pytorch_amd/csrc/core.hip
+++ b/ctc_pytorch_amd/csrc/core.hip
@@ -43,6 +43,7 @@
 static int g_opt_conv_dbg = 0;
 static int g_opt_gemm_bf16_single = 0;
 static int g_opt_gemm_dx_wide = 1;
+static int g_opt_gemm_tn_group = 1;
 static int g_opt_xcd_interleave = 1;
 static int g_opt_bn_rows4 = 1;
 static int g_opt_tn_splits_force = 0;
@@ -77,6 +78,7 @@
   {"tn_splits_force", &g_opt_tn_splits_force, [](int value) -> int { return value < 0 ? 0 : value; }},
   {"gemm_bf16_single", &g_opt_gemm_bf16_single, [](int value) -> int { return value ? 1 : 0; }},
   {"gemm_dx_wide", &g_opt_gemm_dx_wide, [](int value) -> int { return value < 0 ? 0 : (value > 2 ? 2 : value); }},
+  {"gemm_tn_group", &g_opt_gemm_tn_group, [](int value) -> int { return value < 0 ? 0 : (value > 2 ? 2 : value); }},
   {"beam_generic_threads", &g_opt_beam_generic_threads, [](int value) -> int { return (value == 256 || value == 512 || value == 1024) ? value : 0; }},
   {"beam_cand_global", &g_opt_beam_cand_global, [](int value) -> int { return value ? 1 : 0; }},
   {"beam_bitonic", &g_opt_beam_bitonic, [](int value) -> int { return value ? 1 : 0; }},
diff --git a/ctc_pytorch_amd/csrc/gemm.hip b/ctc_pytorch_amd/csrc/gemm.hip
--- a/ctc_pytorch_amd/csrc/gemm.hip
+++ b/ctc_pytorch_amd/csrc/gemm.hip
@@ -1,4 +1,5 @@
 #include <algorithm>
+#include <atomic>
 #include <type_traits>
 
 #include "common.h"
@@ -1266,191 +1267,63 @@
     __syncthreads();
     const int item = __builtin_amdgcn_readfirstlane(s_item);
     if (item >= nt * splits) return;
-    const int z = item / nt, tile = item - z * nt;
-    const int tm = tile / tiles_n, tn = tile - tm * tiles_n;
-    const int m0 = tm * TBM, n0 = tn * TBN;
-    const int kbeg = z * kchunk, kend = min(K, kbeg + kchunk);
-    const int nst = (kend - kbeg + 31) / 32;
-
-    f32x16 acc[4][WNT];
-#pragma unroll
-    for (int i = 0; i < 4; ++i)
-#pragma unroll
-      for (int j = 0; j < WNT; ++j)
-#pragma unroll
-        for (int e = 0; e < 16; ++e) acc[i][j][e] = 0.0f;
-
-    const int acol = m0 + 32 * wave + c4, bcol = n0 + 32 * bsub + c4;
-    const bool a_ok = acol < M, b_ok = bcol < N;
-    u32x4 pw[4 + NB];
-    const unsigned voff_a = a_ok ? (unsigned)((krow * lda + acol) * 4) : 0xfffffff0u;
-    const unsigned voff_b = b_ok ? (unsigned)((krow * ldb + bcol) * 4) : 0xfffffff0u;
-    auto load_piece = [&](int q, int k0) {
-      const int kr = q < 4 ? k0 + 8 * q : k0 + bk0 + 8 * (q - 4);
-      const int ld = q < 4 ? lda : ldb;
-      const float *base = (q < 4 ? A : B) + (size_t)min(kr, K - 1) * ld;
-      int rows = min(8, kend - kr);
-      asm volatile("" : "+s"(rows));
-      const int nrec = max(0, rows) * ld * 4;
-      const __amdgpu_buffer_rsrc_t rs = __builtin_amdgcn_make_buffer_rsrc(const_cast<float *>(base), 0, nrec, 0x00020000);
-      pw[q] = __builtin_amdgcn_raw_buffer_load_b128(rs, q < 4 ? voff_a : voff_b, 0, 0);
-    };
-    auto split_pair = [](float a, float b, unsigned &hw, unsigned &lw) {
-      typedef __bf16 bf16x2_t __attribute__((ext_vector_type(2)));
-      typedef float f32x2_t __attribute__((ext_vector_type(2)));
-      hw = __builtin_bit_cast(unsigned, __builtin_convertvector((f32x2_t){a, b}, bf16x2_t));
-      const f32x2_t r = {a - __uint_as_float(hw << 16), b - __uint_as_float(hw & 0xffff0000u)};
-      lw = __builtin_bit_cast(unsigned, __builtin_convertvector(r, bf16x2_t));
-    };
-    auto convert_piece = [&](int q) {
-      unsigned h01, l01, h23, l23;
-      if constexpr (NP == 3) {
-        split_pair(__uint_as_float(pw[q][0]), __uint_as_float(pw[q][1]), h01, l01);
-        split_pair(__uint_as_float(pw[q][2]), __uint_as_float(pw[q][3]), h23, l23);
-      } else {
-        typedef __bf16 bf16x2_t __attribute__((ext_vector_type(2)));
-        typedef float f32x2_t __attribute__((ext_vector_type(2)));
-        h01 = __builtin_bit_cast(unsigned, __builtin_convertvector((f32x2_t){__uint_as_float(pw[q][0]), __uint_as_float(pw[q][1])}, bf16x2_t));
-        h23 = __builtin_bit_cast(unsigned, __builtin_convertvector((f32x2_t){__uint_as_float(pw[q][2]), __uint_as_float(pw[q][3])}, bf16x2_t));
-        l01 = l23 = 0u;
-      }
-      pw[q] = (u32x4){h01, h23, l01, l23};
-    };
-    auto store_ab = [&](int buf) {
-      unsigned char *sb = qsm + buf * STAGE;
-#pragma unroll
-      for (int q = 0; q < 4 + NB; ++q) {
-        unsigned char *p = sb + (q < 4 ? st_a + q * 512 : st_b + (q - 4) * 512);
-        *reinterpret_cast<uint2 *>(p) = make_uint2(pw[q][0], pw[q][1]);
-        if constexpr (NP == 3) *reinterpret_cast<uint2 *>(p + (q < 4 ? A_BYTES : B_BYTES)) = make_uint2(pw[q][2], pw[q][3]);
-      }
-    };
-    bf16x8_t ah[4], al[4], bh[WNT], bl[WNT];
-    auto tr_frag = [&](const unsigned char *p) {
-      const s16x4_t x0 = __builtin_amdgcn_ds_read_tr16_b64_v4i16((lds4_t)(p));
-      const s16x4_t x1 = __builtin_amdgcn_ds_read_tr16_b64_v4i16((lds4_t)(p + 256));
-      return __builtin_bit_cast(bf16x8_t, __builtin_shufflevector(x0, x1, 0, 1, 2, 3, 4, 5, 6, 7));
-    };
-    auto load_frags = [&](int stage, int ks) {
-      const unsigned char *sb = qsm + (stage & 1) * STAGE + ks * 1024 + troff;
-#pragma unroll
-      for (int j = 0; j < WNT; ++j) {
-        const unsigned char *p = sb + 2 * A_BYTES + (wn * WNT + j) * 2048;
-        bh[j] = tr_frag(p);
-        if constexpr (NP == 3) bl[j] = tr_frag(p + B_BYTES);
-      }
-#pragma unroll
-      for (int i = 0; i < 4; ++i) {
-        const unsigned char *p = sb + (wm * 4 + i) * 2048;
-        ah[i] = tr_frag(p);
-        if constexpr (NP == 3) al[i] = tr_frag(p + A_BYTES);
-      }
-    };
-    auto multiply = [&](auto mode, int k0) {
-      constexpr int MODE = decltype(mode)::value;
-      constexpr int NITEM = MODE == 1 ? 4 : 4 + NB;
-#pragma unroll
-      for (int t = 0; t < NP; ++t)
-#pragma unroll
-        for (int i = 0; i < 4; ++i)
-#pragma unroll
-          for (int j = 0; j < WNT; ++j) {
-            if (NP == 3 && t == 0) acc[i][j] = __builtin_amdgcn_mfma_f32_32x32x16_bf16(al[i], bh[j], acc[i][j], 0, 0, 0);
-            else if (NP == 3 && t == 1) acc[i][j] = __builtin_amdgcn_mfma_f32_32x32x16_bf16(ah[i], bl[j], acc[i][j], 0, 0, 0);
-            else acc[i][j] = __builtin_amdgcn_mfma_f32_32x32x16_bf16(ah[i], bh[j], acc[i][j], 0, 0, 0);
-            const int n = t * NMM + i * WNT + j;
-            if constexpr (NP == 3) {
-              if (MODE != 0 && (n & 1) && (n >> 1) < NITEM) {
-                __builtin_amdgcn_sched_barrier(0);
-                if constexpr (MODE == 1) load_piece(n >> 1, k0);
-                if constexpr (MODE == 2) convert_piece(n >> 1);
-                __builtin_amdgcn_sched_barrier(0);
-              }
-            } else if (MODE != 0 && 2 * n < NITEM) {
-              __builtin_amdgcn_sched_barrier(0);
-#pragma unroll
-              for (int u = 2 * n; u < 2 * n + 2 && u < NITEM; ++u) {
-                if constexpr (MODE == 1) load_piece(u, k0);
-                if constexpr (MODE == 2) convert_piece(u);
-              }
-              __builtin_amdgcn_sched_barrier(0);
-            }
-          }
-    };
-    constexpr std::integral_constant<int, 0> bare{};
-    constexpr std::integral_constant<int, 1> with_loads{};
-    constexpr std::integral_constant<int, 2> with_split{};
-#pragma unroll
-    for (int q = 0; q < 4 + NB; ++q) load_piece(q, kbeg);
-#pragma unroll
-    for (int q = 0; q < 4 + NB; ++q) convert_piece(q);
-    store_ab(0);
-    if (nst > 1) {
-#pragma unroll
-      for (int q = 0; q < 4; ++q) load_piece(q, kbeg + 32);
-    }
-    pp_barrier();
-    if (wm == 1) pp_barrier();
-#ifdef CTCN_GEMM_STATS
-    long long gs_work[4] = {0, 0, 0, 0}, gs_wait[4] = {0, 0, 0, 0};
-    const long long gs_t0 = clock64();
-    long long gs_prev = gs_t0;
-#endif
-    auto stage = [&](int s, auto do_store, auto c1) {
-      load_frags(s, 0);
-      if constexpr (decltype(do_store)::value == 1) {
-        __builtin_amdgcn_sched_barrier(0);
-#pragma unroll
-        for (int q = 4; q < 4 + NB; ++q) load_piece(q, kbeg + (s + 1) * 32);
-      }
-      PPB(0);
-      if constexpr (decltype(do_store)::value == 1) multiply(with_split, 0);
-      else multiply(bare, 0);
-      PPB(1);
-      load_frags(s, 1);
-      if constexpr (decltype(do_store)::value == 1) store_ab((s + 1) & 1);
-      PPB(2);
-      multiply(c1, kbeg + (s + 2) * 32);
-      PPB(3);
-    };
-    int s = 0;
-    for (; s + 2 < nst; ++s) stage(s, with_loads, with_loads);
-#ifdef CTCN_GEMM_STATS
-    if (lane == 0 && (wave & 3) == 0 && item == 0 && g_gemm_stats) {
-      long long *o = g_gemm_stats + (wave >> 2) * 16;
-      for (int i = 0; i < 4; ++i) { o[i] = gs_work[i]; o[4 + i] = gs_wait[i]; }
-      o[8] = clock64() - gs_t0; o[9] = nst - 2; o[10] = 0;
-    }
-#endif
-    if (s + 1 < nst) { stage(s, with_loads, bare); ++s; }
-    stage(s, bare, bare);
-    if (wm == 0) pp_barrier();
-
-    float *o = splits > 1 ? part + (size_t)z * M * N : C;
-    const int ldo = splits > 1 ? N : ldc;
-    const float bt = splits > 1 ? 0.0f : beta;
-#pragma unroll
-    for (int i = 0; i < 4; ++i)
-#pragma unroll
-      for (int j = 0; j < WNT; ++j) {
-        const int col = n0 + wn * 32 * WNT + j * 32 + (lane & 31);
-#pragma unroll
-        for (int e = 0; e < 16; ++e) {
-          const int row = m0 + wm * 128 + i * 32 + (e & 3) + 8 * (e >> 2) + 4 * (lane >> 5);
-          if (row < M && col < N) {
-            float v = acc[i][j][e];
-            float *p = o + (size_t)row * ldo + col;
-            if (bt != 0.0f) v += bt * *p;
-            *p = v;
-          }
-        }
-      }
+#include "gemm_tn_item.h"
     __syncthreads();
   }
 }
 
-__global__ void splitk_reduce_kernel(const float *__restrict__ ws, float *__restrict__ C, int M, int N, int ldc,
-                                     int splits, float beta) {
+constexpr int TN_GROUP_MAX = 8;
+struct TnProductArgs {
+  const float *A, *B;
+  float *C, *part;
+  int M, N, K, lda, ldb, ldc, kchunk, splits, tiles_n, nt;
+  float beta;
+};
+struct TnGroupArgs { TnProductArgs p[TN_GROUP_MAX]; int start[TN_GROUP_MAX + 1]; };
+
+template <int WNT, int NP>
+__global__ __launch_bounds__(512) void gemm_tn_group_kernel(const TnGroupArgs g, unsigned xcd_mask, unsigned *__restrict__ queue) {
+  constexpr int TBM = 256, TBN = 128 * WNT;
+  constexpr int A_BYTES = TBM * 64, B_BYTES = TBN * 64;
+  constexpr int STAGE = 2 * A_BYTES + 2 * B_BYTES;
+  constexpr int NB = 2 * WNT;
+  constexpr int NMM = 4 * WNT;
+  extern __shared__ __attribute__((aligned(16))) unsigned char qsm[];
+  __shared__ int s_item;
+  {
+    unsigned xcc;
+    asm volatile("s_getreg_b32 %0, hwreg(HW_REG_XCC_ID)" : "=s"(xcc));
+    if (!((xcd_mask >> (xcc & 15u)) & 1u)) return;
+  }
+  const int tid = threadIdx.x, lane = tid & 63, wave = __builtin_amdgcn_readfirstlane(tid >> 6);
+  const int wm = wave >> 2, wn = wave & 3;
+  const int krow = lane >> 3, c4 = 4 * (lane & 7);
+  const int bsub = WNT == 2 ? wave : (wave & 3), bk0 = WNT == 2 ? 0 : 16 * (wave >> 2);
+  const int st_a = wave * 2048 + krow * 64 + (lane & 7) * 8;
+  const int st_b = 2 * A_BYTES + bsub * 2048 + (bk0 + krow) * 64 + (lane & 7) * 8;
+  const int troff = (8 * (lane >> 5) + ((lane & 15) >> 2)) * 64 + ((lane >> 4) & 1) * 32 + (lane & 3) * 8;
+  typedef __attribute__((address_space(3))) s16x4_t *lds4_t;
+
+  for (;;) {
+    if (tid == 0) s_item = (int)atomicAdd(queue, 1u);
+    __syncthreads();
+    const int qi = __builtin_amdgcn_readfirstlane(s_item);
+    if (qi >= g.start[TN_GROUP_MAX]) return;
+    int pi = 0;
+#pragma unroll
+    for (int i = 1; i < TN_GROUP_MAX; ++i) pi += qi >= g.start[i] ? 1 : 0;
+    const TnProductArgs &a = g.p[pi];
+    const int item = qi - g.start[pi], nt = a.nt;
+    const int M = a.M, N = a.N, K = a.K, lda = a.lda, ldb = a.ldb, ldc = a.ldc, kchunk = a.kchunk, splits = a.splits, tiles_n = a.tiles_n;
+    const float *__restrict__ const A = a.A, *__restrict__ const B = a.B;
+    float *__restrict__ const C = a.C, *__restrict__ const part = a.part;
+    const float beta = a.beta;
+#include "gemm_tn_item.h"
+    __syncthreads();
+  }
+}
+
+__device__ __forceinline__ void splitk_reduce_body(const float *__restrict__ ws, float *__restrict__ C, int M, int N, int ldc, int splits, float beta) {
   const size_t total = (size_t)M * N;
   if ((N & 3) == 0 && (ldc & 3) == 0 && (((uintptr_t)C | (uintptr_t)ws) & 15) == 0 && total < ((size_t)1 << 33)) {
     const unsigned n4 = (unsigned)(N >> 2), total4 = (unsigned)(total >> 2);
@@ -1489,6 +1362,14 @@
     if (beta != 0.0f) s += beta * *p;
     *p = s;
   }
+}
+__global__ void splitk_reduce_kernel(const float *__restrict__ ws, float *__restrict__ C, int M, int N, int ldc,
+                                     int splits, float beta) {
+  splitk_reduce_body(ws, C, M, N, ldc, splits, beta);
+}
+__global__ void splitk_reduce_group_kernel(const TnGroupArgs g) {
+  const TnProductArgs &a = g.p[blockIdx.y];
+  if (a.splits > 1) splitk_reduce_body(a.part, a.C, a.M, a.N, a.ldc, a.splits, a.beta);
 }
 
 __global__ void transpose01_kernel(const float *__restrict__ in, float *__restrict__ out, int A, int B, int C) {
@@ -1847,6 +1728,172 @@
   return gemm_core(transA, transB, M, N, K, A, lda, B, ldb, C, ldc, beta, precision, ws, ws_bytes, stream, 0u, nullptr, 0);
 }
 
+struct TnGroupPlan {
+  int n, ngroups;
+  GemmPlan plan[TN_GROUP_MAX];
+  int group[TN_GROUP_MAX];
+  int first[TN_GROUP_MAX], count[TN_GROUP_MAX];
+  size_t off_part[TN_GROUP_MAX];
+  int order[TN_GROUP_MAX];
+  int gbegin[3], gitems[2];
+  size_t off_queue;
+};
+static TnGroupPlan plan_tn_group(int n, const GemmShape *g, const GemmEnv *e, int opt_group) {
+  TnGroupPlan t = {};
+  t.n = n;
+  int wfirst = 0;
+  for (int i = 0; i < n; ++i) {
+    t.plan[i] = plan_gemm(g[i], e[i]);
+    t.group[i] = -1;
+    t.count[i] = t.plan[i].tiles_m * t.plan[i].tiles_n * t.plan[i].splits;
+    if (!wfirst && t.plan[i].path == GP_TN) wfirst = t.plan[i].wnt;
+  }
+  if (n < 2 || !wfirst || opt_group == 0 || (opt_group == 1 && e[0].xcd_allow != 0)) return t;
+  t.off_queue = e[0].ws_bytes >= 256 ? (e[0].ws_bytes - 256) & ~(size_t)255 : 0;
+  for (int c = 0; c < 2; ++c) {
+    const int wnt = c == 0 ? wfirst : 3 - wfirst;
+    int m[TN_GROUP_MAX], nm = 0;
+    for (int i = 0; i < n; ++i)
+      if (t.plan[i].path == GP_TN && t.plan[i].wnt == wnt) m[nm++] = i;
+    if (nm < 2) continue;
+    std::stable_sort(m, m + nm, [&](int a, int b) { return t.plan[a].kchunk > t.plan[b].kchunk; });
+    size_t part_bytes = 0, off[TN_GROUP_MAX];
+    for (int k = 0; k < nm; ++k) {
+      off[k] = part_bytes;
+      if (t.plan[m[k]].splits > 1) part_bytes += align_up((size_t)t.plan[m[k]].splits * g[m[k]].M * g[m[k]].N * sizeof(float), 256);
+    }
+    if (part_bytes > t.off_queue || part_bytes + 256 > e[0].ws_bytes) continue;
+    const int gi = t.ngroups++;
+    int at = t.gbegin[gi];
+    for (int k = 0; k < nm; ++k) {
+      const int i = m[k];
+      t.group[i] = gi; t.first[i] = t.gitems[gi]; t.gitems[gi] += t.count[i]; t.off_part[i] = off[k];
+      t.order[at++] = i;
+    }
+    t.gbegin[gi + 1] = at;
+  }
+  return t;
+}
+static bool all_grouped(const TnGroupPlan &t) {
+  for (int i = 0; i < t.n; ++i)
+    if (t.group[i] < 0) return false;
+  return t.n > 0;
+}
+static std::atomic<long> g_tn_group_launches{0};
+extern "C" int ctcn_diag_tn_group_launches(long long *out) {
+  CTCN_REQUIRE(out, "ctcn_diag_tn_group_launches: null pointer");
+  *out = g_tn_group_launches.load();
+  return CTCN_OK;
+}
+
+static GemmEnv tn_env(const ctcn_tn_product &q, bool has_ws, size_t ws_bytes, unsigned xcd_allow, int cus, int xcds) {
+  return {(int)((uintptr_t)q.A & 15), (int)((uintptr_t)q.B & 15), has_ws, ws_bytes, xcd_allow, false, false, cus, xcds, gemm_options()};
+}
+bool ctcn_tn_group_applies(int n, const ctcn_tn_product *p, int precision, bool has_ws, size_t ws_bytes, unsigned xcd_allow, int cus, int xcds) {
+  if (n < 2 || n > TN_GROUP_MAX || !p) return false;
+  GemmShape g[TN_GROUP_MAX];
+  GemmEnv e[TN_GROUP_MAX];
+  for (int i = 0; i < n; ++i) {
+    g[i] = {1, 0, p[i].M, p[i].N, p[i].K, p[i].lda, p[i].ldb, p[i].ldc, precision, 0};
+    e[i] = tn_env(p[i], has_ws, ws_bytes, xcd_allow, cus, xcds);
+  }
+  return all_grouped(plan_tn_group(n, g, e, ctcn_get_option("gemm_tn_group")));
+}
+
+static int launch_tn_group(const TnGroupPlan &t, int gi, const ctcn_tn_product *p, char *wsb, hipStream_t st) {
+  unsigned *queue = (unsigned *)(wsb + t.off_queue);
+  TnGroupArgs ga = {};
+  size_t reduce_blocks = 0;
+  const int nm = t.gbegin[gi + 1] - t.gbegin[gi];
+  for (int k = 0; k < nm; ++k) {
+    const int i = t.order[t.gbegin[gi] + k];
+    const GemmPlan &pl = t.plan[i];
+    TnProductArgs &a = ga.p[k];
+    a.A = p[i].A; a.B = p[i].B; a.C = p[i].C;
+    a.part = pl.splits > 1 ? (float *)(wsb + t.off_part[i]) : nullptr;
+    a.M = p[i].M; a.N = p[i].N; a.K = p[i].K; a.lda = p[i].lda; a.ldb = p[i].ldb; a.ldc = p[i].ldc;
+    a.kchunk = pl.kchunk; a.splits = pl.splits; a.tiles_n = pl.tiles_n; a.nt = pl.tiles_m * pl.tiles_n;
+    a.beta = p[i].beta;
+    ga.start[k] = t.first[i];
+    if (pl.splits > 1) reduce_blocks = std::max(reduce_blocks, std::min((size_t)2048, ceil_div_z((size_t)a.M * a.N, 256)));
+  }
+  for (int k = nm; k <= TN_GROUP_MAX; ++k) ga.start[k] = t.gitems[gi];
+  CTCN_HIP(hipMemsetAsync(queue, 0, 128, st));
+  const GemmPlan &p0 = t.plan[t.order[t.gbegin[gi]]];
+  const int rc = with_wnt(p0.wnt, [&](auto W) {
+    constexpr int WNT = decltype(W)::value;
+    return launch_tile256(bf16_single() ? gemm_tn_group_kernel<WNT, 1> : gemm_tn_group_kernel<WNT, 3>, p0.grid_x, WNT, st, ga, p0.xcd_mask, queue);
+  });
+  if (rc) return rc;
+  CTCN_LAUNCH_CHECK();
+  if (reduce_blocks) {
+    hipLaunchKernelGGL(splitk_reduce_group_kernel, dim3((unsigned)reduce_blocks, nm), dim3(256), 0, st, ga);
+    CTCN_LAUNCH_CHECK();
+  }
+  g_tn_group_launches.fetch_add(1);
+  return CTCN_OK;
+}
+static int tn_product_alone(const ctcn_tn_product &q, int precision, void *ws, size_t ws_bytes, void *stream, unsigned xcd_allow) {
+  return gemm_core(1, 0, q.M, q.N, q.K, q.A, q.lda, q.B, q.ldb, q.C, q.ldc, q.beta, precision, ws, ws_bytes, stream, xcd_allow, nullptr, 0);
+}
+int ctcn_gemm_tn_group_try(int n, const ctcn_tn_product *p, int precision, void *ws, size_t ws_bytes, void *stream, unsigned xcd_allow, bool *taken) {
+  *taken = false;
+  CTCN_REQUIRE(p && n >= 1 && n <= TN_GROUP_MAX, "ctcn_gemm_tn_group: 1 to %d products, got %d", TN_GROUP_MAX, n);
+  CTCN_REQUIRE(!ws || (uintptr_t)ws % 16 == 0, "ctcn_gemm_tn_group: the workspace must be 16-byte aligned");
+  GemmShape g[TN_GROUP_MAX];
+  GemmEnv e[TN_GROUP_MAX];
+  const int opt = ctcn_get_option("gemm_tn_group"), cus = ctcn_device_cus();
+  bool any_tn = false;
+  for (int i = 0; i < n; ++i) {
+    g[i] = {1, 0, p[i].M, p[i].N, p[i].K, p[i].lda, p[i].ldb, p[i].ldc, precision, 0};
+    if (const int rc = check_gemm_shape(g[i])) return rc;
+    CTCN_REQUIRE(p[i].A && p[i].B && p[i].C, "ctcn_gemm_tn_group: null pointer");
+    e[i] = tn_env(p[i], ws != nullptr, ws_bytes, xcd_allow, cus, 0);
+    any_tn = any_tn || tn_eligible(g[i], e[i]);
+  }
+  if (n < 2 || opt == 0 || !any_tn) return CTCN_OK;
+  const int xcds = ctcn_device_xcds();
+  for (int i = 0; i < n; ++i) e[i].xcds = xcds;
+  const TnGroupPlan t = plan_tn_group(n, g, e, opt);
+  if (!t.ngroups) return CTCN_OK;
+  for (int gi = 0; gi < t.ngroups; ++gi)
+    if (const int rc = launch_tn_group(t, gi, p, (char *)ws, (hipStream_t)stream)) return rc;
+  for (int i = 0; i < n; ++i)
+    if (t.group[i] < 0)
+      if (const int rc = tn_product_alone(p[i], precision, ws, ws_bytes, stream, xcd_allow)) return rc;
+  *taken = true;
+  return CTCN_OK;
+}
+extern "C" int ctcn_gemm_tn_group(int n, const ctcn_tn_product *p, int precision, void *ws, size_t ws_bytes, void *stream, unsigned xcd_allow) {
+  bool taken = false;
+  if (const int rc = ctcn_gemm_tn_group_try(n, p, precision, ws, ws_bytes, stream, xcd_allow, &taken)) return rc;
+  if (taken) return CTCN_OK;
+  for (int i = 0; i < n; ++i)
+    if (const int rc = tn_product_alone(p[i], precision, ws, ws_bytes, stream, xcd_allow)) return rc;
+  return CTCN_OK;
+}
+extern "C" int ctcn_diag_tn_group_plan(int n, const int *shapes, int precision, int has_ws, size_t ws_bytes, int cus, int xcds, unsigned xcd_allow,
+                                       long long *out) {
+  CTCN_REQUIRE(shapes && out && n >= 1 && n <= TN_GROUP_MAX && cus > 0 && xcds > 0, "ctcn_diag_tn_group_plan: bad args");
+  GemmShape g[TN_GROUP_MAX];
+  GemmEnv e[TN_GROUP_MAX];
+  for (int i = 0; i < n; ++i) {
+    const int *s = shapes + 8 * i;
+    g[i] = {1, 0, s[0], s[1], s[2], s[3], s[4], s[5], precision, 0};
+    if (const int rc = check_gemm_shape(g[i])) return rc;
+    CTCN_REQUIRE(s[6] >= 0 && s[6] < 16 && s[7] >= 0 && s[7] < 16, "ctcn_diag_tn_group_plan: bad args");
+    e[i] = {s[6], s[7], has_ws != 0, ws_bytes, xcd_allow, false, false, cus, xcds, gemm_options()};
+  }
+  const TnGroupPlan t = plan_tn_group(n, g, e, ctcn_get_option("gemm_tn_group"));
+  for (int i = 0; i < n; ++i) {
+    const bool in = t.group[i] >= 0;
+    const long long v[CTCN_TN_GROUP_PLAN_INTS] = {in, t.group[i], in ? t.first[i] : 0, t.count[i], t.plan[i].splits, t.plan[i].kchunk,
+                                                 in ? (long long)t.off_part[i] : 0, t.plan[i].path == GP_TN};
+    memcpy(out + (size_t)CTCN_TN_GROUP_PLAN_INTS * i, v, sizeof(v));
+  }
+  return CTCN_OK;
+}
+
 constexpr double DX_WIDE_COST = 1.87;
 struct DxPlan { bool eligible, wide; int tiles_wide, tiles_128; };
 static DxPlan plan_dx(int M, int N, int K, int lda, int precision, int a_mod16, bool has_ws, size_t ws_bytes, int cus, int opt_wide, bool single) {
diff --git a/ctc_pytorch_amd/csrc/gemm_tn_item.h b/ctc_pytorch_amd/csrc/gemm_tn_item.h
--- /dev/null
+++ b/ctc_pytorch_amd/csrc/gemm_tn_item.h
@@ -0,0 +1,179 @@
+    const int z = item / nt, tile = item - z * nt;
+    const int tm = tile / tiles_n, tn = tile - tm * tiles_n;
+    const int m0 = tm * TBM, n0 = tn * TBN;
+    const int kbeg = z * kchunk, kend = min(K, kbeg + kchunk);
+    const int nst = (kend - kbeg + 31) / 32;
+
+    f32x16 acc[4][WNT];
+#pragma unroll
+    for (int i = 0; i < 4; ++i)
+#pragma unroll
+      for (int j = 0; j < WNT; ++j)
+#pragma unroll
+        for (int e = 0; e < 16; ++e) acc[i][j][e] = 0.0f;
+
+    const int acol = m0 + 32 * wave + c4, bcol = n0 + 32 * bsub + c4;
+    const bool a_ok = acol < M, b_ok = bcol < N;
+    u32x4 pw[4 + NB];
+    const unsigned voff_a = a_ok ? (unsigned)((krow * lda + acol) * 4) : 0xfffffff0u;
+    const unsigned voff_b = b_ok ? (unsigned)((krow * ldb + bcol) * 4) : 0xfffffff0u;
+    auto load_piece = [&](int q, int k0) {
+      const int kr = q < 4 ? k0 + 8 * q : k0 + bk0 + 8 * (q - 4);
+      const int ld = q < 4 ? lda : ldb;
+      const float *base = (q < 4 ? A : B) + (size_t)min(kr, K - 1) * ld;
+      int rows = min(8, kend - kr);
+      asm volatile("" : "+s"(rows));
+      const int nrec = max(0, rows) * ld * 4;
+      const __amdgpu_buffer_rsrc_t rs = __builtin_amdgcn_make_buffer_rsrc(const_cast<float *>(base), 0, nrec, 0x00020000);
+      pw[q] = __builtin_amdgcn_raw_buffer_load_b128(rs, q < 4 ? voff_a : voff_b, 0, 0);
+    };
+    auto split_pair = [](float a, float b, unsigned &hw, unsigned &lw) {
+      typedef __bf16 bf16x2_t __attribute__((ext_vector_type(2)));
+      typedef float f32x2_t __attribute__((ext_vector_type(2)));
+      hw = __builtin_bit_cast(unsigned, __builtin_convertvector((f32x2_t){a, b}, bf16x2_t));
+      const f32x2_t r = {a - __uint_as_float(hw << 16), b - __uint_as_float(hw & 0xffff0000u)};
+      lw = __builtin_bit_cast(unsigned, __builtin_convertvector(r, bf16x2_t));
+    };
+    auto convert_piece = [&](int q) {
+      unsigned h01, l01, h23, l23;
+      if constexpr (NP == 3) {
+        split_pair(__uint_as_float(pw[q][0]), __uint_as_float(pw[q][1]), h01, l01);
+        split_pair(__uint_as_float(pw[q][2]), __uint_as_float(pw[q][3]), h23, l23);
+      } else {
+        typedef __bf16 bf16x2_t __attribute__((ext_vector_type(2)));
+        typedef float f32x2_t __attribute__((ext_vector_type(2)));
+        h01 = __builtin_bit_cast(unsigned, __builtin_convertvector((f32x2_t){__uint_as_float(pw[q][0]), __uint_as_float(pw[q][1])}, bf16x2_t));
+        h23 = __builtin_bit_cast(unsigned, __builtin_convertvector((f32x2_t){__uint_as_float(pw[q][2]), __uint_as_float(pw[q][3])}, bf16x2_t));
+        l01 = l23 = 0u;
+      }
+      pw[q] = (u32x4){h01, h23, l01, l23};
+    };
+    auto store_ab = [&](int buf) {
+      unsigned char *sb = qsm + buf * STAGE;
+#pragma unroll
+      for (int q = 0; q < 4 + NB; ++q) {
+        unsigned char *p = sb + (q < 4 ? st_a + q * 512 : st_b + (q - 4) * 512);
+        *reinterpret_cast<uint2 *>(p) = make_uint2(pw[q][0], pw[q][1]);
+        if constexpr (NP == 3) *reinterpret_cast<uint2 *>(p + (q < 4 ? A_BYTES : B_BYTES)) = make_uint2(pw[q][2], pw[q][3]);
+      }
+    };
+    bf16x8_t ah[4], al[4], bh[WNT], bl[WNT];
+    auto tr_frag = [&](const unsigned char *p) {
+      const s16x4_t x0 = __builtin_amdgcn_ds_read_tr16_b64_v4i16((lds4_t)(p));
+      const s16x4_t x1 = __builtin_amdgcn_ds_read_tr16_b64_v4i16((lds4_t)(p + 256));
+      return __builtin_bit_cast(bf16x8_t, __builtin_shufflevector(x0, x1, 0, 1, 2, 3, 4, 5, 6, 7));
+    };
+    auto load_frags = [&](int stage, int ks) {
+      const unsigned char *sb = qsm + (stage & 1) * STAGE + ks * 1024 + troff;
+#pragma unroll
+      for (int j = 0; j < WNT; ++j) {
+        const unsigned char *p = sb + 2 * A_BYTES + (wn * WNT + j) * 2048;
+        bh[j] = tr_frag(p);
+        if constexpr (NP == 3) bl[j] = tr_frag(p + B_BYTES);
+      }
+#pragma unroll
+      for (int i = 0; i < 4; ++i) {
+        const unsigned char *p = sb + (wm * 4 + i) * 2048;
+        ah[i] = tr_frag(p);
+        if constexpr (NP == 3) al[i] = tr_frag(p + A_BYTES);
+      }
+    };
+    auto multiply = [&](auto mode, int k0) {
+      constexpr int MODE = decltype(mode)::value;
+      constexpr int NITEM = MODE == 1 ? 4 : 4 + NB;
+#pragma unroll
+      for (int t = 0; t < NP; ++t)
+#pragma unroll
+        for (int i = 0; i < 4; ++i)
+#pragma unroll
+          for (int j = 0; j < WNT; ++j) {
+            if (NP == 3 && t == 0) acc[i][j] = __builtin_amdgcn_mfma_f32_32x32x16_bf16(al[i], bh[j], acc[i][j], 0, 0, 0);
+            else if (NP == 3 && t == 1) acc[i][j] = __builtin_amdgcn_mfma_f32_32x32x16_bf16(ah[i], bl[j], acc[i][j], 0, 0, 0);
+            else acc[i][j] = __builtin_amdgcn_mfma_f32_32x32x16_bf16(ah[i], bh[j], acc[i][j], 0, 0, 0);
+            const int n = t * NMM + i * WNT + j;
+            if constexpr (NP == 3) {
+              if (MODE != 0 && (n & 1) && (n >> 1) < NITEM) {
+                __builtin_amdgcn_sched_barrier(0);
+                if constexpr (MODE == 1) load_piece(n >> 1, k0);
+                if constexpr (MODE == 2) convert_piece(n >> 1);
+                __builtin_amdgcn_sched_barrier(0);
+              }
+            } else if (MODE != 0 && 2 * n < NITEM) {
+              __builtin_amdgcn_sched_barrier(0);
+#pragma unroll
+              for (int u = 2 * n; u < 2 * n + 2 && u < NITEM; ++u) {
+                if constexpr (MODE == 1) load_piece(u, k0);
+                if constexpr (MODE == 2) convert_piece(u);
+              }
+              __builtin_amdgcn_sched_barrier(0);
+            }
+          }
+    };
+    constexpr std::integral_constant<int, 0> bare{};
+    constexpr std::integral_constant<int, 1> with_loads{};
+    constexpr std::integral_constant<int, 2> with_split{};
+#pragma unroll
+    for (int q = 0; q < 4 + NB; ++q) load_piece(q, kbeg);
+#pragma unroll
+    for (int q = 0; q < 4 + NB; ++q) convert_piece(q);
+    store_ab(0);
+    if (nst > 1) {
+#pragma unroll
+      for (int q = 0; q < 4; ++q) load_piece(q, kbeg + 32);
+    }
+    pp_barrier();
+    if (wm == 1) pp_barrier();
+#ifdef CTCN_GEMM_STATS
+    long long gs_work[4] = {0, 0, 0, 0}, gs_wait[4] = {0, 0, 0, 0};
+    const long long gs_t0 = clock64();
+    long long gs_prev = gs_t0;
+#endif
+    auto stage = [&](int s, auto do_store, auto c1) {
+      load_frags(s, 0);
+      if constexpr (decltype(do_store)::value == 1) {
+        __builtin_amdgcn_sched_barrier(0);
+#pragma unroll
+        for (int q = 4; q < 4 + NB; ++q) load_piece(q, kbeg + (s + 1) * 32);
+      }
+      PPB(0);
+      if constexpr (decltype(do_store)::value == 1) multiply(with_split, 0);
+      else multiply(bare, 0);
+      PPB(1);
+      load_frags(s, 1);
+      if constexpr (decltype(do_store)::value == 1) store_ab((s + 1) & 1);
+      PPB(2);
+      multiply(c1, kbeg + (s + 2) * 32);
+      PPB(3);
+    };
+    int s = 0;
+    for (; s + 2 < nst; ++s) stage(s, with_loads, with_loads);
+#ifdef CTCN_GEMM_STATS
+    if (lane == 0 && (wave & 3) == 0 && item == 0 && g_gemm_stats) {
+      long long *o = g_gemm_stats + (wave >> 2) * 16;
+      for (int i = 0; i < 4; ++i) { o[i] = gs_work[i]; o[4 + i] = gs_wait[i]; }
+      o[8] = clock64() - gs_t0; o[9] = nst - 2; o[10] = 0;
+    }
+#endif
+    if (s + 1 < nst) { stage(s, with_loads, bare); ++s; }
+    stage(s, bare, bare);
+    if (wm == 0) pp_barrier();
+
+    float *o = splits > 1 ? part + (size_t)z * M * N : C;
+    const int ldo = splits > 1 ? N : ldc;
+    const float bt = splits > 1 ? 0.0f : beta;
+#pragma unroll
+    for (int i = 0; i < 4; ++i)
+#pragma unroll
+      for (int j = 0; j < WNT; ++j) {
+        const int col = n0 + wn * 32 * WNT + j * 32 + (lane & 31);
+#pragma unroll
+        for (int e = 0; e < 16; ++e) {
+          const int row = m0 + wm * 128 + i * 32 + (e & 3) + 8 * (e >> 2) + 4 * (lane >> 5);
+          if (row < M && col < N) {
+            float v = acc[i][j][e];
+            float *p = o + (size_t)row * ldo + col;
+            if (bt != 0.0f) v += bt * *p;
+            *p = v;
+          }
+        }
+      }
diff --git a/ctc_pytorch_amd/csrc/rnn.hip b/ctc_pytorch_amd/csrc/rnn.hip
--- a/ctc_pytorch_amd/csrc/rnn.hip
+++ b/ctc_pytorch_amd/csrc/rnn.hip
@@ -2220,6 +2220,37 @@
   return ctcn_rnn_fwd_ex(cell, T, B, I, H, dirs, x, w_ih0, w_hh0, w_ih1, w_hh1, y, gates, aux, precision, ws, ws_bytes, stream, &c);
 }
 
+static int weight_products(int cell, int T, int B, int I, int H, int dirs, const float *x, const float *y, const float *gates, const float *aux,
+                           float *const dw_ih[2], float *const dw_hh[2], float beta_w, ctcn_tn_product *out) {
+  const int GH = gates_of(cell) * H, TB = T * B, Kh = (T - 1) * B, ldg = dirs * GH;
+  int n = 0;
+  for (int d = 0; d < dirs; ++d) {
+    if (!dw_ih[d]) continue;
+    const float *da = gates + (size_t)d * GH;
+    const size_t offA = d == 0 ? (size_t)B : 0, offY = d == 0 ? 0 : (size_t)B;
+    const float *yh = y + (size_t)d * H + offY * dirs * H;
+    out[n++] = {GH, I, TB, da, ldg, x, I, dw_ih[d], I, beta_w};
+    if (cell == CTCN_CELL_GRU) {
+      out[n++] = {2 * H, H, Kh, da + offA * ldg, ldg, yh, dirs * H, dw_hh[d], H, beta_w};
+      out[n++] = {H, H, Kh, aux + (size_t)d * H + offA * dirs * H, dirs * H, yh, dirs * H, dw_hh[d] + (size_t)2 * H * H, H, beta_w};
+    } else {
+      out[n++] = {GH, H, Kh, da + offA * ldg, ldg, yh, dirs * H, dw_hh[d], H, beta_w};
+    }
+  }
+  return n;
+}
+
+extern "C" int ctcn_diag_rnn_weights_grouped(int cell, int T, int B, int I, int H, int dirs, int precision, size_t ws_bytes, int cus, int xcds,
+                                             unsigned xcd_allow) {
+  if (cell < 0 || cell > 2 || T <= 0 || B <= 0 || I <= 0 || H <= 0 || (dirs != 1 && dirs != 2) || cus <= 0 || xcds <= 0) return -1;
+  if (T < 2) return 0;
+  float *const base = (float *)(uintptr_t)4096;
+  float *const dw_ih[2] = {base, dirs == 2 ? base : nullptr}, *const dw_hh[2] = {base, dirs == 2 ? base : nullptr};
+  ctcn_tn_product list[6];
+  const int n = weight_products(cell, T, B, I, H, dirs, base, base, base, base, dw_ih, dw_hh, 1.0f, list);
+  return ctcn_tn_group_applies(n, list, precision, ws_bytes > 0, ws_bytes, xcd_allow, cus, xcds) ? 1 : 0;
+}
+
 static int rnn_bwd_gemms(int cell, int T, int B, int I, int H, int dirs, const float *x, const float *w_ih0, const float *w_ih1,
                          const float *y, const float *gates, const float *aux, float *dx, float *dw_ih0, float *dw_hh0, float *dw_ih1,
                          float *dw_hh1, float beta_w, int precision, bool weights, unsigned xcd_allow, void *ws, size_t ws_bytes,
@@ -2239,6 +2270,12 @@
       dx_done = true;
     }
   }
+  bool dw_grouped = false;
+  if (weights && T > 1 && (dw_ih[0] || (dirs == 2 && dw_ih[1]))) {
+    ctcn_tn_product list[6];
+    const int n = weight_products(cell, T, B, I, H, dirs, x, y, gates, aux, dw_ih, dw_hh, beta_w, list);
+    if (int rc = ctcn_gemm_tn_group_try(n, list, precision, ws, ws_bytes, stream, xcd_allow, &dw_grouped)) return rc;
+  }
   for (int d = 0; d < dirs; ++d) {
     const float *da = gates + (size_t)d * GH;
     const int ldg = dirs * GH;
@@ -2247,7 +2284,7 @@
       rc = ctcn_gemm_on_xcds(0, 0, TB, I, GH, da, ldg, w_ih[d], I, dx, I, d == 0 ? 0.0f : 1.0f, precision, ws, ws_bytes, stream, xcd_allow);
       if (rc) return rc;
     }
-    if (!weights || !dw_ih[d]) continue;
+    if (!weights || !dw_ih[d] || dw_grouped) continue;
     rc = ctcn_gemm_on_xcds(1, 0, GH, I, TB, da, ldg, x, I, dw_ih[d], I, beta_w, precision, ws, ws_bytes, stream, xcd_allow, &pl);
     if (rc) return rc;
     const int Kh = (T - 1) * B;
diff --git a/ctc_pytorch_amd/ops.py b/ctc_pytorch_amd/ops.py
--- a/ctc_pytorch_amd/ops.py
+++ b/ctc_pytorch_amd/ops.py
@@ -257,6 +257,12 @@
     return WG_INLINE, 0
 
 
+def plan_grouped_weights(mode, cell, T, B, I, H, dirs, prec, ws_bytes, cus, xcds, tail=True):
+    if mode not in (WG_SPLIT_END, WG_SPLIT_NOW) or dirs != 2 or not tail:
+        return False
+    return _lib.lib().ctcn_diag_rnn_weights_grouped(int(cell), T, B, I, H, dirs, int(prec), int(ws_bytes), int(cus), int(xcds), 0) == 1
+
+
 class _DeviceSide(object):
 
     def __init__(self, dev):
@@ -372,6 +378,39 @@
     _lib.check(_lib.lib().ctcn_gemm_dx(M, N, K, _ptr(A), lda, _ptr(Bm), ldb, _ptr(C), ldc, float(beta), get_precision(), wp, wn, _lib.stream_ptr()),
                "gemm_dx")
     return C
+
+
+def gemm_tn_group(products, xcd_allow=0, ws_tag="main"):
+    _need_gpu(*[t for p in products for t in (p[3], p[5], p[7])])
+    w, wp, wn = _ws(products[0][7], tag=ws_tag)
+    arr = (_lib.TnProduct * len(products))()
+    for q, (M, N, K, A, lda, Bm, ldb, C, ldc, beta) in zip(arr, products):
+        q.M, q.N, q.K, q.A, q.lda, q.B, q.ldb, q.C, q.ldc, q.beta = M, N, K, A.data_ptr(), lda, Bm.data_ptr(), ldb, C.data_ptr(), ldc, float(beta)
+    _lib.check(_lib.lib().ctcn_gemm_tn_group(len(products), ctypes.cast(arr, ctypes.c_void_p), get_precision(), wp, wn, _lib.stream_ptr(), int(xcd_allow)),
+               "gemm_tn_group")
+
+
+def tn_group_launches():
+    n = ctypes.c_longlong(0)
+    _lib.check(_lib.lib().ctcn_diag_tn_group_launches(ctypes.cast(ctypes.pointer(n), ctypes.c_void_p)), "diag_tn_group_launches")
+    return n.value
+
+
+TN_GROUP_PLAN_KEYS = ("grouped", "group", "first", "items", "splits", "kchunk", "off_part", "tn")
+
+
+def tn_group_plan(shapes, prec=1, ws_bytes=None, cus=256, xcds=8, xcd_allow=0):
+    ws_bytes = _lib.WORKSPACE_BYTES if ws_bytes is None else int(ws_bytes)
+    flat = []
+    for s in shapes:
+        M, N, K = s[:3]
+        lda, ldb, ldc = s[3:6] if len(s) >= 6 else (M, N, N)
+        flat += [M, N, K, lda, ldb, ldc] + (list(s[6:8]) if len(s) >= 8 else [0, 0])
+    out = (ctypes.c_longlong * (len(TN_GROUP_PLAN_KEYS) * len(shapes)))()
+    _lib.check(_lib.lib().ctcn_diag_tn_group_plan(len(shapes), ctypes.cast((ctypes.c_int * len(flat))(*flat), ctypes.c_void_p), int(prec), 1 if ws_bytes else 0,
+                                                  ws_bytes, int(cus), int(xcds), int(xcd_allow), ctypes.cast(out, ctypes.c_void_p)), "diag_tn_group_plan")
+    k = len(TN_GROUP_PLAN_KEYS)
+    return [dict(zip(TN_GROUP_PLAN_KEYS, out[k * i:k * i + k])) for i in range(len(shapes))]
 
 
 class _Linear(torch.autograd.Function):
@@ -540,7 +579,9 @@
         _note_launch(launched.value, b"rnn_bwd_step", cell, T, B, H, dirs)
         if above is not None:
             above(ev)
-        if mode in (WG_SPLIT_END, WG_SPLIT_NOW):
+        if plan_grouped_weights(mode, cell, T, B, I, H, dirs, prec, wn, L.ctcn_device_cus(), L.ctcn_device_xcds(), tail=dx is None):
+            _weight_grads(cell, dims, s, dws, prec)
+        elif mode in (WG_SPLIT_END, WG_SPLIT_NOW):
             st, main = side.side_stream(), torch.cuda.current_stream(dev)
             st.wait_stream(main)
             with torch.cuda.stream(st):
diff --git a/include/ctcn.h b/include/ctcn.h
--- a/include/ctcn.h
+++ b/include/ctcn.h
@@ -34,6 +34,15 @@
 
 int ctcn_gemm_dx(int M, int N, int K, const float *A, int lda, const float *B, int ldb, float *C, int ldc, float beta, int precision, void *ws,
                  size_t ws_bytes, void *stream);
+
+typedef struct ctcn_tn_product {
+  int M, N, K;
+  const float *A; int lda;
+  const float *B; int ldb;
+  float *C; int ldc;
+  float beta;
+} ctcn_tn_product;
+int ctcn_gemm_tn_group(int n, const ctcn_tn_product *p, int precision, void *ws, size_t ws_bytes, void *stream, unsigned xcd_allow);
 
 int ctcn_transpose01(const float *in, float *out, int A, int B, int C, void *stream);
 int ctcn_copy_strided4(const float *in, float *out, int d0, int d1, int d2, int d3, size_t s0, size_t s1, size_t s2,
@@ -324,6 +333,10 @@
                            float beta, int precision, void *ws, size_t ws_bytes, void *stream, unsigned xcd_allow);
 #define CTCN_DX_PLAN_INTS 4
 int ctcn_diag_dx_plan(int M, int N, int K, int lda, int precision, int a_mod16, int has_ws, size_t ws_bytes, int cus, int *out);
+#define CTCN_TN_GROUP_PLAN_INTS 8
+int ctcn_diag_tn_group_plan(int n, const int *shapes, int precision, int has_ws, size_t ws_bytes, int cus, int xcds, unsigned xcd_allow, long long *out);
+int ctcn_diag_tn_group_launches(long long *out);
+int ctcn_diag_rnn_weights_grouped(int cell, int T, int B, int I, int H, int dirs, int precision, size_t ws_bytes, int cus, int xcds, unsigned xcd_allow);
 #define CTCN_BEAM_PLAN_INTS 19
 int ctcn_diag_beam_plan(int T, int B, int V, int W, int lds_max, int generic_static_lds, int *out);
 #define CTCN_CTC_LATTICE_PLAN_INTS 6
```

Result: no change. 1.998 million frames/s (median of 6 runs) (+0.3%).
